# zengxianyu/sketchedit

Hardware: AMD Instinct MI355X
Metric: images/sec (higher is better)
Workload: dtype f32; 1 GPU; SketchEdit inference forward (netM+netG, use_cam, pool max) 256x256 batch 32 per GPU, procedural weights; global_batch=32, size=256, per_gpu_batch=32, execution=default, two streams

## Files before the change

sketchedit_amd/csrc/se_api.hip:

```cpp
#include "../../include/sketchedit_hip.h"
#include "../../include/sketchedit_png.h"
#include "se_kernels.h"
#include "se_pack.h"

#include <cstdarg>
#include <cstdint>
#include <cstdlib>
#include <cstdio>
#include <cstring>
#include <algorithm>
#include <map>
#include <mutex>
#include <numeric>
#include <string>
#include <vector>

using namespace se;

namespace {


#define ENC(p)                                                                                    \
  {p "2_downsample", 24, 96, 3, 2, 1, ACT_ELU, 0}, {p "3", 48, 96, 3, 1, 1, ACT_ELU, 0},          \
      {p "4_downsample", 48, 192, 3, 2, 1, ACT_ELU, 0}, {p "5", 96, 192, 3, 1, 1, ACT_ELU, 0},    \
      {p "6", 96, 192, 3, 1, 1, ACT_ELU, 0}, {p "7_atrous", 96, 192, 3, 1, 2, ACT_ELU, 0},        \
      {p "8_atrous", 96, 192, 3, 1, 4, ACT_ELU, 0}, {p "9_atrous", 96, 192, 3, 1, 8, ACT_ELU, 0}, \
      {p "10_atrous", 96, 192, 3, 1, 16, ACT_ELU, 0}
#define DEC(p, c11in, c17out)                                                                        \
  {p "11", c11in, 192, 3, 1, 1, ACT_ELU, 0}, {p "12", 96, 192, 3, 1, 1, ACT_ELU, 0},                 \
      {p "13_upsample_conv", 96, 96, 3, 1, 1, ACT_ELU, 1}, {p "14", 48, 96, 3, 1, 1, ACT_ELU, 0},    \
      {p "15_upsample_conv", 48, 48, 3, 1, 1, ACT_ELU, 1}, {p "16", 24, 24, 3, 1, 1, ACT_ELU, 0},    \
      {p "17", 12, c17out, 3, 1, 1, ACT_NONE, 0}

const LayerDef G_LAYERS[] = {
    {"conv1", 5, 48, 5, 1, 1, ACT_ELU, 0}, ENC("conv"), DEC("conv", 192, 3),
    {"wconv1", 5, 48, 5, 1, 1, ACT_ELU, 0}, ENC("wconv"),
    {"xconv1", 3, 48, 5, 1, 1, ACT_ELU, 0},
    {"xconv2_downsample", 24, 48, 3, 2, 1, ACT_ELU, 0}, {"xconv3", 24, 96, 3, 1, 1, ACT_ELU, 0},
    {"xconv4_downsample", 48, 96, 3, 2, 1, ACT_ELU, 0}, {"xconv5", 48, 192, 3, 1, 1, ACT_ELU, 0},
    {"xconv6", 96, 192, 3, 1, 1, ACT_ELU, 0}, {"xconv7_atrous", 96, 192, 3, 1, 2, ACT_ELU, 0},
    {"xconv8_atrous", 96, 192, 3, 1, 4, ACT_ELU, 0}, {"xconv9_atrous", 96, 192, 3, 1, 8, ACT_ELU, 0},
    {"xconv10_atrous", 96, 192, 3, 1, 16, ACT_ELU, 0},
    {"pmconv1", 3, 48, 5, 1, 1, ACT_ELU, 0},
    {"pmconv2_downsample", 24, 48, 3, 2, 1, ACT_ELU, 0}, {"pmconv3", 24, 96, 3, 1, 1, ACT_ELU, 0},
    {"pmconv4_downsample", 48, 192, 3, 2, 1, ACT_ELU, 0}, {"pmconv5", 96, 192, 3, 1, 1, ACT_ELU, 0},
    {"pmconv6", 96, 192, 3, 1, 1, ACT_RELU, 0}, {"pmconv9", 96, 192, 3, 1, 1, ACT_ELU, 0},
    {"pmconv10", 96, 192, 3, 1, 1, ACT_ELU, 0},
    DEC("allconv", 192, 3),
};
const LayerDef M_LAYERS[] = {
    {"conv1", 4, 48, 5, 1, 1, ACT_ELU, 0}, ENC("conv"), DEC("conv", 96, 3), DEC("conv_mask_", 96, 1),
};
const int NG = sizeof(G_LAYERS) / sizeof(LayerDef), NM = sizeof(M_LAYERS) / sizeof(LayerDef);


struct Arena {
  struct Blk { size_t off, size; bool used; };
  std::vector<Blk> blks;
  size_t cap = 0, peak = 0;
  bool dry = false;
  char* base = nullptr;
  void reset(char* b, size_t c, bool d, int which = 0) {
    base = d ? (char*)(which ? ((size_t)1 << 62) + 4096 : 4096) : b;
    cap = d ? (size_t)1 << 61 : c; dry = d; peak = 0;
    blks.clear(); blks.push_back({0, cap, false});
  }
  bool owns(const void* p) const { return (size_t)p >= (size_t)base && (size_t)p < (size_t)base + cap; }
  float* alloc(size_t nfloats) {
    size_t need = (nfloats * 4 + 255) & ~(size_t)255;
    for (size_t i = 0; i < blks.size(); ++i) {
      if (!blks[i].used && blks[i].size >= need) {
        size_t off = blks[i].off;
        if (blks[i].size > need) {
          Blk rest{off + need, blks[i].size - need, false};
          blks[i].size = need;
          blks.insert(blks.begin() + i + 1, rest);
        }
        blks[i].used = true;
        if (off + need > peak) peak = off + need;
        return (float*)(base + off);
      }
    }
    return nullptr;
  }
  void release(const float* p) {
    if (!p) return;
    size_t off = (const char*)p - base;
    for (size_t i = 0; i < blks.size(); ++i) {
      if (blks[i].off == off && blks[i].used) {
        blks[i].used = false;
        if (i + 1 < blks.size() && !blks[i + 1].used) { blks[i].size += blks[i + 1].size; blks.erase(blks.begin() + i + 1); }
        if (i > 0 && !blks[i - 1].used) { blks[i - 1].size += blks[i].size; blks.erase(blks.begin() + i); }
        return;
      }
    }
  }
};

}

struct se_ctx {
  int device = 0;
  std::mutex mu;
  std::string err;
  std::map<std::string, Layer> G, M;
  Layer wconv1_j4;
  float* zeros = nullptr;
  float* lut8 = nullptr;
  Arena arena;
  Arena arena2;
  hipStream_t st = nullptr;
  hipStream_t st_main = nullptr;
  hipStream_t st_side = nullptr;
  hipEvent_t ev_fork = nullptr, ev_join = nullptr;
  bool dry = false;
  bool low_latency = false;
  int cur_net = SE_NET_G;
  bool bf16 = false;
  bool serial = false;
  bool fork2 = true;
  bool conservative = false;
  const se_netG_taps* taps = nullptr;
  float* vbias_ws = nullptr;
  const float* vec32 = nullptr;
  unsigned char* rgb8 = nullptr;
  unsigned char* m8 = nullptr;
  Profiler prof;
  struct Peaks { size_t main, side; };
  std::map<std::vector<long long>, Peaks> peaks;
  size_t dry_max_act = 0;
  std::map<std::vector<long long>, long long> act_per_img;
  struct GraphEntry {
    std::vector<long long> key;
    hipGraph_t graph = nullptr;
    hipGraphExec_t exec = nullptr;
    hipStream_t stream = nullptr;
    unsigned long long last_use = 0;
  };
  unsigned long long graph_clock = 0;
  std::vector<GraphEntry> graphs;
  struct ResampleTable {
    int in, out, filter, ksize;
    std::vector<int> host;
    int* dev = nullptr;
    unsigned long long last_use = 0;
  };
  std::vector<ResampleTable> rs_tables;
  unsigned long long rs_clock = 0;
  unsigned char* rs_scratch = nullptr;
  size_t rs_scratch_bytes = 0;
  hipStream_t rs_stream = nullptr;
  bool rs_used = false;
  hipEvent_t rs_event = nullptr;
  se_window* win_host = nullptr;
  se_window* win_dev = nullptr;
  size_t win_cap = 0, win_pos = 0;
  hipEvent_t win_half_done[2] = {nullptr, nullptr};
  bool win_half_used[2] = {false, false};
  hipStream_t win_stream = nullptr;
  bool win_used = false;
  hipEvent_t win_event = nullptr;
};

namespace {

thread_local std::string g_create_err;

int fail(se_ctx* c, const char* fmt, ...) {
  char buf[512];
  va_list ap;
  va_start(ap, fmt);
  vsnprintf(buf, sizeof buf, fmt, ap);
  va_end(ap);
  if (c) c->err = buf; else g_create_err = buf;
  return 1;
}
#define HIPCHK(c, call)                                                                   \
  do {                                                                                    \
    hipError_t e_ = (call);                                                               \
    if (e_ != hipSuccess) return fail(c, "%s failed: %s (%s:%d)", #call, hipGetErrorString(e_), __FILE__, __LINE__); \
  } while (0)

int xcd_remap_enabled() { return opt(OPT_XCD_REMAP); }

long long addr_limit() {
  const int v = opt(OPT_TEST_OFFSET_LIMIT);
  return v > 0 ? (long long)v : (1ll << 31);
}

int poison_byte() {
  const int v = opt(OPT_TEST_POISON);
  return v >= 1 && v <= 255 ? v : 0;
}
int poison(se_ctx* c, void* p, size_t bytes, hipStream_t st) {
  const int v = poison_byte();
  if (!v || !p || !bytes) return 0;
  HIPCHK(c, hipMemsetAsync(p, v, bytes, st));
  return 0;
}

int try_rtile(se_ctx* c, const Layer& L, bool bf, const float* src0, int C0, const float* src1, float* dst, int B, int Hin, int Win,
              int Ho, int Wo, int pad, bool* done) {
  *done = false;
  const LayerDef& d = L.def;
  if (!opt(OPT_RTILE) || src1 || d.stride != 1 || d.rate != 1 || (L.cfg != GC_N48 && L.cfg != GC_N24)) return 0;
  {
    const int TR0 = rtile_rows(bf);
    const long tiles = (long)B * ((Hin + TR0 - 1) / TR0) * ((Win + 15) / 16) * (d.up ? 4 : 1);
    if (c->low_latency && tiles < opt(OPT_RTILE_LL_MIN)) return 0;
  }
  const int es = bf ? 2 : 4, gran = bf ? 8 : 4;
  const DirectImage& di = L.direct[bf];
  const int CG = di.CG, nch = di.nch;
  const float* wimg = di.w;
  if (!wimg || C0 != CG * gran) return 0;
  {
    const int wx_mode = opt(OPT_RTILE_WX);
    if (wx_mode != 0 && !bf && L.d_wx && d.k == 3 && !d.up && C0 == 24 && d.cin == 24 && d.cout == 24 && (Win % 2) == 0 &&
        (long long)B * Hin * Win * 96 < (1ll << 31)) {
      RTileParams p;
      memset(&p, 0, sizeof p);
      p.src = src0; p.wpk = L.d_wx; p.bias = L.d_b; p.dst = dst;
      p.B = B; p.Hin = Hin; p.Win = Win; p.C = C0; p.G = L.G; p.OH = Ho; p.OW = Wo;
      p.ty = (Hin + 15) / 16; p.tx = (Win + 15) / 16;
      p.act = d.act; p.xcd = xcd_remap_enabled(); p.NP = 32;
      udiv_magic_host((unsigned)(p.ty * p.tx), &p.div_cg_m, &p.div_cg_l);
      udiv_magic_host((unsigned)p.tx, &p.div_rw_m, &p.div_rw_l);
      const double alg = 2.0 * (double)B * Ho * Wo * d.cout * d.cin * 9;
      const bool two_d = wx_mode != 1 && L.d_wx2 && (Hin % 2) == 0;
      set_launch_cost(alg, 4.0 * ((double)B * Hin * Win * d.cin + (double)B * Ho * Wo * (d.cout / 2)), d.name,
                      (double)B * p.ty * p.tx * 8.0 * (two_d ? 96.0 : 160.0) * 2048.0);
      if (two_d) {
        p.wpk = L.d_wx2;
        HIPCHK(c, launch_rtilew2(p, c->st));
        *done = true;
        return 0;
      }
      HIPCHK(c, launch_rtilew(p, c->st));
      *done = true;
      return 0;
    }
  }
  if (opt(OPT_RTILE_DENSE) != 0 && !bf && L.d_wd && L.dense && d.k == 5 && !d.up && L.cfg == GC_N48 && (long long)Hin * Win * C0 * 4 < (1ll << 31)) {
    const long long per_img = (long long)Hin * Win * C0 * 4;
    const long long lim = addr_limit();
    const int bmax = (int)std::max<long long>(1, (lim - 1) / per_img);
    for (int b0 = 0; b0 < B; b0 += bmax) {
      const int nb = std::min(bmax, B - b0);
      RTileParams p;
      memset(&p, 0, sizeof p);
      p.src = src0 + (size_t)b0 * Hin * Win * C0; p.wpk = L.d_wd; p.bias = L.d_b; p.dst = dst + (size_t)b0 * Ho * Wo * L.G;
      p.B = nb; p.Hin = Hin; p.Win = Win; p.C = C0; p.G = L.G; p.OH = Ho; p.OW = Wo;
      p.ty = (Hin + 7) / 8; p.tx = (Win + 15) / 16;
      p.act = d.act; p.xcd = xcd_remap_enabled(); p.dense = L.dense; p.nch = L.nchd; p.NP = 48;
      const double alg = 2.0 * (double)nb * Ho * Wo * d.cout * d.cin * 25;
      if (opt(OPT_RTILE_D5W) != 0 && L.d_wdw && (Win % 2) == 0) {
        p.wpk = L.d_wdw; p.dense = L.dense + 100;
        set_launch_cost(alg, 4.0 * ((double)nb * Hin * Win * d.cin + (double)nb * Ho * Wo * (d.cout / 2)), d.name,
                        (double)nb * p.ty * p.tx * 4.0 * (6.0 * ((5 * L.dense + 3) / 4) * 3.0) * 2048.0);
        HIPCHK(c, launch_rtile(p, c->st));
        continue;
      }
      set_launch_cost(alg, 4.0 * ((double)nb * Hin * Win * d.cin + (double)nb * Ho * Wo * (d.cout / 2)), d.name,
                      2.0 * (double)nb * Hin * Win * 48.0 * (4.0 * ((25 * L.dense + 3) / 4)));
      HIPCHK(c, launch_rtile(p, c->st));
    }
    *done = true;
    return 0;
  }
  if (opt(OPT_RTILE_DENSE) != 0 && bf && L.d_w16d && d.k == 5 && !d.up && L.cfg == GC_N48 && C0 == 8 &&
      (long long)B * Hin * Win * 16 < (1ll << 31)) {
    RTileParams p;
    memset(&p, 0, sizeof p);
    p.src = src0; p.wpk = L.d_w16d; p.bias = L.d_b; p.dst = dst;
    p.B = B; p.Hin = Hin; p.Win = Win; p.C = C0; p.CG = 1; p.T = 25; p.KW = 5;
    p.pad = pad; p.OH = Ho; p.OW = Wo; p.G = (L.G + 7) & ~7;
    p.nch = 2; p.NP = 48; p.RH = 32 + 4; p.RW = 21;
    p.raw_bytes = (p.RH * p.RW * 8 + 1023) & ~1023;
    udiv_magic_host((unsigned)p.RW, &p.div_rw_m, &p.div_rw_l);
    udiv_magic_host(1u, &p.div_cg_m, &p.div_cg_l);
    p.ty = (Hin + 31) / 32; p.tx = (Win + 15) / 16;
    p.act = d.act; p.bf16 = 1; p.xcd = xcd_remap_enabled(); p.dense = 204;
    const double alg = 2.0 * (double)B * Ho * Wo * d.cout * d.cin * 25;
    set_launch_cost(alg, 2.0 * ((double)B * Hin * Win * d.cin + (double)B * Ho * Wo * (d.cout / 2)), d.name,
                    2.0 * (double)B * Hin * Win * 48.0 * 128.0);
    HIPCHK(c, launch_rtile(p, c->st));
    *done = true;
    return 0;
  }
  const int KW = d.up ? 2 : d.k, KH = KW;
  RTileParams p;
  memset(&p, 0, sizeof p);
  const int TR = rtile_rows(bf);
  p.RH = TR + KH - 1; p.RW = 16 + KW - 1;
  p.raw_bytes = (p.RH * p.RW * C0 * es + 1023) & ~1023;
  if (p.raw_bytes + nch * L.NP * 128 > 80 * 1024) return 0;
  if ((long long)B * Hin * Win * C0 * es >= (1ll << 31)) return 0;
  p.src = src0; p.wpk = wimg; p.bias = L.d_b; p.dst = dst;
  p.B = B; p.Hin = Hin; p.Win = Win; p.C = C0; p.CG = CG; p.T = L.T; p.KW = KW;
  p.magicCG = (65536 + CG - 1) / CG; p.magicKW = 256 / KW + 1;
  for (int gi = 0; gi < nch * 8 + 8; ++gi)
    if (((gi * p.magicCG) >> 16) != gi / CG) return 0;
  for (int t = 0; t <= L.T + 8; ++t)
    if (((t * p.magicKW) >> 8) != t / KW) return 0;
  p.pad = pad; p.up2 = d.up ? 1 : 0; p.OH = Ho; p.OW = Wo;
  p.G = bf ? (L.G + 7) & ~7 : L.G;
  p.nch = nch; p.NP = L.NP;
  udiv_magic_host((unsigned)(C0 * es / 16), &p.div_cg_m, &p.div_cg_l);
  udiv_magic_host((unsigned)p.RW, &p.div_rw_m, &p.div_rw_l);
  p.ty = (Hin + TR - 1) / TR; p.tx = (Win + 15) / 16;
  p.act = d.act; p.bf16 = bf ? 1 : 0; p.xcd = xcd_remap_enabled();
  {
    const double alg = 2.0 * (double)B * Ho * Wo * d.cout * d.cin * d.k * d.k;
    const double exec = 2.0 * (double)B * Hin * Win * (d.up ? 4.0 : 1.0) * L.NP * (nch * (bf ? 64.0 : 32.0));
    set_launch_cost(alg, (double)es * ((double)B * Hin * Win * d.cin + (double)B * Ho * Wo * (d.cout / 2)), d.name, exec);
  }
  HIPCHK(c, launch_rtile(p, c->st));
  *done = true;
  return 0;
}

int run_gather(se_ctx* c, const Layer& L, bool bf, const float* src0, int C0, const float* src1, int C1, int src1_vec, float* dst,
               int B, int Hin, int Win, int Ho, int Wo, int pad) {
  const LayerDef& d = L.def;
  const DirectImage& di = L.direct[bf];
  const int es = bf ? 2 : 4, gran = bf ? 8 : 4;
  GConvParams p;
  memset(&p, 0, sizeof p);
  p.bf16 = bf ? 1 : 0;
  p.src0 = src0; p.src1 = src1 ? src1 : src0; p.wpk = di.w; p.bias = L.d_b; p.dst = dst; p.zeros = c->zeros;
  p.B = B; p.Hin = Hin; p.Win = Win; p.Ho = d.up ? Hin : Ho; p.Wo = d.up ? Win : Wo;
  p.up2 = d.up ? 1 : 0; p.OH = Ho; p.OW = Wo;
  p.C0 = C0; p.C1 = C1 ? C1 : C0; p.C0g = C0 / gran; p.CG = di.CG;
  const int KW = d.up ? 2 : d.k;
  p.T = L.T; p.KW = KW; p.stride = d.stride; p.dil = d.rate; p.pad = pad;
  p.magicCG = (65536 + di.CG - 1) / di.CG; p.magicKW = 256 / KW + 1; p.magicKH = L.T / KW;
  for (int gi = 0; gi < di.nch * 8 + 8; ++gi)
    if (((gi * p.magicCG) >> 16) != gi / di.CG) return fail(c, "layer %s: magic division check failed", d.name);
  for (int t = 0; t <= L.T + 8; ++t)
    if (((t * p.magicKW) >> 8) != t / KW) return fail(c, "layer %s: magic tap division check failed", d.name);
  const int Gs = bf ? (L.G + 7) & ~7 : L.G;
  if ((double)B * Hin * Win * (C0 > C1 ? C0 : C1) * es >= 2147483648.0 || (double)B * Ho * Wo * Gs * es >= 2147483648.0)
    return fail(c, "layer %s: a tensor of this launch exceeds 2^31 bytes (32-bit byte offsets) -- split the batch", d.name);
  for (int j = 0; j < p.magicKH; ++j) p.rep |= 1u << (j * KW);
  udiv_magic_host((unsigned)(p.Ho * p.Wo), &p.div_hw_m, &p.div_hw_l);
  udiv_magic_host((unsigned)p.Wo, &p.div_w_m, &p.div_w_l);
  p.Hlim = Hin; p.Wlim = Win;
  p.src1_vec = src1_vec; p.nch = di.nch; p.G = Gs; p.act = d.act; p.total_pix = B * p.Ho * p.Wo;
  p.xcd = xcd_remap_enabled();
  p.np_full = L.NP; p.nf_full = L.NP / 32; p.small_grid = c->low_latency ? 1 : 0;
  {
    const double alg = 2.0 * (double)B * Ho * Wo * d.cout * d.cin * d.k * d.k;
    const double exec = 2.0 * (double)B * p.Ho * p.Wo * (d.up ? 4.0 : 1.0) * L.NP * (di.nch * (bf ? 64.0 : 32.0));
    set_launch_cost(alg, (double)es * ((double)B * Hin * Win * d.cin + (double)B * Ho * Wo * (d.cout / 2)), d.name, exec);
  }
  HIPCHK(c, launch_gconv(L.cfg, p, c->st));
  return 0;
}

static bool rconv16_dual_ok(const Layer& L, const LayerDef& d, int Hin, int Win) {
  if (opt(OPT_RCONV16_DUAL) == 0) return false;
  return L.d_w16s && (d.rate % 2) == 0 && Win / d.rate == 8 && Hin / d.rate <= 8 && Hin / d.rate >= 4;
}

int run_gconv16(se_ctx* c, const Layer& L, const float* src0, int C0, const float* src1, int C1, int src1_vec, float* dst,
                int B, int Hin, int Win, int Ho, int Wo, int pad) {
  const LayerDef& d = L.def;
  if (!L.direct[1].w) return fail(c, "layer %s: no bf16 weight image", d.name);
  if ((C0 + C1) != L.direct[1].CG * 8) return fail(c, "layer %s: bf16 source channels %d+%d != packed %d", d.name, C0, C1, L.direct[1].CG * 8);
  const bool use_rconv = opt(OPT_RCONV16) != 0;
  {
    if (opt(OPT_VECBIAS) != 0 && use_rconv && !c->low_latency && src1 && src1_vec && c->vbias_ws && c->vec32 && L.d_w16s && L.d_wv16 &&
        d.k == 3 && d.stride == 1 && d.rate == 1 && !d.up && d.cin == 192 && d.cout == 192 && C0 == 96 && C1 == 96 &&
        Hin >= 12 && Win >= 12 && (long long)B * Hin * Win * 192 < (1ll << 31)) {
      HIPCHK(c, launch_vecbias(L.d_wv16, c->vec32, c->vbias_ws, B, 96, c->st, 1));
      RConvParams rp;
      memset(&rp, 0, sizeof rp);
      rp.src = src0; rp.wpk = L.d_w16s; rp.bias = L.d_b; rp.dst = dst; rp.vbias = c->vbias_ws;
      rp.B = B; rp.h = Hin; rp.w = Win; rp.d = 1; rp.hs = Hin; rp.ws = Win;
      rp.ty = (Hin + 7) / 8; rp.tx = (Win + 15) / 16;
      rp.act = d.act; rp.xcd = xcd_remap_enabled();
      const double alg = 2.0 * (double)B * Ho * Wo * d.cout * d.cin * 9;
      set_launch_cost(alg, 2.0 * 2.0 * (double)B * Hin * Win * 96, d.name, 2.0 * (double)B * Hin * Win * 192.0 * 864.0);
      HIPCHK(c, launch_rconv16(rp, c->st));
      return 0;
    }
  }
  if (use_rconv && !c->low_latency && d.k == 3 && d.stride == 1 && !d.up && d.cin == 96 && d.cout == 192 && !src1 && C0 == 96 &&
      (Hin % d.rate) == 0 && (Win % d.rate) == 0 && L.direct[1].nch == 14 && L.d_w16s && (long long)B * Hin * Win * 192 < (1ll << 31) &&
      ((Hin / d.rate >= 12 && Win / d.rate >= 12) || rconv16_dual_ok(L, d, Hin, Win))) {
    RConvParams rp;
    memset(&rp, 0, sizeof rp);
    rp.dual = !(Hin / d.rate >= 12 && Win / d.rate >= 12);
    rp.src = src0; rp.wpk = L.d_w16s; rp.bias = L.d_b; rp.dst = dst;
    rp.B = B; rp.h = Hin; rp.w = Win; rp.d = d.rate; rp.hs = Hin / d.rate; rp.ws = Win / d.rate;
    rp.ty = (rp.hs + 7) / 8; rp.tx = (rp.ws + 15) / 16;
    rp.act = d.act; rp.xcd = xcd_remap_enabled();
    const double alg = 2.0 * (double)B * Ho * Wo * d.cout * d.cin * 9;
    set_launch_cost(alg, 2.0 * 2.0 * (double)B * Hin * Win * 96, d.name, 2.0 * (double)B * Hin * Win * 192.0 * 864.0);
    HIPCHK(c, launch_rconv16(rp, c->st));
    return 0;
  }
  const bool use_rconv96 = opt(OPT_RCONV96) != 0;
  if (use_rconv96 && !c->low_latency && L.d_w96 && !src1 && C0 == d.cin && Hin >= 12 && Win >= 12 &&
      (long long)B * Ho * Wo * 96 < (1ll << 31) && (long long)B * Hin * Win * C0 * 2 < (1ll << 31)) {
    RConv96Params rp;
    memset(&rp, 0, sizeof rp);
    rp.src = src0; rp.wpk = L.d_w96; rp.bias = L.d_b; rp.dst = dst;
    rp.B = B; rp.h = Hin; rp.w = Win; rp.CG = C0 / 8;
    rp.stride = d.stride; rp.oh = Ho; rp.ow = Wo;
    rp.ty = ((d.stride == 2 ? Ho : Hin) + 15) / 16; rp.tx = ((d.stride == 2 ? Wo : Win) + 15) / 16;
    rp.up2 = d.up ? 1 : 0; rp.act = d.act; rp.xcd = xcd_remap_enabled();
    const int T = d.up ? 4 : 9, nstep = (T * rp.CG + 3) / 4;
    const double alg = 2.0 * (double)B * Ho * Wo * d.cout * d.cin * 9;
    set_launch_cost(alg, 2.0 * ((double)B * Hin * Win * d.cin + (double)B * Ho * Wo * 48), d.name,
                    2.0 * (double)B * (d.stride == 2 ? (double)Ho * Wo : (double)Hin * Win) * (d.up ? 4.0 : 1.0) * 96.0 * (nstep * 32.0));
    HIPCHK(c, launch_rconv96(rp, c->st));
    return 0;
  }
  {
    bool done = false;
    if (try_rtile(c, L, true, src0, C0, src1, dst, B, Hin, Win, Ho, Wo, pad, &done)) return 1;
    if (done) return 0;
  }
  return run_gather(c, L, true, src0, C0, src1, C1, src1_vec, dst, B, Hin, Win, Ho, Wo, pad);
}

static WinoParams wino_params(const float* src, const float* upk, const float* bias, float* dst, int B, int h, int w, int d,
                              int tcols, int act) {
  WinoParams wp;
  memset(&wp, 0, sizeof wp);
  wp.src = src; wp.upk = upk; wp.bias = bias; wp.dst = dst;
  wp.B = B; wp.h = h; wp.w = w; wp.d = d; wp.th = h / 2; wp.tw = w / tcols;
  wp.total_tiles = B * wp.th * wp.tw; wp.act = act;
  wp.xcd = xcd_remap_enabled();
  udiv_magic_host((unsigned)(wp.th * wp.tw), &wp.div_tpi_m, &wp.div_tpi_l);
  udiv_magic_host((unsigned)wp.tw, &wp.div_tw_m, &wp.div_tw_l);
  udiv_magic_host((unsigned)wp.d, &wp.div_d_m, &wp.div_d_l);
  return wp;
}

int run_gconv(se_ctx* c, const Layer& L, const float* src0, int C0, const float* src1, int C1, int src1_vec, float* dst,
              int B, int Hin, int Win) {
  const LayerDef& d = L.def;
  const ConvShape sh = conv_shape(d, Hin, Win);
  const int Ho = sh.Ho, Wo = sh.Wo, pad = sh.pad;
  if (!L.packed) return fail(c, "layer %s: weights not loaded", d.name);
  if (c->bf16) return run_gconv16(c, L, src0, C0, src1, C1, src1_vec, dst, B, Hin, Win, Ho, Wo, pad);
  if ((C0 + C1) != L.direct[0].CG * 4) return fail(c, "layer %s: source channels %d+%d != packed %d", d.name, C0, C1, L.direct[0].CG * 4);
  const int ll_min_wg = opt(OPT_LL_WINO_MIN_WG), ll_min_wg48 = opt(OPT_LL_WINO48_MIN_WG);
  auto wino_grid_ok = [&](long wgs, bool n192 = false) {
    const int m = n192 ? ll_min_wg : ll_min_wg48;
    return !c->low_latency || (m > 0 && wgs >= m);
  };
  const bool use_wino = opt(OPT_WINOGRAD) != 0;
  const bool wino_src_ok = (!src1 && C0 == 96 && d.cin == 96) || (src1 && C0 == 96 && C1 == 96 && d.cin == 192);
  const bool wino_addr_ok = (long long)B * Hin * Win * 384 < (1ll << 31);
  const double alg3x3 = 2.0 * (double)B * Ho * Wo * d.cout * d.cin * 9;
  if (use_wino && !d.up && L.d_u && wino_src_ok && !wino_addr_ok) {
    static bool said = false;
    if (!said) {
      said = true;
      fprintf(stderr, "sketchedit_hip: layer %s: %d x %dx%d x 96 floats exceed the Winograd kernel's 32-bit byte offsets; "
                      "using the direct kernel (about 2x slower) -- split the batch\n", d.name, B, Hin, Win);
    }
  }
  if (use_wino && !d.up && L.d_u && wino_src_ok && wino_addr_ok && (Hin % (2 * d.rate)) == 0 && (Win % (2 * d.rate)) == 0 &&
      wino_grid_ok(((long)(Hin / 2) * (Win / 2) + 63) / 64, true)) {
    const bool folded = opt(OPT_VECBIAS) != 0 && src1 && src1_vec && d.rate == 1 && L.d_u1 && L.d_wv && c->vbias_ws && Hin >= 2 && Win >= 2;
    if (folded) HIPCHK(c, launch_vecbias(L.d_wv, src1, c->vbias_ws, B, 96, c->st));
    const float* s1 = folded ? nullptr : src1;
    const int f43_mode = opt(OPT_WINOGRAD_F43);
    const bool f43_net_ok = c->cur_net == SE_NET_G || (f43_mode == 1 && !c->conservative);
    const bool f43 = (f43_mode == 1 || f43_mode == 2) && f43_net_ok && (s1 ? (!src1_vec && L.d_u24b) : L.d_u24 != nullptr) && L.d_ub24 && (Win % (4 * d.rate)) == 0;
    WinoParams wp = f43 ? wino_params(src0, s1 ? L.d_u24b : L.d_u24, L.d_ub24, dst, B, Hin, Win, d.rate, 4, d.act)
                        : wino_params(src0, folded ? L.d_u1 : L.d_u, L.d_b, dst, B, Hin, Win, d.rate, 2, d.act);
    wp.src1 = s1; wp.src1_vec = folded ? 0 : src1_vec; wp.vbias = folded ? c->vbias_ws : nullptr;
    if ((double)B * Hin * Win * 384.0 >= 2147483648.0) return fail(c, "layer %s: tensor exceeds 2^31 bytes", d.name);
    if (f43) {
      set_launch_cost(alg3x3, 4.0 * 2.0 * (double)B * Hin * Win * 96, d.name, alg3x3 * 24.0 / 72.0 * (folded ? 0.5 : 1.0));
      HIPCHK(c, launch_wino24(wp, c->st));
      return 0;
    }
    set_launch_cost(alg3x3, 4.0 * 2.0 * (double)B * Hin * Win * 96, d.name, alg3x3 * 16.0 / 36.0 * (folded ? 0.5 : 1.0));
    HIPCHK(c, launch_wino(wp, c->st));
    return 0;
  }
  {
    if (use_wino && opt(OPT_WINOGRAD_F43) != 0 && !d.up && !src1 && C0 == 48 && d.cin == 48 && d.cout == 192 && d.stride == 1 && L.d_u24 && L.d_ub24 &&
        (long long)B * Hin * Win * 384 < (1ll << 31) && (Hin % (2 * d.rate)) == 0 && (Win % (4 * d.rate)) == 0 &&
        wino_grid_ok(((long)(Hin / 2) * (Win / 4) + 31) / 32, true)) {
      const WinoParams wp = wino_params(src0, L.d_u24, L.d_ub24, dst, B, Hin, Win, d.rate, 4, d.act);
      set_launch_cost(alg3x3, 4.0 * ((double)B * Hin * Win * 48 + (double)B * Hin * Win * 96), d.name, alg3x3 * 24.0 / 72.0);
      HIPCHK(c, launch_wino24_c48(wp, c->st));
      return 0;
    }
  }
  const bool use_wino48 = opt(OPT_WINOGRAD48) != 0;
  if (use_wino && use_wino48 && !d.up && L.d_u && L.d_ub && !src1 && C0 == 48 && d.cin == 48 && (long long)B * Hin * Win * 192 < (1ll << 31) &&
      (Hin % (2 * d.rate)) == 0 && (Win % (2 * d.rate)) == 0 && wino_grid_ok(((long)(Hin / 2) * (Win / 2) + 63) / 64)) {
    const WinoParams wp = wino_params(src0, L.d_u, L.d_ub, dst, B, Hin, Win, d.rate, 2, d.act);
    set_launch_cost(alg3x3, 4.0 * 2.0 * (double)B * Hin * Win * 48, d.name, alg3x3 * 16.0 / 36.0);
    HIPCHK(c, launch_wino48(wp, c->st));
    return 0;
  }
  if (use_wino && use_wino48 && !d.up && L.d_u && L.d_ub && !src1 && C0 == 24 && d.cin == 24 && d.cout == 96 && d.stride == 1 &&
      (long long)B * Hin * Win * 192 < (1ll << 31) && (Hin % (2 * d.rate)) == 0 && (Win % (2 * d.rate)) == 0 &&
      wino_grid_ok(((long)(Hin / 2) * (Win / 2) + 63) / 64)) {
    const WinoParams wp = wino_params(src0, L.d_u, L.d_ub, dst, B, Hin, Win, d.rate, 2, d.act);
    set_launch_cost(alg3x3, 4.0 * ((double)B * Hin * Win * 24 + (double)B * Hin * Win * 48), d.name, alg3x3 * 16.0 / 36.0);
    HIPCHK(c, launch_wino48_c24(wp, c->st));
    return 0;
  }
  const bool use_winoup = opt(OPT_WINOGRAD_UP) != 0;
  if (use_wino && use_winoup && d.up && L.d_u && L.d_ub && !src1 && C0 == 96 && d.cin == 96 &&
      (long long)B * Hin * Win * 384 < (1ll << 31) && (Hin % 2) == 0 && (Win % 2) == 0 &&
      wino_grid_ok(4 * (((long)(Hin / 2) * (Win / 2) + 63) / 64))) {
    const WinoParams wp = wino_params(src0, L.d_u, L.d_ub, dst, B, Hin, Win, 1, 2, d.act);
    set_launch_cost(alg3x3, 4.0 * ((double)B * Hin * Win * 96 + (double)B * Ho * Wo * 48), d.name,
                    alg3x3 * 9.0 / 36.0);
    HIPCHK(c, launch_winoup(wp, c->st));
    return 0;
  }
  const bool use_winoup48 = opt(OPT_WINOGRAD_UP48) != 0;
  if (use_wino && use_winoup && use_winoup48 && d.up && L.d_u && L.d_ub && !src1 && C0 == 48 && d.cin == 48 && d.cout == 48 &&
      (long long)B * Hin * Win * 192 < (1ll << 31) && (long long)B * Ho * Wo * 96 < (1ll << 31) && (Hin % 2) == 0 && (Win % 2) == 0 &&
      wino_grid_ok(4 * (((long)(Hin / 2) * (Win / 2) + 63) / 64))) {
    const WinoParams wp = wino_params(src0, L.d_u, L.d_ub, dst, B, Hin, Win, 1, 2, d.act);
    set_launch_cost(alg3x3, 4.0 * ((double)B * Hin * Win * 48 + (double)B * Ho * Wo * 24), d.name,
                    alg3x3 * 9.0 / 36.0 * 28.0 / 27.0);
    HIPCHK(c, launch_winoup48(wp, c->st));
    return 0;
  }
  {
    bool done = false;
    if (try_rtile(c, L, false, src0, C0, src1, dst, B, Hin, Win, Ho, Wo, pad, &done)) return 1;
    if (done) return 0;
  }
  return run_gather(c, L, false, src0, C0, src1, C1, src1_vec, dst, B, Hin, Win, Ho, Wo, pad);
}

struct Act {
  float* p = nullptr;
  int H = 0, W = 0, C = 0;
};

struct Plan {
  se_ctx* c;
  std::map<std::string, Layer>& net;
  int B;
  int rc = 0;
  Arena* ar;
  Plan(se_ctx* c_, std::map<std::string, Layer>& n, int B_) : c(c_), net(n), B(B_), ar(&c_->arena) {}
  float* alloc_raw(size_t nfloats) {
    float* p = ar->alloc(nfloats);
    if (!p && !rc) rc = fail(c, "workspace too small (need more than %zu bytes)", ar->cap);
    if (p && !rc && !c->dry && poison(c, p, (nfloats * 4 + 255) & ~(size_t)255, c->st)) rc = 1;
    return p;
  }
  Act alloc(int H, int W, int C) {
    Act a; a.H = H; a.W = W;
    if (c->bf16) {
      a.C = (C + 7) & ~7;
      a.p = alloc_raw(((size_t)B * H * W * a.C + 1) / 2);
    } else {
      a.C = C;
      a.p = alloc_raw((size_t)B * H * W * C);
    }
    if (c->dry) c->dry_max_act = std::max(c->dry_max_act, (size_t)B * H * W * a.C * (c->bf16 ? 2 : 4));
    return a;
  }
  void release(const float* p) {
    if (!p) return;
    if (c->arena2.owns(p)) c->arena2.release(p); else c->arena.release(p);
  }
  void free(Act& a) { release(a.p); a.p = nullptr; }
  bool forked() const { return (c->low_latency || (c->fork2 && !c->serial)) && c->st_side; }
  int side_begin() {
    if (!forked()) return 0;
    ar = &c->arena2;
    if (c->dry) return 0;
    HIPCHK(c, hipEventRecord(c->ev_fork, c->st_main));
    HIPCHK(c, hipStreamWaitEvent(c->st_side, c->ev_fork, 0));
    c->st = c->st_side;
    return 0;
  }
  int side_end() {
    if (!forked()) return 0;
    ar = &c->arena;
    if (c->dry) return 0;
    HIPCHK(c, hipEventRecord(c->ev_join, c->st_side));
    c->st = c->st_main;
    return 0;
  }
  int join() {
    if (!forked() || c->dry) return 0;
    HIPCHK(c, hipStreamWaitEvent(c->st_main, c->ev_join, 0));
    return 0;
  }
  Act conv(const char* name, Act& in, bool rel = true, const float* src1 = nullptr, int C1 = 0, int vec = 0) {
    if (rc) return Act();
    return conv_layer(net.at(name), in, rel, src1, C1, vec);
  }
  Act conv_layer(Layer& L, Act& in, bool rel = true, const float* src1 = nullptr, int C1 = 0, int vec = 0) {
    Act out;
    if (rc) return out;
    const ConvShape sh = conv_shape(L.def, in.H, in.W);
    out = alloc(sh.Ho, sh.Wo, L.def.cout / 2);
    if (rc) return out;
    if (!c->dry) rc = run_gconv(c, L, in.p, in.C, src1, C1, vec, out.p, B, in.H, in.W);
    if (rel) free(in);
    return out;
  }
};

Act encoder(Plan& P, const std::string& p, Act& in, Act* keep9, Layer* first = nullptr) {
  Act x = first ? P.conv_layer(*first, in) : P.conv((p + "1").c_str(), in);
  x = P.conv((p + "2_downsample").c_str(), x);
  x = P.conv((p + "3").c_str(), x);
  x = P.conv((p + "4_downsample").c_str(), x);
  x = P.conv((p + "5").c_str(), x);
  x = P.conv((p + "6").c_str(), x);
  x = P.conv((p + "7_atrous").c_str(), x);
  x = P.conv((p + "8_atrous").c_str(), x);
  Act x9 = P.conv((p + "9_atrous").c_str(), x);
  Act x10 = P.conv((p + "10_atrous").c_str(), x9, keep9 == nullptr);
  if (keep9) *keep9 = x9;
  return x10;
}

Act decoder(Plan& P, const std::string& p, Act& in, const float* src1 = nullptr, int C1 = 0, int vec = 0) {
  Act x = P.conv((p + "11").c_str(), in, true, src1, C1, vec);
  x = P.conv((p + "12").c_str(), x);
  x = P.conv((p + "13_upsample_conv").c_str(), x);
  x = P.conv((p + "14").c_str(), x);
  x = P.conv((p + "15_upsample_conv").c_str(), x);
  x = P.conv((p + "16").c_str(), x);
  return x;
}

int small(Plan& P, const char* name, Act& in, int mode, float* out_nchw, float* hard, const float* img,
          const float* mask, float* xnow, float* composed, int no_mask_coarse, long packed_bs = 0,
          const unsigned char* lock = nullptr) {
  if (P.rc) return P.rc;
  se_ctx* c = P.c;
  if (!c->dry) {
    Layer& L = P.net.at(name);
    if (!L.packed) return P.rc = fail(c, "layer %s: weights not loaded", name);
    SmallConvParams sp;
    memset(&sp, 0, sizeof sp);
    sp.x = in.p; sp.w = L.direct[c->bf16].w; sp.b = L.d_b; sp.B = P.B; sp.H = in.H; sp.W = in.W; sp.cout = L.def.cout;
    sp.bf16 = c->bf16 ? 1 : 0;
    sp.mode = mode; sp.out_nchw = out_nchw; sp.hard = hard; sp.img = img; sp.mask = mask; sp.xnow = xnow;
    sp.composed = composed; sp.no_mask_coarse = no_mask_coarse;
    if (mode == 3) { sp.rgb8 = c->rgb8; sp.m8 = c->m8; }
    if (mode == 0) sp.lock = lock;
    if (packed_bs) {
      if (mode == 0) sp.out_bs = packed_bs;
      if (mode == 3) { sp.mask_bs = packed_bs; sp.comp_bs = packed_bs; }
    }
    set_launch_cost(2.0 * (double)P.B * in.H * in.W * L.def.cout * 108.0,
                    4.0 * (double)P.B * in.H * in.W * (12 + L.def.cout), L.def.name);
    hipError_t e = launch_small_conv(sp, c->st);
    if (e != hipSuccess) return P.rc = fail(c, "small conv %s: %s", name, hipGetErrorString(e));
  }
  P.free(in);
  return 0;
}

int plan_netM(se_ctx* c, const float* image, const float* sketch, float* mask_out, float* hard_out, float* maskim_out,
              int B, int H, int W, long packed_bs = 0, const unsigned char* lock = nullptr) {
  Plan P(c, c->M, B);
  c->cur_net = SE_NET_M;
  Act in = P.alloc(H, W, 4);
  if (P.rc) return P.rc;
  if (!c->dry) HIPCHK(c, c->bf16 ? launch_pack_m16(image, sketch, in.p, B, H, W, c->st) : launch_pack_m(image, sketch, in.p, B, H, W, c->st));
  Act x9;
  const bool want_img = maskim_out != nullptr;
  Act x10 = encoder(P, "conv", in, want_img ? &x9 : nullptr);
  if (want_img) {
    Act d = decoder(P, "conv", x9);
    small(P, "conv17", d, 1, maskim_out, nullptr, nullptr, nullptr, nullptr, nullptr, 0);
  }
  Act d = decoder(P, "conv_mask_", x10);
  small(P, "conv_mask_17", d, 0, mask_out, hard_out, nullptr, nullptr, nullptr, nullptr, 0, packed_bs, lock);
  return P.rc;
}

int run_attention(se_ctx* c, Plan& P, Act& x, const float* mask_full, Act& out, float* similar_nchw);

int plan_netG(se_ctx* c, const float* x, const float* x2, const float* mask, const float* mask2, const float* guide,
              float* coarse_out, float* fine_out, const float* soft_mask, float* composed_out, int B, int H, int W,
              int flags, long packed_bs = 0) {
  Plan P(c, c->G, B);
  c->cur_net = SE_NET_G;
  const int joint = (flags & SE_FLAG_JOINT_TRAIN_INP) ? 1 : 0;
  Act cin = P.alloc(H, W, 8);
  P.ar = P.forked() ? &c->arena2 : &c->arena;
  Act sin = P.alloc(H, W, joint ? 4 : 8);
  P.ar = &c->arena;
  if (P.rc) return P.rc;
  if (!c->dry)
    HIPCHK(c, (c->bf16 ? launch_pack_g16 : launch_pack_g)(x, x2, mask, mask2, guide, cin.p, sin.p, B, H, W,
                                                          (flags & SE_FLAG_NO_MASK_CC) ? 1 : 0, joint, c->st));
  if (P.side_begin()) return 1;
  Act xs = encoder(P, "wconv", sin, nullptr, joint ? &c->wconv1_j4 : nullptr);
  Act part = P.alloc(1, COLREDUCE_SPLITS, 192), vec32 = P.alloc(1, 1, 192), vec = P.alloc(1, 1, 96);
  if (P.rc) return P.rc;
  if (!c->dry)
    HIPCHK(c, launch_colreduce(xs.p, part.p, c->bf16 ? vec32.p : vec.p, B, xs.H * xs.W, 96, (flags & SE_FLAG_POOL_MAX) ? 0 : 1,
                               c->st, c->bf16 ? 1 : 0, c->bf16 ? vec.p : nullptr));
  if (!c->dry && c->taps && c->taps->style_vec)
    HIPCHK(c, hipMemcpyAsync(c->taps->style_vec, c->bf16 ? vec32.p : vec.p, (size_t)B * 96 * 4, hipMemcpyDeviceToDevice, c->st));
  P.free(xs);
  P.free(part);
  if (!c->bf16) P.free(vec32);
  if (P.side_end()) return 1;
  Act xc = encoder(P, "conv", cin, nullptr);
  if (P.rc) return P.rc;
  if (P.join()) return 1;
  float* vb = P.alloc_raw((size_t)B * 9 * 192);
  if (P.rc) return P.rc;
  c->vbias_ws = vb;
  c->vec32 = c->bf16 ? vec32.p : nullptr;
  Act d = decoder(P, "conv", xc, vec.p, 96, 1);
  c->vbias_ws = nullptr; c->vec32 = nullptr;
  P.release(vb);
  if (c->bf16) P.free(vec32);
  P.free(vec);
  Act xnow = P.alloc(H, W, 4);
  if (P.rc) return P.rc;
  small(P, "conv17", d, 2, coarse_out, nullptr, x, mask, xnow.p, nullptr, (flags & SE_FLAG_NO_MASK_COARSE) ? 1 : 0);
  if (P.rc) return P.rc;
  if (P.side_begin()) return 1;
  Act pm = P.conv("pmconv1", xnow, false);
  pm = P.conv("pmconv2_downsample", pm);
  pm = P.conv("pmconv3", pm);
  pm = P.conv("pmconv4_downsample", pm);
  pm = P.conv("pmconv5", pm);
  pm = P.conv("pmconv6", pm);
  if (P.rc) return P.rc;
  if (!c->dry && c->taps && c->taps->pmconv6)
    HIPCHK(c, (c->bf16 ? launch_nhwc16_to_nchw : launch_nhwc_to_nchw)(pm.p, c->taps->pmconv6, B, 96, 96, pm.H, pm.W, c->st));
  if (flags & SE_FLAG_USE_CAM) {
    Act att = P.alloc(pm.H, pm.W, 96);
    if (P.rc) return P.rc;
    if (run_attention(c, P, pm, mask, att, nullptr)) return P.rc ? P.rc : 1;
    P.free(pm);
    pm = att;
    if (!c->dry && c->taps && c->taps->attn_out)
      HIPCHK(c, (c->bf16 ? launch_nhwc16_to_nchw : launch_nhwc_to_nchw)(pm.p, c->taps->attn_out, B, 96, 96, pm.H, pm.W, c->st));
  }
  pm = P.conv("pmconv9", pm);
  pm = P.conv("pmconv10", pm);
  if (P.rc) return P.rc;
  if (P.side_end()) return 1;
  Act hcur = P.conv("xconv1", xnow, false);
  hcur = P.conv("xconv2_downsample", hcur);
  hcur = P.conv("xconv3", hcur);
  hcur = P.conv("xconv4_downsample", hcur);
  hcur = P.conv("xconv5", hcur);
  hcur = P.conv("xconv6", hcur);
  hcur = P.conv("xconv7_atrous", hcur);
  hcur = P.conv("xconv8_atrous", hcur);
  hcur = P.conv("xconv9_atrous", hcur);
  Act hallu = P.conv("xconv10_atrous", hcur);
  if (P.rc) return P.rc;
  if (P.join()) return 1;
  P.free(xnow);
  Act d2 = decoder(P, "allconv", hallu, pm.p, 96, 0);
  P.free(pm);
  small(P, "allconv17", d2, 3, fine_out, nullptr, x, soft_mask, nullptr, soft_mask ? composed_out : nullptr, 0, packed_bs);
  c->rgb8 = nullptr; c->m8 = nullptr;
  return P.rc;
}

int att_row_stride(int R, bool bf) {
  const int chunk = bf ? 64 : 32;
  int Rp = (R + chunk - 1) / chunk * chunk;
  return Rp;
}

bool att_streaming(int h, int w, bool bf, bool want_similar) {
  const int R = (h / 2) * (w / 2), Rp = att_row_stride(R, bf);
  const bool fits = (double)R * Rp * 4.0 < 2147483648.0;
  if (want_similar && !fits) return true;
  if (opt(OPT_ATT_STREAM) == 1 && !want_similar) return true;
  return !fits;
}

int run_attention(se_ctx* c, Plan& P, Act& x, const float* mask_full, Act& out, float* similar_nchw) {
  const int h = x.H, w = x.W, B = P.B;
  const int hs = (h - 4) / 2 + 1, ws = (w - 4) / 2 + 1, L = hs * ws, Lp = (L + 31) & ~31;
  const bool bf = c->bf16;
  const bool stream = att_streaming(h, w, bf, similar_nchw != nullptr);
  const int hc = h / 2, wc = w / 2, R = hc * wc;
  const int Rp = att_row_stride(R, bf);
  const int guard = (wc + 8 + 63) & ~63;
  if (stream && similar_nchw)
    return P.rc = fail(c, "attention: similar_out (the %d x %d score matrix) is not available on a %dx%d feature map: "
                          "it runs in the streaming form, which never forms it", L, L, h, w);
  float* part = P.alloc_raw((size_t)B * COLREDUCE_SPLITS * 96);
  float* rn = P.alloc_raw((size_t)B * 96);
  float* xn = P.alloc_raw(bf ? ((size_t)B * h * w * 96 + 1) / 2 : (size_t)B * h * w * 96);
  float *valid = nullptr, *S = nullptr, *S2 = nullptr, *xT = nullptr, *stats = nullptr;
  if (stream) {
    valid = P.alloc_raw(3 * (size_t)B * Rp);
    stats = P.alloc_raw((size_t)B * R * 2);
    xT = P.alloc_raw((bf ? (size_t)B * 4 * 96 * Rp / 2 : (size_t)B * 4 * 96 * Rp) + att_stream_xt_tail());
  } else {
    valid = P.alloc_raw(7 * ((size_t)B * Rp + guard) + (size_t)B * 768 + (size_t)B * hc * 384);
    stats = P.alloc_raw((size_t)B * R * 2);
    xT = P.alloc_raw(bf ? (size_t)B * 4 * 96 * Rp / 2 : (size_t)B * 4 * 96 * Rp);
    S = P.alloc_raw((size_t)B * R * Rp + 2 * guard);
    S2 = P.alloc_raw(bf ? (size_t)B * R * Rp / 2 : (size_t)B * R * Rp);
  }
  if (P.rc) return P.rc;
  if (!c->dry) {
    HIPCHK(c, launch_colreduce(x.p, part, rn, B, h * w, 96, 2, c->st, bf ? 1 : 0));
    AttParams a;
    memset(&a, 0, sizeof a);
    a.x = x.p; a.rn = rn; a.xn = xn; a.hard = mask_full; a.out = out.p;
    a.B = B; a.h = h; a.w = w; a.hs = hs; a.ws = ws; a.L = L; a.Lp = Lp;
    a.scale = 10.f; a.th = 0.1f;
    if (stream) {
      a.hc = hc; a.wc = wc; a.R = R; a.Rp = Rp; a.bf16 = bf ? 1 : 0;
      a.validR = valid; a.kmul = valid + (size_t)B * Rp; a.kadd = valid + 2 * (size_t)B * Rp;
      a.xT = xT; a.stats = stats;
      HIPCHK(c, launch_attention_stream(a, c->st));
    } else {
      a.hc = hc; a.wc = wc; a.R = R; a.Rp = Rp; a.bf16 = bf ? 1 : 0;
      a.validR = valid + guard; a.xT = xT; a.E = S + guard; a.P = S2; a.stats = stats; a.guard = guard; a.similar = similar_nchw;
      a.kmul = valid + ((size_t)B * Rp + guard) + guard; a.kadd = valid + 2 * ((size_t)B * Rp + guard) + guard;
      a.kadd2 = valid + 3 * ((size_t)B * Rp + guard) + guard; a.ea4 = valid + 4 * ((size_t)B * Rp + guard) + guard;
      a.ea = valid + 5 * ((size_t)B * Rp + guard) + guard; a.eb = valid + 6 * ((size_t)B * Rp + guard) + guard;
      a.emean = valid + 7 * ((size_t)B * Rp + guard); a.epart = a.emean + (size_t)B * 768;
      HIPCHK(c, launch_attention(a, c->st));
    }
  }
  P.release(S2); P.release(S); P.release(xT); P.release(stats); P.release(valid);
  P.release(xn); P.release(rn); P.release(part);
  return 0;
}

int check_dims(se_ctx* c, int B, int H, int W) {
  if (B < 1 || H < 16 || W < 16 || (H % 8) || (W % 8)) return fail(c, "bad shape B=%d H=%d W=%d (H, W must be multiples of 8, >= 16)", B, H, W);
  return 0;
}

long long max_act_bytes_per_image(se_ctx* c, int H, int W, int flags) {
  const std::vector<long long> key = {H, W, (flags & SE_FLAG_BF16) ? 1 : 0};
  auto it = c->act_per_img.find(key);
  if (it != c->act_per_img.end()) return it->second;
  const bool dry0 = c->dry, ll0 = c->low_latency, bf0 = c->bf16;
  c->dry = true; c->low_latency = false; c->bf16 = (flags & SE_FLAG_BF16) != 0;
  c->dry_max_act = 0;
  float dummy;
  c->arena.reset(nullptr, 0, true, 0); c->arena2.reset(nullptr, 0, true, 1);
  plan_netM(c, nullptr, nullptr, nullptr, nullptr, &dummy, 1, H, W, 0);
  c->arena.reset(nullptr, 0, true, 0); c->arena2.reset(nullptr, 0, true, 1);
  plan_netG(c, nullptr, nullptr, nullptr, nullptr, nullptr, nullptr, nullptr, nullptr, nullptr, 1, H, W, SE_FLAG_USE_CAM | SE_FLAG_POOL_MAX, 0);
  c->dry = dry0; c->low_latency = ll0; c->bf16 = bf0;
  const long long v = (long long)c->dry_max_act;
  c->act_per_img[key] = v;
  return v;
}

int pass_size(se_ctx* c, int B, int H, int W, int flags) {
  const long long per_img = max_act_bytes_per_image(c, H, W, flags);
  const long long lim = addr_limit();
  if (per_img <= 0) { fail(c, "internal: no activation size for %dx%d", H, W); return 0; }
  if (per_img >= lim) {
    fail(c, "a %dx%d image exceeds the kernels' 32-bit byte offsets (%lld bytes per activation, limit %lld)", H, W, per_img, lim);
    return 0;
  }
  const long long bmax = (lim - 1) / per_img;
  if (B <= bmax) return B;
  const long long passes = (B + bmax - 1) / bmax;
  return (int)((B + passes - 1) / passes);
}

se_ctx::Peaks plan_peaks(se_ctx* c, int which, int B, int H, int W, int flags, bool want_maskim) {
  const std::vector<long long> key = {which, B, H, W,
                                      flags & (SE_FLAG_USE_CAM | SE_FLAG_JOINT_TRAIN_INP | SE_FLAG_LOW_LATENCY | SE_FLAG_BF16),
                                      want_maskim ? 1 : 0, c->fork2 ? 1 : 0, opt_epoch(), c->serial ? 1 : 0};
  auto it = c->peaks.find(key);
  if (it != c->peaks.end()) return it->second;
  const bool dry0 = c->dry, ll0 = c->low_latency, bf0 = c->bf16;
  c->dry = true;
  c->low_latency = (flags & SE_FLAG_LOW_LATENCY) != 0;
  c->bf16 = (flags & SE_FLAG_BF16) != 0;
  float dummy;
  se_ctx::Peaks pk{0, 0};
  if (which & 1) {
    c->arena.reset(nullptr, 0, true, 0); c->arena2.reset(nullptr, 0, true, 1);
    plan_netM(c, nullptr, nullptr, nullptr, nullptr, want_maskim ? &dummy : nullptr, B, H, W);
    pk.main = c->arena.peak; pk.side = c->arena2.peak;
  }
  if (which & 2) {
    c->arena.reset(nullptr, 0, true, 0); c->arena2.reset(nullptr, 0, true, 1);
    plan_netG(c, nullptr, nullptr, nullptr, nullptr, nullptr, nullptr, nullptr, nullptr, nullptr, B, H, W, flags);
    if (c->arena.peak > pk.main) pk.main = c->arena.peak;
    if (c->arena2.peak > pk.side) pk.side = c->arena2.peak;
  }
  c->dry = dry0; c->low_latency = ll0; c->bf16 = bf0;
  c->peaks[key] = pk;
  return pk;
}

int carve(se_ctx* c, const se_ctx::Peaks& pk, void* ws, size_t ws_bytes, size_t tail) {
  if (ws_bytes < pk.main + pk.side + tail)
    return fail(c, "workspace too small: %zu bytes, this call needs %zu", ws_bytes, pk.main + pk.side + tail);
  c->arena.reset((char*)ws, ws_bytes - tail - pk.side, false);
  c->arena2.reset((char*)ws + (ws_bytes - tail - pk.side), pk.side, false);
  return 0;
}

void begin_call(se_ctx* c, void* stream, int flags) {
  c->st = c->st_main = (hipStream_t)stream;
  c->dry = false;
  c->low_latency = (flags & SE_FLAG_LOW_LATENCY) != 0;
  c->bf16 = (flags & SE_FLAG_BF16) != 0;
  c->conservative = (flags & SE_FLAG_CONSERVATIVE) != 0;
  c->serial = c->prof.on;
  c->taps = nullptr;
  c->rgb8 = nullptr; c->m8 = nullptr;
  c->cur_net = SE_NET_G;
  set_profiler(&c->prof);
}

void destroy_graph(se_ctx::GraphEntry& g) {
  if (g.exec) {
    if (g.stream) (void)hipStreamSynchronize(g.stream);
    (void)hipGraphExecDestroy(g.exec);
  }
  if (g.graph) (void)hipGraphDestroy(g.graph);
  g.exec = nullptr; g.graph = nullptr;
}
void drop_graphs(se_ctx* c) {
  for (auto& g : c->graphs) destroy_graph(g);
  c->graphs.clear();
}
void evict_lru_graph(se_ctx* c) {
  size_t lru = 0;
  for (size_t i = 1; i < c->graphs.size(); ++i)
    if (c->graphs[i].last_use < c->graphs[lru].last_use) lru = i;
  destroy_graph(c->graphs[lru]);
  c->graphs.erase(c->graphs.begin() + lru);
}

int rs_enter(se_ctx* c, hipStream_t st) {
  if (c->rs_used && c->rs_stream != st) {
    if (!c->rs_event) HIPCHK(c, hipEventCreateWithFlags(&c->rs_event, hipEventDisableTiming));
    HIPCHK(c, hipEventRecord(c->rs_event, c->rs_stream));
    HIPCHK(c, hipStreamWaitEvent(st, c->rs_event, 0));
  }
  c->rs_stream = st;
  c->rs_used = true;
  return 0;
}

const se_ctx::ResampleTable* rs_table(se_ctx* c, int in, int out, int filter) {
  for (auto& t : c->rs_tables)
    if (t.in == in && t.out == out && t.filter == filter) { t.last_use = ++c->rs_clock; return &t; }
  const int ksize = resample_ksize(in, out, filter);
  if (ksize < 0) { fail(c, "resize: bad arguments (in %d, out %d, filter %d)", in, out, filter); return nullptr; }
  if (ksize > RESAMPLE_MAX_KSIZE) { fail(c, "resize: %d -> %d needs %d taps per output, more than the kernels take (%d)", in, out, ksize, RESAMPLE_MAX_KSIZE); return nullptr; }
  if (c->rs_tables.size() >= 64) {
    size_t lru = 0;
    for (size_t i = 1; i < c->rs_tables.size(); ++i)
      if (c->rs_tables[i].last_use < c->rs_tables[lru].last_use) lru = i;
    (void)hipStreamSynchronize(c->rs_stream);
    (void)hipFree(c->rs_tables[lru].dev);
    c->rs_tables.erase(c->rs_tables.begin() + lru);
  }
  se_ctx::ResampleTable t;
  t.in = in; t.out = out; t.filter = filter; t.ksize = ksize;
  t.host.resize((size_t)out * (2 + ksize));
  resample_coeffs(in, out, filter, t.host.data(), t.host.data() + 2 * (size_t)out);
  hipError_t e = hipMalloc(&t.dev, t.host.size() * sizeof(int));
  if (e == hipSuccess) e = hipMemcpyAsync(t.dev, t.host.data(), t.host.size() * sizeof(int), hipMemcpyHostToDevice, c->rs_stream);
  if (e != hipSuccess) {
    if (t.dev) (void)hipFree(t.dev);
    fail(c, "resize: coefficient upload failed: %s", hipGetErrorString(e));
    return nullptr;
  }
  t.last_use = ++c->rs_clock;
  c->rs_tables.push_back(std::move(t));
  return &c->rs_tables.back();
}

unsigned char* rs_scratch(se_ctx* c, size_t bytes) {
  if (bytes > c->rs_scratch_bytes) {
    if (c->rs_scratch) {
      (void)hipStreamSynchronize(c->rs_stream);
      (void)hipFree(c->rs_scratch);
      c->rs_scratch = nullptr; c->rs_scratch_bytes = 0;
    }
    const size_t sz = (bytes + ((size_t)1 << 20) - 1) & ~(((size_t)1 << 20) - 1);
    if (hipMalloc(&c->rs_scratch, sz) != hipSuccess) { c->rs_scratch = nullptr; fail(c, "resize: cannot allocate %zu bytes", sz); return nullptr; }
    c->rs_scratch_bytes = sz;
  }
  return c->rs_scratch;
}

int resize_locked(se_ctx* c, hipStream_t st, const unsigned char* in, int B, int Hin, int Win, int C, ResizeOut o, int Hout,
                  int Wout, int filter) {
  if (!in || (o.mode == RESIZE_OUT_U8 ? !o.u8 : !o.f32)) return fail(c, "null pointer argument");
  if (B < 1 || B > 65535 || Hin < 1 || Win < 1 || Hout < 1 || Wout < 1 || Hin > 65535 || Hout > 65535 || (C != 1 && C != 3))
    return fail(c, "resize: bad shape B=%d %dx%dx%d -> %dx%d (C in {1, 3}, heights and B < 65536)", B, Hin, Win, C, Hout, Wout);
  if (filter != SE_RESAMPLE_BILINEAR && filter != SE_RESAMPLE_BICUBIC && filter != SE_RESAMPLE_LANCZOS)
    return fail(c, "resize: unsupported filter %d", filter);
  if (o.mode == RESIZE_OUT_IMAGE_F32) o.lut = c->lut8;
  if (rs_enter(c, st)) return 1;
  set_profiler(&c->prof);
  o.H = Hout; o.W = Wout;
  const bool need_h = Win != Wout, need_v = Hin != Hout;
  if (!need_h && !need_v) {
    if (o.mode == RESIZE_OUT_U8) {
      HIPCHK(c, hipMemcpyAsync(o.u8, in, (size_t)B * Hin * Win * C, hipMemcpyDeviceToDevice, st));
      return 0;
    }
    if (((size_t)Hin * Win) % 4 || ((uintptr_t)in & 3) || ((uintptr_t)o.f32 & 15))
      return fail(c, "resize: an unresized fp32 output needs H W %% 4 == 0, a 4-byte aligned input and a 16-byte aligned output");
    if (o.mode == RESIZE_OUT_IMAGE_F32 && C == 3)
      HIPCHK(c, launch_dequantize_u8(in, nullptr, c->lut8, o.f32, nullptr, B, Hin, Win, st));
    else if (o.mode == RESIZE_OUT_SKETCH_F32 && C == 1)
      HIPCHK(c, launch_dequantize_u8(nullptr, in, c->lut8, nullptr, o.f32, B, Hin, Win, st));
    else
      return fail(c, "resize: fp32 outputs are a 3-channel image or a 1-channel sketch");
    return 0;
  }
  const se_ctx::ResampleTable* th = need_h ? rs_table(c, Win, Wout, filter) : nullptr;
  const se_ctx::ResampleTable* tv = need_v ? rs_table(c, Hin, Hout, filter) : nullptr;
  if ((need_h && !th) || (need_v && !tv)) return 1;
  if (need_h && need_v) th = rs_table(c, Win, Wout, filter);
  const unsigned char* src = in;
  if (need_h) {
    ResizeOut oh = o;
    if (need_v) {
      unsigned char* mid = rs_scratch(c, (size_t)B * Hin * Wout * C);
      if (!mid) return 1;
      if (poison(c, mid, (size_t)B * Hin * Wout * C, st)) return 1;
      oh.mode = RESIZE_OUT_U8; oh.u8 = mid; oh.H = Hin;
      src = mid;
    }
    const int* d = th->dev;
    HIPCHK(c, launch_resample_h(in, d, d + 2 * (size_t)Wout, th->host.data(), th->ksize, B, Hin, Win, Wout, C, oh, st));
  }
// ... 87 lines not shown
  std::string key(name);
  if (key.rfind("module.", 0) == 0) key = key.substr(7);
  const size_t dot = key.rfind('.');
  if (dot == std::string::npos) return fail(c, "bad key %s", name);
  const std::string lname = key.substr(0, dot), kind = key.substr(dot + 1);
  auto& net = net_id == SE_NET_G ? c->G : c->M;
  auto it = net.find(lname);
  if (it == net.end()) return fail(c, "unexpected key %s for net %d", name, net_id);
  Layer& L = it->second;
  const LayerDef& d = L.def;
  if (kind == "weight") {
    if (ndim != 4 || shape[0] != d.cout || shape[1] != d.cin || shape[2] != d.k || shape[3] != d.k)
      return fail(c, "size mismatch for %s", name);
    L.w.assign(host, host + (size_t)d.cout * d.cin * d.k * d.k);
    L.have_w = true;
  } else if (kind == "bias") {
    if (ndim != 1 || shape[0] != d.cout) return fail(c, "size mismatch for %s", name);
    L.b.assign(host, host + d.cout);
    L.have_b = true;
  } else {
    return fail(c, "unexpected key %s", name);
  }
  if (!L.have_w || !L.have_b) return 0;
  std::vector<int> chans(d.cin);
  std::iota(chans.begin(), chans.end(), 0);
  if (pack_layer_images(L, chans, c->err)) return 1;
  if (std::string(d.name) == "wconv1" && d.cin == 5) {
    Layer& J = c->wconv1_j4;
    J.def = d; J.w = L.w; J.b = L.b; J.have_w = J.have_b = true;
    return pack_layer_images(J, {0, 1, 2, 4}, c->err);
  }
  return 0;
}

int se_weights_ready(se_ctx* c) {
  if (!c) return 0;
  std::lock_guard<std::mutex> lk(c->mu);
  for (auto* net : {&c->G, &c->M})
    for (auto& kv : *net)
      if (!kv.second.packed) return 0;
  return 1;
}

size_t se_workspace_bytes(se_ctx* c, int B, int H, int W) {
  if (!c) return 0;
  std::lock_guard<std::mutex> lk(c->mu);
  if (check_dims(c, B, H, W)) return 0;
  c->fork2 = opt(OPT_FORK_DEFAULT) != 0;
  size_t peak = 0;
  for (int cam = 0; cam < 2; ++cam)
    for (int joint = 0; joint < 2; ++joint)
      for (int ll = 0; ll < 2; ++ll)
        for (int bf = 0; bf < 2; ++bf) {
          const int flags = (cam ? SE_FLAG_USE_CAM : 0) | (joint ? SE_FLAG_JOINT_TRAIN_INP : 0) | (ll ? SE_FLAG_LOW_LATENCY : 0) |
                            (bf ? SE_FLAG_BF16 : 0) | SE_FLAG_POOL_MAX;
          const int nb = pass_size(c, B, H, W, flags);
          if (!nb) return 0;
          const int last = B % nb;
          for (int ser = 0; ser < 2; ++ser)
            for (int mi = 0; mi < 2; ++mi)
              for (int bb : {nb, last}) {
                if (!bb) continue;
                c->serial = ser != 0;
                const se_ctx::Peaks pk = plan_peaks(c, 3, bb, H, W, flags, mi != 0);
                if (pk.main + pk.side > peak) peak = pk.main + pk.side;
              }
          c->serial = false;
        }
  return peak + 6 * (((size_t)B * H * W * 4 + 255) & ~(size_t)255);
}

int se_netM_forward_ex(se_ctx* c, void* stream, const float* image, const float* sketch, float* mask_out,
                       float* maskim_out, void* ws, size_t ws_bytes, int B, int H, int W, int exec_flags) {
  if (!c) return 1;
  std::lock_guard<std::mutex> lk(c->mu);
  if (check_dims(c, B, H, W)) return 1;
  if (!image || !sketch || !mask_out || !ws) return fail(c, "null pointer argument");
  HIPCHK(c, hipSetDevice(c->device));
  c->serial = c->prof.on;
  c->fork2 = opt(OPT_FORK_DEFAULT) != 0;
  exec_flags &= SE_FLAG_LOW_LATENCY | SE_FLAG_BF16 | SE_FLAG_CONSERVATIVE;
  const int nb = pass_size(c, B, H, W, exec_flags);
  if (!nb) return 1;
  const size_t HW = (size_t)H * W;
  for (int b0 = 0; b0 < B; b0 += nb) {
    const int bb = std::min(nb, B - b0);
    if (carve(c, plan_peaks(c, 1, bb, H, W, exec_flags, maskim_out != nullptr), ws, ws_bytes, 0)) return 1;
    begin_call(c, stream, exec_flags);
    const int rc = plan_netM(c, image + b0 * 3 * HW, sketch + b0 * HW, mask_out + b0 * HW, nullptr,
                             maskim_out ? maskim_out + b0 * 3 * HW : nullptr, bb, H, W);
    if (rc) return rc;
  }
  return 0;
}

int se_netM_forward(se_ctx* c, void* stream, const float* image, const float* sketch, float* mask_out,
                    float* maskim_out, void* ws, size_t ws_bytes, int B, int H, int W) {
  return se_netM_forward_ex(c, stream, image, sketch, mask_out, maskim_out, ws, ws_bytes, B, H, W, 0);
}

int se_netG_forward_taps(se_ctx* c, void* stream, const float* x, const float* x2, const float* mask, const float* mask2,
                         const float* guide, float* coarse_out, float* fine_out, void* ws, size_t ws_bytes, int B, int H,
                         int W, int flags, const se_netG_taps* taps) {
  if (!c) return 1;
  std::lock_guard<std::mutex> lk(c->mu);
  if (check_dims(c, B, H, W)) return 1;
  if (!x || !x2 || !mask || !mask2 || !guide || !fine_out || !ws) return fail(c, "null pointer argument");
  HIPCHK(c, hipSetDevice(c->device));
  c->serial = c->prof.on;
  c->fork2 = opt(OPT_FORK_DEFAULT) != 0;
  const int nb = pass_size(c, B, H, W, flags);
  if (!nb) return 1;
  if (taps && nb < B) return fail(c, "se_netG_forward_taps: %d images do not fit one pass (%d)", B, nb);
  const size_t HW = (size_t)H * W;
  for (int b0 = 0; b0 < B; b0 += nb) {
    const int bb = std::min(nb, B - b0);
    if (carve(c, plan_peaks(c, 2, bb, H, W, flags, false), ws, ws_bytes, 0)) return 1;
    begin_call(c, stream, flags);
    c->taps = taps;
    const int rc = plan_netG(c, x + b0 * 3 * HW, x2 + b0 * 3 * HW, mask + b0 * HW, mask2 + b0 * HW, guide + b0 * HW,
                             coarse_out ? coarse_out + b0 * 3 * HW : nullptr, fine_out + b0 * 3 * HW, nullptr, nullptr, bb, H, W, flags);
    c->taps = nullptr;
    if (rc) return rc;
  }
  return 0;
}

int se_netG_forward(se_ctx* c, void* stream, const float* x, const float* x2, const float* mask, const float* mask2,
                    const float* guide, float* coarse_out, float* fine_out, void* ws, size_t ws_bytes, int B, int H,
                    int W, int flags) {
  return se_netG_forward_taps(c, stream, x, x2, mask, mask2, guide, coarse_out, fine_out, ws, ws_bytes, B, H, W, flags, nullptr);
}

namespace {
int enqueue_inference(se_ctx* c, void* stream, const float* image, const float* sketch, float* composed_out, float* mask_out,
                      float* hard_out, float* maskim_out, float* coarse_out, float* fine_out, void* ws, size_t ws_bytes,
                      int B, int H, int W, int flags, const unsigned char* lock8 = nullptr) {
  const size_t plane = ((size_t)B * H * W * 4 + 255) & ~(size_t)255;
  float* hard_all = hard_out ? hard_out : (float*)((char*)ws + ws_bytes - plane);
  const size_t HW = (size_t)H * W;
  const long packed_bs = (flags & SE_FLAG_PACKED_OUT) ? 4l * H * W : 0;
  if (packed_bs) mask_out = composed_out + 3 * HW;
  const size_t comp_bs = packed_bs ? (size_t)packed_bs : 3 * HW, mask_bs = packed_bs ? (size_t)packed_bs : HW;
  const int nb = pass_size(c, B, H, W, flags);
  if (!nb) return 1;
  if (!hard_out && poison(c, hard_all, plane, (hipStream_t)stream)) return 1;
  for (int b0 = 0; b0 < B; b0 += nb) {
    const int bb = std::min(nb, B - b0);
    const se_ctx::Peaks pk = plan_peaks(c, 3, bb, H, W, flags, maskim_out != nullptr);
    if (carve(c, pk, ws, ws_bytes, plane)) return 1;
    const float *img = image + b0 * 3 * HW, *sk = sketch + b0 * HW;
    float *hard = hard_all + b0 * HW, *mk = mask_out + b0 * mask_bs;
    begin_call(c, stream, flags);
    int rc = plan_netM(c, img, sk, mk, hard, maskim_out ? maskim_out + b0 * 3 * HW : nullptr, bb, H, W, packed_bs,
                       lock8 ? lock8 + b0 * HW : nullptr);
    if (rc) return rc;
    if (carve(c, pk, ws, ws_bytes, plane)) return 1;
    rc = plan_netG(c, img, img, hard, hard, sk, coarse_out ? coarse_out + b0 * 3 * HW : nullptr, fine_out ? fine_out + b0 * 3 * HW : nullptr,
                   mk, composed_out + b0 * comp_bs, bb, H, W, flags, packed_bs);
    if (rc) return rc;
  }
  return 0;
}
}

int se_inference(se_ctx* c, void* stream, const float* image, const float* sketch, float* composed_out,
                 float* mask_out, float* hard_out, float* maskim_out, float* coarse_out, float* fine_out, void* ws,
                 size_t ws_bytes, int B, int H, int W, int flags) {
  if (!c) return 1;
  std::lock_guard<std::mutex> lk(c->mu);
  if (check_dims(c, B, H, W)) return 1;
  if (!image || !sketch || !composed_out || (!mask_out && !(flags & SE_FLAG_PACKED_OUT)) || !ws) return fail(c, "null pointer argument");
  HIPCHK(c, hipSetDevice(c->device));
  c->serial = c->prof.on;
  c->fork2 = opt(OPT_FORK_DEFAULT) != 0;
  if (!(flags & SE_FLAG_GRAPH) || c->prof.on || poison_byte() != 0)
    return enqueue_inference(c, stream, image, sketch, composed_out, mask_out, hard_out, maskim_out, coarse_out, fine_out, ws,
                             ws_bytes, B, H, W, flags);
  const std::vector<long long> key = {(long long)(size_t)image, (long long)(size_t)sketch, (long long)(size_t)composed_out,
                                      (long long)(size_t)mask_out, (long long)(size_t)hard_out, (long long)(size_t)maskim_out,
                                      (long long)(size_t)coarse_out, (long long)(size_t)fine_out, (long long)(size_t)ws,
                                      (long long)ws_bytes, B, H, W, flags, opt_epoch()};
  se_ctx::GraphEntry* ge = nullptr;
  for (auto& g : c->graphs)
    if (g.key == key) { ge = &g; break; }
  if (!ge) {
    if (c->graphs.size() >= 16) evict_lru_graph(c);
    c->graphs.emplace_back();
    c->graphs.back().key = key;
    c->graphs.back().last_use = ++c->graph_clock;
    return enqueue_inference(c, stream, image, sketch, composed_out, mask_out, hard_out, maskim_out, coarse_out, fine_out, ws,
                             ws_bytes, B, H, W, flags);
  }
  ge->last_use = ++c->graph_clock;
  if (!ge->exec) {
    if (!stream) return fail(c, "SE_FLAG_GRAPH needs a non-default stream (capture is not permitted on the legacy stream)");
    HIPCHK(c, hipStreamBeginCapture((hipStream_t)stream, hipStreamCaptureModeThreadLocal));
    const int rc = enqueue_inference(c, stream, image, sketch, composed_out, mask_out, hard_out, maskim_out, coarse_out,
                                     fine_out, ws, ws_bytes, B, H, W, flags);
    hipGraph_t graph = nullptr;
    const hipError_t e = hipStreamEndCapture((hipStream_t)stream, &graph);
    if (rc) { if (graph) (void)hipGraphDestroy(graph); return rc; }
    if (e != hipSuccess) return fail(c, "hipStreamEndCapture failed: %s", hipGetErrorString(e));
    hipGraphExec_t exec = nullptr;
    const hipError_t e2 = hipGraphInstantiate(&exec, graph, nullptr, nullptr, 0);
    if (e2 != hipSuccess) { (void)hipGraphDestroy(graph); return fail(c, "hipGraphInstantiate failed: %s", hipGetErrorString(e2)); }
    ge->graph = graph; ge->exec = exec;
  }
  ge->stream = (hipStream_t)stream;
  ge->last_use = ++c->graph_clock;
  HIPCHK(c, hipGraphLaunch(ge->exec, (hipStream_t)stream));
  return 0;
}

int se_inference_locked(se_ctx* c, void* stream, const float* image, const float* sketch, const unsigned char* lock_u8,
                        float* composed_out, float* mask_out, float* hard_out, float* maskim_out, float* coarse_out, float* fine_out,
                        void* ws, size_t ws_bytes, int B, int H, int W, int flags) {
  if (!c) return 1;
  std::lock_guard<std::mutex> lk(c->mu);
  if (check_dims(c, B, H, W)) return 1;
  if (!image || !sketch || !composed_out || (!mask_out && !(flags & SE_FLAG_PACKED_OUT)) || !ws) return fail(c, "null pointer argument");
  HIPCHK(c, hipSetDevice(c->device));
  c->serial = c->prof.on;
  c->fork2 = opt(OPT_FORK_DEFAULT) != 0;
  return enqueue_inference(c, stream, image, sketch, composed_out, mask_out, hard_out, maskim_out, coarse_out, fine_out, ws,
                           ws_bytes, B, H, W, flags & ~SE_FLAG_GRAPH, lock_u8);
}

namespace {
int inference_u8_locked(se_ctx* c, void* stream, const float* image, const float* sketch, unsigned char* rgb_out,
                        unsigned char* mask_u8_out, void* ws, size_t ws_bytes, int B, int H, int W, int flags, int tail_planes,
                        const unsigned char* lock8 = nullptr) {
  flags &= ~(SE_FLAG_GRAPH | SE_FLAG_PACKED_OUT);
  const size_t plane = ((size_t)B * H * W * 4 + 255) & ~(size_t)255;
  const size_t tail = (2 + (size_t)tail_planes) * plane;
  if (ws_bytes < tail) return fail(c, "workspace too small: %zu bytes", ws_bytes);
  float* hard_all = (float*)((char*)ws + ws_bytes - tail + plane);
  float* soft_all = (float*)((char*)ws + ws_bytes - tail);
  const size_t HW = (size_t)H * W;
  const int nb = pass_size(c, B, H, W, flags);
  if (!nb) return 1;
  if (poison(c, soft_all, 2 * plane, (hipStream_t)stream)) return 1;
  for (int b0 = 0; b0 < B; b0 += nb) {
    const int bb = std::min(nb, B - b0);
    const se_ctx::Peaks pk = plan_peaks(c, 3, bb, H, W, flags, false);
    if (carve(c, pk, ws, ws_bytes, tail)) return 1;
    const float *img = image + b0 * 3 * HW, *sk = sketch + b0 * HW;
    float *hard = hard_all + b0 * HW, *soft = soft_all + b0 * HW;
    begin_call(c, stream, flags);
    int rc = plan_netM(c, img, sk, soft, hard, nullptr, bb, H, W, 0, lock8 ? lock8 + b0 * HW : nullptr);
    if (rc) return rc;
    if (carve(c, pk, ws, ws_bytes, tail)) return 1;
    c->rgb8 = rgb_out + b0 * 3 * HW; c->m8 = mask_u8_out ? mask_u8_out + b0 * HW : nullptr;
    rc = plan_netG(c, img, img, hard, hard, sk, nullptr, nullptr, soft, nullptr, bb, H, W, flags);
    if (rc) return rc;
  }
  return 0;
}
}

int se_inference_u8(se_ctx* c, void* stream, const float* image, const float* sketch, unsigned char* rgb_out,
                    unsigned char* mask_u8_out, void* ws, size_t ws_bytes, int B, int H, int W, int flags) {
  if (!c) return 1;
  std::lock_guard<std::mutex> lk(c->mu);
  if (check_dims(c, B, H, W)) return 1;
  if (!image || !sketch || !rgb_out || !ws) return fail(c, "null pointer argument");
  HIPCHK(c, hipSetDevice(c->device));
  c->serial = c->prof.on;
  c->fork2 = opt(OPT_FORK_DEFAULT) != 0;
  return inference_u8_locked(c, stream, image, sketch, rgb_out, mask_u8_out, ws, ws_bytes, B, H, W, flags, 0);
}

int se_inference_u8_locked(se_ctx* c, void* stream, const float* image, const float* sketch, const unsigned char* lock_u8,
                           unsigned char* rgb_out, unsigned char* mask_u8_out, void* ws, size_t ws_bytes, int B, int H, int W, int flags) {
  if (!c) return 1;
  std::lock_guard<std::mutex> lk(c->mu);
  if (check_dims(c, B, H, W)) return 1;
  if (!image || !sketch || !rgb_out || !ws) return fail(c, "null pointer argument");
  HIPCHK(c, hipSetDevice(c->device));
  c->serial = c->prof.on;
  c->fork2 = opt(OPT_FORK_DEFAULT) != 0;
  return inference_u8_locked(c, stream, image, sketch, rgb_out, mask_u8_out, ws, ws_bytes, B, H, W, flags, 0, lock_u8);
}

int se_dequantize_u8(se_ctx* c, void* stream, const unsigned char* image_u8, const unsigned char* sketch_u8, float* image_out,
                     float* sketch_out, int B, int H, int W) {
  if (!c) return 1;
  std::lock_guard<std::mutex> lk(c->mu);
  if (check_dims(c, B, H, W)) return 1;
  if ((image_out && !image_u8) || (sketch_out && !sketch_u8)) return fail(c, "null pointer argument");
  HIPCHK(c, hipSetDevice(c->device));
  set_profiler(&c->prof);
  HIPCHK(c, launch_dequantize_u8(image_u8, sketch_u8, c->lut8, image_out, sketch_out, B, H, W, (hipStream_t)stream));
  return 0;
}

int se_inference_u8io(se_ctx* c, void* stream, const unsigned char* image_u8, const unsigned char* sketch_u8,
                      unsigned char* rgb_out, unsigned char* mask_u8_out, void* ws, size_t ws_bytes, int B, int H, int W,
                      int flags) {
  if (!c) return 1;
  std::lock_guard<std::mutex> lk(c->mu);
  if (check_dims(c, B, H, W)) return 1;
  if (!image_u8 || !sketch_u8 || !rgb_out || !ws) return fail(c, "null pointer argument");
  HIPCHK(c, hipSetDevice(c->device));
  c->serial = c->prof.on;
  c->fork2 = opt(OPT_FORK_DEFAULT) != 0;
  const size_t plane = ((size_t)B * H * W * 4 + 255) & ~(size_t)255;
  if (ws_bytes < 6 * plane) return fail(c, "workspace too small: %zu bytes", ws_bytes);
  float* image = (float*)((char*)ws + ws_bytes - 4 * plane);
  float* sketch = (float*)((char*)ws + ws_bytes - plane);
  set_profiler(&c->prof);
  if (poison(c, image, 4 * plane, (hipStream_t)stream)) return 1;
// ... 973 lines not shown
```

sketchedit_amd/csrc/se_attention.hip:

```cpp
#include "se_device.h"

#include <cstdlib>

namespace se {


template <bool BF16>
__global__ void att2_prep_kernel(const AttParams p) {
  const long idx = (long)blockIdx.x * 256 + threadIdx.x;
  const long nx = (long)p.B * p.h * p.w * (BF16 ? 12 : 24);
  if (idx < nx) {
    if (BF16) {
      const int cg = idx % 12;
      const long pix = idx / 12;
      const int b = pix / (p.h * p.w);
      const uint4 v = *(const uint4*)((const char*)p.x + idx * 16);
      const f32x4 r0 = *(const f32x4*)(p.rn + b * 96 + cg * 8), r1 = *(const f32x4*)(p.rn + b * 96 + cg * 8 + 4);
      *(uint4*)((char*)p.xn + idx * 16) =
          make_uint4(pack_bf16x2(bf16_lo(v.x) * r0[0], bf16_hi(v.x) * r0[1]), pack_bf16x2(bf16_lo(v.y) * r0[2], bf16_hi(v.y) * r0[3]),
                     pack_bf16x2(bf16_lo(v.z) * r1[0], bf16_hi(v.z) * r1[1]), pack_bf16x2(bf16_lo(v.w) * r1[2], bf16_hi(v.w) * r1[3]));
    } else {
      const int cg = idx % 24;
      const long pix = idx / 24;
      const int b = pix / (p.h * p.w);
      const f32x4 v = *(const f32x4*)(p.x + idx * 4);
      f32x4 r = *(const f32x4*)(p.rn + b * 96 + cg * 4);
      if (p.sym) r = (f32x4){sqrtf(r[0]), sqrtf(r[1]), sqrtf(r[2]), sqrtf(r[3])};
      *(f32x4*)(p.xn + idx * 4) = v * r;
    }
  }
  if (idx < (long)p.B * p.Rp) {
    const int b = idx / p.Rp, s = idx - (long)b * p.Rp;
    float val = -1.f;
    const int sy = s / p.wc, sx = s - sy * p.wc;
    if (s < p.R && sy < p.hs && sx < p.ws) {
      const int H = p.h * 4, W = p.w * 4;
      float hole = 0.f;
      for (int yy = 0; yy < 16; ++yy)
        for (int xx = 0; xx < 16; ++xx) hole += p.hard[((long)b * H + sy * 8 + yy) * W + sx * 8 + xx];
      const float mm = 1.f - hole * (1.f / 256.f);
      val = mm > p.th ? 1.f : 0.f;
    }
    p.validR[idx] = val;
    if (p.kmul) {
      p.kmul[idx] = val > 0.f ? p.scale * 1.44269504088896340736f : 0.f;
      p.kadd[idx] = val >= 0.f ? 0.f : -INFINITY;
    }
  }
  if (idx < p.guard) {
    p.validR[-1 - idx] = -1.f;
    if (p.kmul) { p.kmul[-1 - idx] = 0.f; p.kadd[-1 - idx] = -INFINITY; }
    p.E[-1 - idx] = 0.f;
    p.E[(size_t)p.B * p.R * p.Rp + idx] = 0.f;
  }
}

template <bool BF16>
__global__ __launch_bounds__(256) void att2_transpose_kernel(const AttParams p) {
  __shared__ float t[32][97];
  const int s0 = blockIdx.x * 32, cls = blockIdx.y, b = blockIdx.z, py = cls >> 1, px = cls & 1;
  for (int e = threadIdx.x; e < 32 * 96; e += 256) {
    const int sl = e / 96, c = e - sl * 96, s = s0 + sl;
    float v = 0.f;
    if (s < p.R) {
      const int sy = s / p.wc, sx = s - sy * p.wc;
      const size_t at = ((size_t)(b * p.h + 2 * sy + py) * p.w + 2 * sx + px) * 96 + c;
      v = BF16 ? __uint_as_float((unsigned)((const unsigned short*)p.x)[at] << 16) : p.x[at];
    }
    t[sl][c] = v;
  }
  __syncthreads();
  for (int e = threadIdx.x; e < 96 * 32; e += 256) {
    const int c = e >> 5, sl = e & 31;
    const size_t at = (((size_t)b * 4 + cls) * 96 + c) * p.Rp + s0 + sl;
    if (BF16) ((unsigned short*)p.xT)[at] = (unsigned short)(__float_as_uint(t[sl][c]) >> 16);
    else p.xT[at] = t[sl][c];
  }
}

template <bool BF16>
__global__ __launch_bounds__(384) void att2_emean1_kernel(const AttParams p) {
  const int ry = blockIdx.x, b = blockIdx.y, e = threadIdx.x, cls = e / 96, c = e - cls * 96;
  const size_t row0 = ((size_t)(b * p.h + 2 * ry + (cls >> 1)) * p.w + (cls & 1)) * 96 + c;
  float acc = 0.f;
  for (int rx = 0; rx < p.wc; ++rx) {
    const size_t at = row0 + (size_t)rx * 192;
    acc += BF16 ? bf16_lo(((const unsigned short*)p.x)[at]) : p.x[at];
  }
  p.epart[((size_t)b * p.hc + ry) * 384 + e] = acc;
}
__global__ __launch_bounds__(384) void att2_emean2_kernel(const AttParams p) {
  const int b = blockIdx.x, e = threadIdx.x, c = e % 96;
  float a4[4] = {0.f, 0.f, 0.f, 0.f};
  for (int ry = 0; ry < p.hc; ry += 4)
#pragma unroll
    for (int u = 0; u < 4; ++u)
      if (ry + u < p.hc) a4[u] += p.epart[((size_t)b * p.hc + ry + u) * 384 + e];
  const float acc = (a4[0] + a4[1]) + (a4[2] + a4[3]);
  const float m = acc / (float)p.R;
  p.emean[(size_t)b * 768 + e] = m;
  p.emean[(size_t)b * 768 + 384 + e] = m * p.rn[b * 96 + c];
}
template <bool BF16>
__global__ __launch_bounds__(256) void att2_eoff_kernel(const AttParams p) {
  const int lane = threadIdx.x & 63;
  const long gi = (long)blockIdx.x * 4 + (threadIdx.x >> 6);
  if (gi >= (long)p.B * p.Rp) return;
  const int b = (int)(gi / p.Rp), r = (int)(gi - (long)b * p.Rp);
  const float* mx = p.emean + (size_t)b * 768, *mk = mx + 384;
  float a = 0.f, bb = 0.f, g = 0.f;
  if (r < p.R) {
    const int ry = r / p.wc, rx = r - ry * p.wc;
#pragma unroll
    for (int t = 0; t < 6; ++t) {
      const int e = t * 64 + lane, cls = e / 96, c = e - cls * 96;
      const size_t at = ((size_t)(b * p.h + 2 * ry + (cls >> 1)) * p.w + 2 * rx + (cls & 1)) * 96 + c;
      const float xv = BF16 ? bf16_lo(((const unsigned short*)p.x)[at]) : p.x[at];
      const float kv = BF16 ? bf16_lo(((const unsigned short*)p.xn)[at]) : p.xn[at];
      a = fmaf(xv, mk[e], a);
      bb = fmaf(mx[e], kv, bb);
      g = fmaf(mx[e], mk[e], g);
    }
#pragma unroll
    for (int o = 32; o > 0; o >>= 1) { a += __shfl_xor(a, o); bb += __shfl_xor(bb, o); g += __shfl_xor(g, o); }
    bb -= g;
  }
  if (lane == 0) { p.ea[gi] = a; p.eb[gi] = bb; }
}
__global__ __launch_bounds__(256) void att2_eoff4_kernel(const AttParams p) {
  const long gi = (long)blockIdx.x * 256 + threadIdx.x;
  if (gi >= (long)p.B * p.Rp) return;
  const int b = (int)(gi / p.Rp), k = (int)(gi - (long)b * p.Rp);
  const float* ea = p.ea + (size_t)b * p.Rp, *eb = p.eb + (size_t)b * p.Rp;
  auto at = [&](const float* t, int i) { return i < p.R ? t[i] : 0.f; };
  p.ea4[gi] = ((at(ea, k) + at(ea, k + 1)) + at(ea, k + p.wc)) + at(ea, k + p.wc + 1);
  const float b4 = ((at(eb, k) + at(eb, k + 1)) + at(eb, k + p.wc)) + at(eb, k + p.wc + 1);
  p.kadd2[gi] = fmaf(b4, p.kmul[gi], p.kadd[gi]);
}

template <int NT, int PT, bool BF16>
__global__ __launch_bounds__(256) void att2_pair_kernel(const AttParams p) {
  constexpr int PXB = BF16 ? 192 : 384;
  constexpr int PIX = PT * 64, NP = NT * 16;
  constexpr int XBYTES = PIX * 128, WBYTES = NP * 128;
  constexpr int NX = PT * 2, NW = (NT * 2 + 3) / 4;
  extern __shared__ __attribute__((aligned(16))) char smem[];
  char* Xb = smem;
  char* Wb = smem + 2 * XBYTES;

  const int tid = threadIdx.x, lane = tid & 63;
  const int w = __builtin_amdgcn_readfirstlane(tid >> 6);
  int b = blockIdx.z, bx = blockIdx.x, by = blockIdx.y;
  if (p.sym) {
    static_assert(PIX == 4 * NP, "tile enumeration");
    const int lb = xcd_tile(blockIdx.x, gridDim.x);
    b = lb / p.symT;
    const int t = lb - b * p.symT;
    int pn = (int)((sqrtf(64.f + 128.f * (float)t) - 8.f) * (1.f / 64.f));
    while (32 * (pn + 1) * (pn + 1) + 8 * (pn + 1) <= t) ++pn;
    while (32 * pn * pn + 8 * pn > t) --pn;
    const int u = t - (32 * pn * pn + 8 * pn);
    if (u < 64 * pn) {
      bx = u >> 4;
      by = 16 * pn + (u & 15);
    } else {
      const int v = u - 64 * pn;
      const int j = v < 16 ? 0 : (v < 28 ? 1 : (v < 36 ? 2 : 3));
      bx = 4 * pn + j;
      by = 16 * pn + 4 * j + (v - (j == 0 ? 0 : (j == 1 ? 16 : (j == 2 ? 28 : 36))));
    }
    if (by * NP >= p.R) return;
  }
  const int q0 = bx * PIX, k0 = by * NP;
  auto origin = [&](int i) -> unsigned {
    if (i >= p.R) return 0x80000000u;
    const int ry = i / p.wc, rx = i - ry * p.wc;
    return (unsigned)(((2 * ry) * p.w + 2 * rx) * PXB);
  };
  const se_i32x4 rs_q = make_rsrc((const char*)(p.sym ? p.xn : p.x) + (size_t)b * p.h * p.w * PXB, (unsigned)p.h * p.w * (unsigned)PXB);
  const se_i32x4 rs_k = make_rsrc((const char*)p.xn + (size_t)b * p.h * p.w * PXB, (unsigned)p.h * p.w * (unsigned)PXB);
  unsigned qo[NX], ko[NW];
#pragma unroll
  for (int i = 0; i < NX; ++i) qo[i] = origin(q0 + (i * 4 + w) * 8 + (lane >> 3));
#pragma unroll
  for (int j = 0; j < NW; ++j) ko[j] = (j * 4 + w) < NT * 2 ? origin(k0 + (j * 4 + w) * 8 + (lane >> 3)) : 0x80000000u;

  const int s_log = (lane & 7) ^ (4 * (w & 1) + (lane >> 4));
  int off0, off1;
  frag_offsets(lane, off0, off1);
  const unsigned lds_x = lds_addr_of(Xb), lds_w = lds_addr_of(Wb);

  auto stage = [&](int ch, int buf) {
    const int gi = ch * 8 + s_log;
    constexpr int GPP = BF16 ? 12 : 24;
    const int tap = (gi * (BF16 ? 5462 : 2731)) >> 16, cg = gi - tap * GPP;
    const unsigned doff = (unsigned)((__mul24(tap >> 1, p.w) + (tap & 1)) * PXB + cg * 16);
    const unsigned xdst = lds_x + buf * XBYTES, wdst = lds_w + buf * WBYTES;
#pragma unroll
    for (int i = 0; i < NX; ++i) bufdma16(qo[i] + doff, rs_q, xdst + (i * 4 + w) * 1024);
#pragma unroll
    for (int j = 0; j < NW; ++j) {
      const int rbk = j * 4 + w;
      if (rbk < NT * 2) bufdma16(ko[j] + doff, rs_k, wdst + rbk * 1024);
    }
  };

  f32x4 acc[NT][PT];
#pragma unroll
  for (int nt = 0; nt < NT; ++nt)
#pragma unroll
    for (int pt = 0; pt < PT; ++pt) acc[nt][pt] = (f32x4){0.f, 0.f, 0.f, 0.f};
  if (BF16 && p.e16) {
    const float* ea = p.ea + (size_t)b * p.Rp, *eb = p.eb + (size_t)b * p.Rp;
    float eq[PT];
#pragma unroll
    for (int pt = 0; pt < PT; ++pt) eq[pt] = ea[min(q0 + w * PT * 16 + pt * 16 + (lane & 15), p.Rp - 1)];
#pragma unroll
    for (int nt = 0; nt < NT; ++nt) {
      const f32x4 ek = *(const f32x4*)(eb + min(k0 + nt * 16 + (lane >> 4) * 4, p.Rp - 4));
#pragma unroll
      for (int pt = 0; pt < PT; ++pt) acc[nt][pt] = (f32x4){-(eq[pt] + ek[0]), -(eq[pt] + ek[1]), -(eq[pt] + ek[2]), -(eq[pt] + ek[3])};
    }
  }
  constexpr int NCH = BF16 ? 6 : 12;
  stage(0, 0);
  dma_wait_all();
  __syncthreads();
  for (int ch = 0; ch < NCH; ++ch) {
    const int buf = ch & 1;
    if (ch + 1 < NCH) stage(ch + 1, buf ^ 1);
    if (BF16) mfma_chunk16<NT, PT>(acc, Wb + buf * WBYTES, Xb + buf * XBYTES + w * PT * 2048, off0, off1);
    else mfma_chunk<NT, PT>(acc, Wb + buf * WBYTES, Xb + buf * XBYTES + w * PT * 2048, off0, off1);
    dma_wait_all();
// ... 645 lines not shown
  float qc[4];
#pragma unroll
  for (int j = 0; j < 4; ++j) {
    const int qy = qy0 + w, qx = qx0 + j;
    qc[j] = (EH && qy < p.hs && qx < p.ws) ? p.ea4[(size_t)b * p.Rp + qy * p.wc + qx] : 0.f;
  }
  for (int n = 0; n < nchunks; ++n) {
    const char* Eb = smem + (n % NS) * SB;
    const float* Kt = (const float*)(smem + (n % NS) * SB + NIP * 1024);
    __syncthreads();
    const int c = 2 * lane;
    f32x2 r0[5], r1[5];
    float x0[5], x1[5];
#pragma unroll
    for (int j = 0; j < 5; ++j) {
      lds_row3<EH>(Eb + (w * 5 + j) * WSB, c, r0[j], x0[j]);
      lds_row3<EH>(Eb + (w * 5 + 5 + j) * WSB, c + p.wc, r1[j], x1[j]);
    }
    const f32x2 mu = *(const f32x2*)(Kt + c), ad = *(const f32x2*)(Kt + C + c);
    const bool live = n * C + c < p.Rp;
#pragma unroll
    for (int j = 0; j < 4; ++j) {
      f32x2 sum = ((r0[j] + (f32x2){r0[j + 1][1], x0[j + 1]}) + r1[j]) + (f32x2){r1[j + 1][1], x1[j + 1]};
      if (EH) sum += (f32x2){qc[j], qc[j]};
      f32x2 t = sum * mu + ad;
      if (!live) t = (f32x2){-INFINITY, -INFINITY};
      const float mn = fmaxf(m_[j], fmaxf(t[0], t[1]));
      l_[j] = l_[j] * __builtin_amdgcn_exp2f(m_[j] - mn) + (__builtin_amdgcn_exp2f(t[0] - mn) + __builtin_amdgcn_exp2f(t[1] - mn));
      m_[j] = mn;
    }
  }
#pragma unroll
  for (int j = 0; j < 4; ++j) {
    float m = m_[j];
#pragma unroll
    for (int o = 32; o > 0; o >>= 1) m = fmaxf(m, __shfl_xor(m, o));
    float l = l_[j] * __builtin_amdgcn_exp2f(m_[j] - m);
#pragma unroll
    for (int o = 32; o > 0; o >>= 1) l += __shfl_xor(l, o);
    const int qy = qy0 + w, qx = qx0 + j;
    if (lane == 0 && qy < p.hs && qx < p.ws) *(float2*)(p.stats + ((size_t)b * p.R + qy * p.wc + qx) * 2) = make_float2(m, 1.f / l);
  }
}

template <int PT, int NT, bool BF16>
__global__ __launch_bounds__(256) void att2_pv_kernel(const AttParams p) {
  constexpr int PIX = PT * 64, NP = NT * 16, NRH = 6 / NT;
  constexpr int ES = BF16 ? 2 : 4;
  constexpr int XBYTES = PIX * 128, WBYTES = NP * 128;
  constexpr int NX = PT * 2, NW = (NT * 2 + 3) / 4;
  extern __shared__ __attribute__((aligned(16))) char smem[];
  char* Xb = smem;
  char* Wb = smem + 2 * XBYTES;

  const int tid = threadIdx.x, lane = tid & 63;
  const int w = __builtin_amdgcn_readfirstlane(tid >> 6);
  const int lb = xcd_tile(blockIdx.x, gridDim.x);
  const int cls = lb & 3, py = cls >> 1, px = cls & 1;
  const int rh = (lb >> 2) % NRH, lt = (lb >> 2) / NRH;
  const int nt_ = (p.R + PIX - 1) / PIX;
  const int b = lt / nt_, t0 = (lt - b * nt_) * PIX;
  const int s_log = (lane & 7) ^ (4 * (w & 1) + (lane >> 4));
  const se_i32x4 rs_P = make_rsrc((const char*)p.Pt + (size_t)b * p.R * p.Rp * ES, (unsigned)p.R * p.Rp * (unsigned)ES);
  const se_i32x4 rs_V = make_rsrc((const char*)p.xT + (((size_t)b * 4 + cls) * 96 + rh * NP) * p.Rp * ES, (unsigned)NP * p.Rp * (unsigned)ES);
  unsigned xo[NX], wo[NW];
#pragma unroll
  for (int i = 0; i < NX; ++i) {
    const int rl = (i * 4 + w) * 8 + (lane >> 3);
    const int r = t0 + rl;
    xo[i] = (rl < PIX && r < p.R) ? (unsigned)(r * p.Rp) * (unsigned)ES + s_log * 16u : 0x80000000u;
  }
#pragma unroll
  for (int j = 0; j < NW; ++j) {
    const int rl = (j * 4 + w) * 8 + (lane >> 3);
    wo[j] = rl < NP ? (unsigned)(rl * p.Rp) * (unsigned)ES + s_log * 16u : 0x80000000u;
  }
  int off0, off1;
  frag_offsets(lane, off0, off1);
  const unsigned lds_x = lds_addr_of(Xb), lds_w = lds_addr_of(Wb);
  const int nch = BF16 ? p.Rp >> 6 : p.Rp >> 5;

  auto stage = [&](int ch, int buf) {
    const unsigned delta = (unsigned)ch * 128u;
#pragma unroll
    for (int i = 0; i < NX; ++i)
      if ((i * 4 + w) * 8 < PIX) bufdma16(xo[i] + delta, rs_P, lds_x + buf * XBYTES + (i * 4 + w) * 1024);
#pragma unroll
    for (int j = 0; j < NW; ++j)
      if ((j * 4 + w) * 8 < NP) bufdma16(wo[j] + delta, rs_V, lds_w + buf * WBYTES + (j * 4 + w) * 1024);
  };

  f32x4 acc[NT][PT];
#pragma unroll
  for (int nt = 0; nt < NT; ++nt)
#pragma unroll
    for (int pt = 0; pt < PT; ++pt) acc[nt][pt] = (f32x4){0.f, 0.f, 0.f, 0.f};

  stage(0, 0);
  dma_wait_all();
  __syncthreads();
  for (int ch = 0; ch < nch; ++ch) {
    const int buf = ch & 1;
    if (ch + 1 < nch) stage(ch + 1, buf ^ 1);
    if (BF16) mfma_chunk16<NT, PT>(acc, Wb + buf * WBYTES, Xb + buf * XBYTES + w * PT * 2048, off0, off1);
    else mfma_chunk<NT, PT>(acc, Wb + buf * WBYTES, Xb + buf * XBYTES + w * PT * 2048, off0, off1);
    dma_wait_all();
    __syncthreads();
  }
  const int q = lane >> 4;
#pragma unroll
  for (int pt = 0; pt < PT; ++pt) {
    const int i = t0 + (w * PT + pt) * 16 + (lane & 15);
    if (i >= p.R) continue;
    const int yy = i / p.wc, xx = i - yy * p.wc;
    char* o = (char*)p.out + (((long)(b * p.h + 2 * yy + py) * p.w + 2 * xx + px) * 96 + rh * NP) * ES;
#pragma unroll
    for (int nt = 0; nt < NT; ++nt) {
      const f32x4 a = acc[nt][pt];
      if (BF16) *(uint2*)(o + (nt * 16 + q * 4) * 2) = make_uint2(pack_bf16x2(a[0], a[1]), pack_bf16x2(a[2], a[3]));
      else *(f32x4*)(o + (nt * 16 + q * 4) * 4) = a;
    }
  }
}

template <bool BF16>
__global__ void att2_similar_kernel(const AttParams p) {
  const long idx = (long)blockIdx.x * 256 + threadIdx.x;
  if (idx >= (long)p.B * p.L * p.L) return;
  const int i = idx % p.L;
  const long bj = idx / p.L;
  const int j = bj % p.L, b = bj / p.L;
  const int r = (i / p.ws) * p.wc + i % p.ws, s = (j / p.ws) * p.wc + j % p.ws;
  const size_t at = ((size_t)b * p.R + r) * p.Rp + s;
  p.similar[idx] = BF16 ? bf16_lo(((const unsigned short*)p.P)[at]) : p.P[at];
}

static bool att_lds_form(int wc) {
  return wc % 4 == 0 && wc <= 124 && opt(OPT_ATT_PTILDE_LDS) != 0;
}
static bool att_fused(bool bf16, int Rp, int wc) {
  const int e1 = opt(OPT_ATT_FUSED), e2 = opt(OPT_ATT_FUSED_BF16);
  const int f32mode = e1 < 0 ? -1 : (e1 != 0 ? 1 : 0);
  if (bf16) {
    if (e2 == 0) return false;
    if (e2 > 0) return f32mode < 0 ? att_lds_form(wc) : f32mode == 1;
    return f32mode != 0 && att_lds_form(wc);
  }
  return f32mode < 0 ? (Rp <= 1024 || att_lds_form(wc)) : f32mode == 1;
}

template <bool BF16>
static void enqueue_att2_prep(const AttParams& p, hipStream_t st) {
  const long n = (long)p.B * p.h * p.w * (BF16 ? 12 : 24);
  hipLaunchKernelGGL(att2_prep_kernel<BF16>, dim3((unsigned)((n + 255) / 256)), dim3(256), 0, st, p);
  hipLaunchKernelGGL(att2_transpose_kernel<BF16>, dim3(p.Rp / 32, 4, p.B), dim3(256), 0, st, p);
}

template <bool BF16>
static hipError_t launch_attention_v2_t(const AttParams& p0, hipStream_t st) {
  AttParams p = p0;
  const bool fused = att_fused(BF16, p.Rp, p.wc) && !p.similar && p.stats;
  p.Pt = fused ? p.P : p.E;
  p.sym = (!BF16 && opt(OPT_ATT_SYM) != 0) ? 1 : 0;
  const bool stats_lds = opt(OPT_ATT_STATS_LDS) != 0;
  p.e16 = (BF16 && fused && att_lds_form(p.wc) && stats_lds && opt(OPT_ATT_E16) != 0) ? 1 : 0;
  {
    const long n = (long)p.B * p.h * p.w * (BF16 ? 12 : 24);
    if (p.guard < p.wc + 8 || ((n + 255) / 256) * 256 < (long)p.guard) return hipErrorInvalidValue;
    ProfScope ps_(st, PL_ATT_PREP);
    enqueue_att2_prep<BF16>(p, st);
    if (p.e16) {
      const long nr = (long)p.B * p.Rp;
      hipLaunchKernelGGL(att2_emean1_kernel<BF16>, dim3(p.hc, p.B), dim3(384), 0, st, p);
      hipLaunchKernelGGL(att2_emean2_kernel, dim3(p.B), dim3(384), 0, st, p);
      hipLaunchKernelGGL(att2_eoff_kernel<BF16>, dim3((unsigned)((nr + 3) / 4)), dim3(256), 0, st, p);
      hipLaunchKernelGGL(att2_eoff4_kernel, dim3((unsigned)((nr + 255) / 256)), dim3(256), 0, st, p);
    }
  }
  {
    const double alg_flops = 2.0 * p.B * (double)p.L * p.L * 1536.0;
    const double alg_bytes = (BF16 ? 2.0 : 4.0) * 2.0 * p.B * (double)p.h * p.w * 96;
    const long big_grid = (long)((p.R + 255) / 256) * ((p.R + 63) / 64) * p.B;
    if (big_grid >= 512) {
      constexpr int NT = 4, PT = 4;
      constexpr int LDS = 2 * PT * 64 * 128 + 2 * NT * 16 * 128;
      hipError_t e = ensure_max_lds((const void*)att2_pair_kernel<NT, PT, BF16>, LDS);
      if (e != hipSuccess) return e;
      dim3 grid((p.R + PT * 64 - 1) / (PT * 64), (p.Rp + NT * 16 - 1) / (NT * 16), p.B);
      if (p.sym) {
        const int np = ((int)grid.y + 15) / 16;
        p.symT = 32 * np * np + 8 * np;
        grid = dim3((unsigned)(p.symT * p.B));
      }
      set_launch_cost(alg_flops, alg_bytes, nullptr, 2.0 * (double)grid.x * grid.y * grid.z * (PT * 64.0) * (NT * 16.0) * 384.0);
      set_launch_grid((long)grid.x * grid.y * grid.z);
      ProfScope ps_(st, PL_ATT_SCORE);
      hipLaunchKernelGGL((att2_pair_kernel<NT, PT, BF16>), grid, dim3(256), LDS, st, p);
    } else {
      constexpr int NT = 2, PT = 2;
      constexpr int LDS = 2 * PT * 64 * 128 + 2 * NT * 16 * 128;
      hipError_t e = ensure_max_lds((const void*)att2_pair_kernel<NT, PT, BF16>, LDS);
      if (e != hipSuccess) return e;
      dim3 grid((p.R + PT * 64 - 1) / (PT * 64), (p.Rp + NT * 16 - 1) / (NT * 16), p.B);
      if (p.sym) {
        const int np = ((int)grid.y + 15) / 16;
        p.symT = 32 * np * np + 8 * np;
        grid = dim3((unsigned)(p.symT * p.B));
      }
      set_launch_cost(alg_flops, alg_bytes, nullptr, 2.0 * (double)grid.x * grid.y * grid.z * (PT * 64.0) * (NT * 16.0) * 384.0);
      set_launch_grid((long)grid.x * grid.y * grid.z);
      ProfScope ps_(st, PL_ATT_SCORE);
      hipLaunchKernelGGL((att2_pair_kernel<NT, PT, BF16>), grid, dim3(256), LDS, st, p);
    }
  }
  if (fused) {
    const bool lds_form = att_lds_form(p.wc);
#define SE_LAUNCH_STATS_LDS(EH, NIP)                                                                                   \
  do {                                                                                                                 \
    constexpr int lds = 3 * ((NIP) + 1) * 1024;                                                                        \
    hipError_t e = ensure_max_lds((const void*)att2_stats_lds_kernel<EH, NIP, 3>, lds);                                \
    if (e != hipSuccess) return e;                                                                                     \
    const int npy = (p.hs + 3) / 4, npx = (p.ws + 3) / 4;                                                              \
    hipLaunchKernelGGL((att2_stats_lds_kernel<EH, NIP, 3>), dim3((unsigned)(p.B * npy * npx)), dim3(384), lds, st, p, npy, npx); \
  } while (0)
#define SE_LAUNCH_PTILDE_LDS(EH, NIP, NS)                                                                              \
  do {                                                                                                                 \
    constexpr int lds = (NS) * ((NIP) + 1) * 1024 + 25 * 256 * 4;                                                      \
    hipError_t e = ensure_max_lds((const void*)att2_ptilde_lds_kernel<BF16, EH, NIP, NS>, lds);                        \
    if (e != hipSuccess) return e;                                                                                     \
    const int npy = (p.hc + 3) / 4, npx = p.wc / 4;                                                                    \
    hipLaunchKernelGGL((att2_ptilde_lds_kernel<BF16, EH, NIP, NS>), dim3((unsigned)(p.B * npy * npx)), dim3(640), lds, st, p, npy, npx); \
  } while (0)
    {
      const long rows = tile_order_count(p.B, p.hs, p.ws);
      ProfScope ps_(st, PL_ATT_SOFTMAX);
      const dim3 grid((unsigned)((rows + 3) / 4));
      if (lds_form && stats_lds && (p.e16 || p.Rp > 1024)) {
        if (p.e16) { if (p.wc <= 64) SE_LAUNCH_STATS_LDS(true, 10); else SE_LAUNCH_STATS_LDS(true, 14); }
        else { if (p.wc <= 64) SE_LAUNCH_STATS_LDS(false, 20); else SE_LAUNCH_STATS_LDS(false, 26); }
      } else if (p.Rp <= 64 * 16) hipLaunchKernelGGL((att2_stats_kernel<16, BF16>), grid, dim3(256), 0, st, p);
      else if (p.Rp <= 64 * 64) hipLaunchKernelGGL((att2_stats_kernel<64, BF16>), grid, dim3(256), 0, st, p);
      else hipLaunchKernelGGL((att2_stats_kernel<0, BF16>), grid, dim3(256), 0, st, p);
    }
    {
      const long rows = tile_order_count(p.B, p.hc, p.wc);
      ProfScope ps_(st, PL_ATT_BOXSUM);
      const dim3 grid((unsigned)((rows + 3) / 4));
      if (lds_form) {
        bool done = false;
        if constexpr (BF16) {
          if (p.e16) {
            if (p.wc <= 64) SE_LAUNCH_PTILDE_LDS(true, 16, 3); else SE_LAUNCH_PTILDE_LDS(true, 18, 3);
            done = true;
          }
        }
        if (!done) { if (p.wc <= 64) SE_LAUNCH_PTILDE_LDS(false, 28, 4); else SE_LAUNCH_PTILDE_LDS(false, 36, 3); }
      } else if (p.wc % 4 == 0) hipLaunchKernelGGL((att2_ptilde4_kernel<BF16>), dim3((unsigned)((rows + 7) / 8)), dim3(512), 0, st, p);
      else hipLaunchKernelGGL((att2_ptilde1_kernel<BF16>), grid, dim3(256), 0, st, p);
    }
#undef SE_LAUNCH_STATS_LDS
#undef SE_LAUNCH_PTILDE_LDS
  } else {
    {
      const long rows = tile_order_count(p.B, p.hs, p.ws);
      ProfScope ps_(st, PL_ATT_SOFTMAX);
      const dim3 grid((unsigned)((rows + 3) / 4));
      if (p.Rp <= 64 * 16) hipLaunchKernelGGL((att2_softmax_reg_kernel<16, BF16>), grid, dim3(256), 0, st, p);
      else if (p.Rp <= 64 * 64) hipLaunchKernelGGL((att2_softmax_reg_kernel<64, BF16>), grid, dim3(256), 0, st, p);
      else hipLaunchKernelGGL(att2_softmax_kernel<BF16>, grid, dim3(256), 0, st, p);
    }
    if (p.similar) {
      const long n = (long)p.B * p.L * p.L;
      ProfScope ps_(st, PL_LAYOUT);
      hipLaunchKernelGGL(att2_similar_kernel<BF16>, dim3((unsigned)((n + 255) / 256)), dim3(256), 0, st, p);
    }
    {
      const long rows = tile_order_count(p.B, p.hc, p.wc);
      ProfScope ps_(st, PL_ATT_BOXSUM);
      if (p.wc % (BF16 ? 8 : 4) == 0) hipLaunchKernelGGL(att2_boxsum4_kernel<BF16>, dim3((unsigned)((rows + 3) / 4)), dim3(256), 0, st, p);
      else hipLaunchKernelGGL(att2_boxsum_kernel<BF16>, dim3((unsigned)((rows + 3) / 4)), dim3(256), 0, st, p);
    }
  }
  {
    const long big_grid = (long)((p.R + 255) / 256) * 4 * p.B;
    set_launch_cost(2.0 * p.B * (double)p.L * p.L * 1536.0, (BF16 ? 2.0 : 4.0) * 2.0 * p.B * (double)p.h * p.w * 96, nullptr,
                    2.0 * p.B * 4.0 * (double)p.R * p.Rp * 96.0);
    if (big_grid >= 512) {
      constexpr int PT = BF16 ? 3 : 2, NT = 6;
      constexpr int LDS = 2 * PT * 64 * 128 + 2 * NT * 16 * 128;
      hipError_t e = ensure_max_lds((const void*)att2_pv_kernel<PT, NT, BF16>, LDS);
      if (e != hipSuccess) return e;
      dim3 grid((unsigned)(((p.R + PT * 64 - 1) / (PT * 64)) * 4 * p.B));
      set_launch_grid((long)grid.x);
      ProfScope ps_(st, PL_ATT_PV);
      hipLaunchKernelGGL((att2_pv_kernel<PT, NT, BF16>), grid, dim3(256), LDS, st, p);
    } else {
      constexpr int PT = 1, NT = 3;
      constexpr int LDS = 2 * PT * 64 * 128 + 2 * NT * 16 * 128;
      hipError_t e = ensure_max_lds((const void*)att2_pv_kernel<PT, NT, BF16>, LDS);
      if (e != hipSuccess) return e;
      dim3 grid((unsigned)(((p.R + 63) / 64) * 2 * 4 * p.B));
      set_launch_grid((long)grid.x);
      ProfScope ps_(st, PL_ATT_PV);
      hipLaunchKernelGGL((att2_pv_kernel<PT, NT, BF16>), grid, dim3(256), LDS, st, p);
    }
  }
// ... 17 lines not shown
```

sketchedit_amd/csrc/se_kernels.h:

```cpp
#pragma once
#include <hip/hip_runtime.h>
#include <stddef.h>
#include <stdint.h>

#include <vector>

struct se_window;

namespace se {

enum ProfLabel { PL_GCONV_N192 = 0, PL_GCONV_N96, PL_GCONV_N48, PL_GCONV_N24, PL_WINO_N192, PL_WINO_N96, PL_WINO_UP96, PL_SMALL_CONV, PL_PACK, PL_COLREDUCE,
                 PL_ATT_PREP, PL_ATT_SCORE, PL_ATT_SOFTMAX, PL_ATT_BOXSUM, PL_ATT_PV, PL_LAYOUT,
                 PL_ATT_STREAM_STATS, PL_ATT_STREAM_OUT, PL_RESIZE_H, PL_RESIZE_V, PL_WINDOW_GATHER, PL_WINDOW_BORDER, PL_WINDOW_PASTE,
                 PL_WINDOW_RESAMPLE_H, PL_WINDOW_PASTE_V, PL_WINDOW_SAVE, PL_WINDOW_SWAP, PL_WINDOW_LOCK_GATHER, PL_WINDOW_PASTE_LOCKED,
                 PL_WINDOW_PASTE_V_LOCKED, PL_SKETCH_TILES, PL_SKETCH_STROKES, PL_PNG_ROWS, PL_PNG_STRIPES,
                 PL_PNG_FINISH, PL_COUNT };
const char* prof_label_name(int l);
struct Profiler {
  struct Rec { int label; const char* name; double flops; double exec_flops; double bytes; long blocks; hipEvent_t a, b; };
  std::vector<Rec> recs;
  std::vector<hipEvent_t> pool;
  size_t used = 0;
  bool on = false;
};
void set_profiler(Profiler* p);
void set_launch_cost(double flops, double bytes, const char* name = nullptr, double exec_flops = -1.0);
void set_launch_grid(long blocks);
hipError_t ensure_max_lds(const void* func, int bytes);

#define SE_OPTIONS(X)                                                                                         \
  X(XCD_REMAP, 1)                                                             \
  X(RTILE, 1)                                              \
  X(RTILE_LL_MIN, 256)         \
  X(RTILE_WX, 2)          \
  X(RTILE_DENSE, 1)                                          \
  X(RTILE_D5W, 1)                                        \
  X(TEST_OFFSET_LIMIT, 0)  \
  X(TEST_POISON, 0)       \
  X(RCONV16, 1) X(RCONV16_DUAL, 1) X(RCONV96, 1) X(VECBIAS, 1)                                                  \
  X(WINOGRAD, 1) X(WINOGRAD48, 1) X(WINOGRAD_UP, 1) X(WINOGRAD_UP48, 1)                                         \
  X(WINOGRAD_F43, 1)      \
  X(GCONV_FAST, 1) X(FORK_DEFAULT, 1) X(LL_WINO_MIN_WG, 64) X(LL_WINO48_MIN_WG, 128)                            \
  X(ATT_FUSED, -1) X(ATT_FUSED_BF16, -1) X(ATT_PTILDE_LDS, 1) X(ATT_STATS_LDS, 1) X(ATT_E16, 1) X(ATT_SYM, 1)   \
  X(ATT_STREAM, 0)
enum Opt {
#define X(name, dflt) OPT_##name,
  SE_OPTIONS(X)
#undef X
  OPT_COUNT
};
int opt(int o);
int opt_set(const char* name, int value);
int opt_get(const char* name, int* value);
void opt_reset();
long long opt_epoch();

struct GConvParams {
  const float* src0;
  const float* src1;
  const float* wpk;
  const float* bias;
  float* dst;
  const float* zeros;
  int B, Hin, Win, Ho, Wo;
  int C0, C1;
  int C0g, CG;
  int T, KW;
  int magicCG, magicKW;
  int magicKH;
  unsigned rep;
  unsigned div_hw_m, div_w_m;
  int div_hw_l, div_w_l;
  int stride, dil, pad;
  int ushift;
  int up2;
  int OH, OW;
  int Hlim, Wlim;
  int src1_vec;
  int nch;
  int G;
  int act;
  int total_pix;
  int xcd;
  int np_full;
  int nf_full;
  int bf16;
  int small_grid;
};

static inline void udiv_magic_host(unsigned d, unsigned* m, int* l) {
  int ll = 0;
  while ((1ull << ll) < d) ++ll;
  *l = ll;
  *m = (unsigned)(((1ull << 32) * ((1ull << ll) - d)) / d + 1);
}

enum GConvCfg { GC_N192 = 0, GC_N96 = 1, GC_N48 = 2, GC_N24 = 3 };
static inline int gconv_np(int cfg) { return cfg == GC_N192 ? 192 : cfg == GC_N96 ? 96 : cfg == GC_N48 ? 48 : 32; }
static inline bool gconv_mixed(int cfg) { return cfg >= GC_N48; }

hipError_t launch_gconv(int cfg, const GConvParams& p, hipStream_t st);

struct WinoParams {
  const float* src;
  const float* src1;
  int src1_vec;
  const float* upk;
  const float* bias;
  float* dst;
  int B, h, w, d;
  int th, tw;
  int total_tiles;
  int act;
  int xcd;
  unsigned div_tpi_m, div_tw_m, div_d_m;
  int div_tpi_l, div_tw_l, div_d_l;
  const float* vbias;
};
hipError_t launch_wino(const WinoParams& p, hipStream_t st);
hipError_t launch_vecbias(const float* wv, const float* vec, float* T, int B, int C1, hipStream_t st, int round_vec = 0);
hipError_t launch_wino24(const WinoParams& p, hipStream_t st);
hipError_t launch_wino24_c48(const WinoParams& p, hipStream_t st);
hipError_t launch_wino48(const WinoParams& p, hipStream_t st);
hipError_t launch_wino48_c24(const WinoParams& p, hipStream_t st);
hipError_t launch_winoup(const WinoParams& p, hipStream_t st);
hipError_t launch_winoup48(const WinoParams& p, hipStream_t st);

struct RConvParams {
  const void* src;
  const void* wpk;
  const float* bias;
  void* dst;
  int B, h, w, d;
  int hs, ws;
  int ty, tx;
  int act;
  int xcd;
  const float* vbias;
  int dual;
};
hipError_t launch_rconv16(const RConvParams& p, hipStream_t st);

struct RConv96Params {
  const void* src;
  const void* wpk;
  const float* bias;
  void* dst;
  int B, h, w;
  int CG;
  int ty, tx;
  int stride, oh, ow;
  int up2;
  int act;
  int xcd;
};
hipError_t launch_rconv96(const RConv96Params& p, hipStream_t st);

struct RTileParams {
  const float* src;
  const float* wpk;
  const float* bias;
  float* dst;
  int B, Hin, Win;
  int C;
  int CG;
  int T, KW;
  int magicCG, magicKW;
  int pad;
  int up2, OH, OW;
  int G;
  int nch, NP;
  int RH, RW;
  int raw_bytes;
  unsigned div_cg_m, div_rw_m;
  int div_cg_l, div_rw_l;
  int ty, tx;
  int act, bf16, xcd;
  int dense;
};
hipError_t launch_rtile(const RTileParams& p, hipStream_t st);
hipError_t launch_rtilew(const RTileParams& p, hipStream_t st);
hipError_t launch_rtilew2(const RTileParams& p, hipStream_t st);
int rtile_rows(bool bf16);

struct SmallConvParams {
  const float* x;
  const float* w;
  const float* b;
  int B, H, W, cout;
  int mode;
  float* out_nchw;
  float* hard;
  const float* img;
  const float* mask;
  float* xnow;
  float* composed;
  int no_mask_coarse;
  long out_bs;
  long mask_bs;
  long comp_bs;
  int bf16;
  unsigned char* rgb8;
  unsigned char* m8;
  const unsigned char* lock;
};
hipError_t launch_small_conv(const SmallConvParams& p, hipStream_t st);

hipError_t launch_pack_m(const float* image, const float* sketch, float* dst4, int B, int H, int W, hipStream_t st);
hipError_t launch_pack_g(const float* x, const float* x2, const float* mask, const float* mask2, const float* guide,
                         float* coarse8, float* style8, int B, int H, int W, int no_mask_cc, int joint,
                         hipStream_t st);
hipError_t launch_nchw_to_nhwc(const float* src, float* dst, int B, int C, int Cpad, int H, int W, hipStream_t st);
hipError_t launch_dequantize_u8(const unsigned char* rgb, const unsigned char* sk8, const float* lut, float* image, float* sketch,
                                int B, int H, int W, hipStream_t st);
hipError_t launch_nhwc_to_nchw(const float* src, float* dst, int B, int C, int Cstride, int H, int W, hipStream_t st);
hipError_t launch_quantize_u8(const float* composed, const float* mask, unsigned char* rgb, unsigned char* m8, int B, int H,
                              int W, hipStream_t st);
hipError_t launch_colreduce(const float* x, float* partial, float* out, int B, int HW, int C, int op, hipStream_t st,
                            int x_bf16 = 0, float* out_bf16 = nullptr);
hipError_t launch_pack_m16(const float* image, const float* sketch, float* dst8, int B, int H, int W, hipStream_t st);
hipError_t launch_pack_g16(const float* x, const float* x2, const float* mask, const float* mask2, const float* guide,
                           float* coarse8, float* style8, int B, int H, int W, int no_mask_cc, int joint, hipStream_t st);
hipError_t launch_nchw_to_nhwc16(const float* src, float* dst, int B, int C, int Cpad, int H, int W, hipStream_t st);
hipError_t launch_nhwc16_to_nchw(const float* src, float* dst, int B, int C, int Cstride, int H, int W, hipStream_t st);
static const int COLREDUCE_SPLITS = 128;

struct AttParams {
  const float* x;
  const float* rn;
  float* xn;
  const float* hard;
  float* valid;
  float* S;
  float* out;
  int B, h, w, hs, ws, L, Lp;
  float scale;
  float th;
  int hc, wc, R, Rp;
  float* xT;
  float* E;
  float* P;
  float* Pt;
  float* stats;
  float* kmul;
  float* kadd;
  int guard;
  float* validR;
  float* similar;
  int bf16;
  int e16;
  float* emean;
  float* epart;
  float* ea;
  float* eb;
  float* ea4;
  float* kadd2;
  int sym;
  int symT;
};
hipError_t launch_attention(const AttParams& p, hipStream_t st);
hipError_t launch_att2_prep(const AttParams& p, hipStream_t st);
hipError_t launch_attention_stream(const AttParams& p, hipStream_t st);
int att_stream_xt_tail();

int resample_ksize(int in, int out, int filter);
int resample_coeffs(int in, int out, int filter, int* bounds, int* kk);
enum { RESIZE_OUT_U8 = 0, RESIZE_OUT_IMAGE_F32 = 1, RESIZE_OUT_SKETCH_F32 = 2, RESIZE_OUT_LOCK_U8 = 3 };
struct ResizeOut {
  int mode;
  unsigned char* u8;
  float* f32;
  const float* lut;
  int H, W;
};
hipError_t launch_resample_h(const unsigned char* in, const int* d_bounds, const int* d_kk, const int* h_bounds, int ksize,
                             int B, int Hrows, int Win, int Wout, int C, const ResizeOut& o, hipStream_t st);
hipError_t launch_resample_v(const unsigned char* in, const int* d_bounds, const int* d_kk, int ksize, int B, int Hin, int Hout,
                             int W, int C, const ResizeOut& o, hipStream_t st);
hipError_t launch_window_resample_h(const se_window* d_wins, const int* d_bounds, const int* d_kk, const int* h_bounds, int ksize,
                                    int B, int hs, int ws, int Wout, int C, const ResizeOut& o, hipStream_t st);
hipError_t launch_window_paste_v(const se_window* d_wins, const unsigned char* rgb, const unsigned char* m8, const int* d_bounds,
                                 const int* d_kk, int ksize, int B, int Hin, int hs, int P, int ws, hipStream_t st, bool locked = false);
hipError_t launch_window_lock_resample_h(const se_window* d_wins, const int* d_bounds, const int* d_kk, const int* h_bounds, int ksize,
                                         int B, int hs, int ws, int Wout, const ResizeOut& o, hipStream_t st);
constexpr int RESAMPLE_MAX_KSIZE = 8191;

hipError_t launch_window_gather(const se_window* d_wins, const float* lut, float* image, float* sketch, int B, int H, int W,
                                hipStream_t st);
hipError_t launch_window_border(const se_window* d_wins, const unsigned char* m8, int* hits, int B, int H, int W, int hs, int ws,
                                hipStream_t st);
hipError_t launch_window_paste(const se_window* d_wins, const unsigned char* rgb, const unsigned char* m8, int B, int H, int W,
                               hipStream_t st, bool locked = false);
hipError_t launch_window_lock_gather(const se_window* d_wins, unsigned char* out, int B, int H, int W, hipStream_t st);
hipError_t launch_window_journal(const se_window* d_wins, int B, int hs, int ws, bool swap, hipStream_t st);
hipError_t launch_sketch_tiles(const unsigned char* plane, int Hi, int Wi, int tile, int* tiles_out, hipStream_t st);
hipError_t launch_sketch_strokes(const se_window* d_wins, int B, int hs, int ws, const int* segs, long nseg_sum, unsigned char* sketch_out,
                                 hipStream_t st);
int png_stripes(int hs);
size_t png_stripe_bound(size_t n);
size_t png_slot_bytes(int ws);
hipError_t launch_png_rows(const se_window* d_wins, int B, int hs, int ws, unsigned char* ftype, hipStream_t st);
hipError_t launch_png_stripes(const se_window* d_wins, int B, int hs, int ws, const unsigned char* ftype, unsigned* sizes, unsigned* parts,
                              unsigned char* slots, hipStream_t st);
hipError_t launch_png_finish(int B, int hs, int ws, const unsigned* sizes, const unsigned* parts, const unsigned char* slots, unsigned char* out,
                             size_t cap, unsigned long long* sizes_out, hipStream_t st);

}
```

sketchedit_amd/csrc/se_misc.hip:

```cpp
#include "se_device.h"

#include <atomic>
#include <cstdlib>
#include <cstring>
#include <mutex>
#include <set>
#include <utility>

namespace se {

namespace {
struct OptTable {
  std::atomic<int> v[OPT_COUNT];
  int dflt[OPT_COUNT];
  OptTable() { load(); }
  void load() {
    static const char* names[OPT_COUNT] = {
#define X(name, d) "SE_" #name,
        SE_OPTIONS(X)
#undef X
    };
    static const int builtin[OPT_COUNT] = {
#define X(name, d) d,
        SE_OPTIONS(X)
// ... 40 lines not shown
  return 0;
}
void opt_reset() {
  OptTable& t = opt_table();
  for (int i = 0; i < OPT_COUNT; ++i) t.v[i].store(t.dflt[i], std::memory_order_relaxed);
  g_opt_epoch.fetch_add(1, std::memory_order_relaxed);
}

static thread_local Profiler* g_prof = nullptr;
static thread_local double g_next_flops = 0.0, g_next_bytes = 0.0, g_next_exec = 0.0;
static thread_local const char* g_next_name = nullptr;
static thread_local long g_next_blocks = 0;
void set_profiler(Profiler* p) { g_prof = p; }
void set_launch_grid(long blocks) { g_next_blocks = blocks; }
void set_launch_cost(double flops, double bytes, const char* name, double exec_flops) {
  g_next_flops = flops; g_next_bytes = bytes; g_next_name = name; g_next_exec = exec_flops < 0.0 ? flops : exec_flops;
}

hipError_t ensure_max_lds(const void* func, int bytes) {
  static std::mutex mu;
  static std::set<std::pair<int, const void*>> done;
  int dev = 0;
  hipError_t e = hipGetDevice(&dev);
  if (e != hipSuccess) return e;
  std::lock_guard<std::mutex> lk(mu);
  const auto key = std::make_pair(dev, func);
  if (done.count(key)) return hipSuccess;
  e = hipFuncSetAttribute(func, hipFuncAttributeMaxDynamicSharedMemorySize, bytes);
  if (e == hipSuccess) done.insert(key);
  return e;
}
const char* prof_label_name(int l) {
  static const char* n[PL_COUNT] = {"gconv_n192", "gconv_n96", "gconv_n48", "gconv_n24", "wino_n192", "wino_n96", "wino_up96", "small_conv", "pack",
                                    "colreduce", "att_prep", "att_score", "att_softmax", "att_boxsum", "att_pv", "layout",
                                    "att_stream_stats", "att_stream_out", "resize_h", "resize_v", "window_gather", "window_border",
                                    "window_paste", "window_resample_h", "window_paste_v", "window_save", "window_swap", "window_lock_gather",
                                    "window_paste_locked", "window_paste_v_locked", "sketch_tiles", "sketch_strokes", "png_rows", "png_stripes",
                                    "png_finish"};
  return (l >= 0 && l < PL_COUNT) ? n[l] : "?";
}

ProfScope::ProfScope(hipStream_t s, int label) : st(s) {
  Profiler* p = g_prof;
  const double fl = g_next_flops, by = g_next_bytes, ex = g_next_exec;
  const char* nm = g_next_name;
  const long nb = g_next_blocks;
  g_next_blocks = 0;
  g_next_flops = g_next_bytes = g_next_exec = 0.0;
  g_next_name = nullptr;
  if (!p || !p->on) return;
  Profiler::Rec r;
  r.label = label; r.name = nm; r.flops = fl; r.exec_flops = ex; r.bytes = by; r.blocks = nb;
  if (p->used + 2 > p->pool.size()) return;
  r.a = p->pool[p->used++];
  r.b = p->pool[p->used++];
  (void)hipEventRecord(r.a, st);
  p->recs.push_back(r);
  idx = (int)p->recs.size() - 1;
}
ProfScope::~ProfScope() {
  if (idx >= 0) (void)hipEventRecord(g_prof->recs[idx].b, st);
}


template <int COUT, bool BF16, int SR>
__global__ __launch_bounds__(256) void small_conv_kernel(const SmallConvParams p) {
  const int HW = p.H * p.W;
  const int strips = (p.H + SR - 1) / SR;
  const long sidx = (long)xcd_tile(blockIdx.x, gridDim.x) * 256 + threadIdx.x;
  if (sidx >= (long)p.B * strips * p.W) return;
  const int b = (int)(sidx / ((long)strips * p.W));
  const int rem0 = (int)(sidx - (long)b * strips * p.W);
  const int sy = rem0 / p.W, x = rem0 - sy * p.W, y0 = sy * SR;
  f32x2 acc[SR][COUT];
#pragma unroll
  for (int o = 0; o < SR; ++o)
#pragma unroll
    for (int c = 0; c < COUT; ++c) acc[o][c] = (f32x2){p.b[c], 0.f};
  const f32x2* w2 = (const f32x2*)p.w;
  constexpr int PXB = BF16 ? 32 : 48;
  const __amdgpu_buffer_rsrc_t rs = __builtin_amdgcn_make_buffer_rsrc((void*)p.x, 0, (int)((unsigned)p.B * (unsigned)HW * (unsigned)PXB), 0x00020000);
  typedef unsigned u32x4 __attribute__((ext_vector_type(4)));
  typedef unsigned u32x2 __attribute__((ext_vector_type(2)));
  constexpr int RD = BF16 ? 6 : 12;
  auto load_row = [&](int r, unsigned (&raw)[3][RD]) {
    const int iy = y0 - 1 + r;
    const bool rowin = (unsigned)iy < (unsigned)p.H;
#pragma unroll
    for (int kx = 0; kx < 3; ++kx) {
      const int ix = x + kx - 1;
      const bool in = rowin && (unsigned)ix < (unsigned)p.W;
      const unsigned off = in ? (unsigned)((b * p.H + iy) * p.W + ix) * (unsigned)PXB : 0x80000000u;
      if (BF16) {
        const u32x4 a = __builtin_amdgcn_raw_buffer_load_b128(rs, (int)off, 0, 0);
        const u32x2 c = __builtin_amdgcn_raw_buffer_load_b64(rs, (int)off, 16, 0);
        raw[kx][0] = a[0]; raw[kx][1] = a[1]; raw[kx][2] = a[2]; raw[kx][3] = a[3]; raw[kx][4] = c[0]; raw[kx][5 % RD] = c[1];
      } else {
#pragma unroll
        for (int q = 0; q < 3; ++q) {
          const u32x4 t = __builtin_amdgcn_raw_buffer_load_b128(rs, (int)off, q * 16, 0);
#pragma unroll
          for (int e = 0; e < 4; ++e) raw[kx][(q * 4 + e) % RD] = t[e];
        }
      }
    }
  };
  auto use_row = [&](int r, const unsigned (&raw)[3][RD]) {
#pragma unroll
    for (int kx = 0; kx < 3; ++kx) {
      f32x2 v[6];
#pragma unroll
      for (int i = 0; i < 6; ++i)
        v[i] = BF16 ? (f32x2){bf16_lo(raw[kx][i % RD]), bf16_hi(raw[kx][i % RD])}
                    : (f32x2){__uint_as_float(raw[kx][(2 * i) % RD]), __uint_as_float(raw[kx][(2 * i + 1) % RD])};
#pragma unroll
      for (int o = 0; o < SR; ++o) {
        const int ky = r - o;
        if (ky < 0 || ky > 2) continue;
#pragma unroll
        for (int c = 0; c < COUT; ++c) {
          const f32x2* wc = w2 + (c * 9 + ky * 3 + kx) * 6;
#pragma unroll
          for (int i = 0; i < 6; ++i) acc[o][c] = v[i] * wc[i] + acc[o][c];
        }
      }
    }
  };
  unsigned rawA[3][RD], rawB[3][RD];
  load_row(0, rawA);
#pragma unroll 1
  for (int r = 0; r < SR + 2; r += 2) {
    load_row(r + 1, rawB);
    use_row(r, rawA);
    if (r + 2 < SR + 2) load_row(r + 2, rawA);
    use_row(r + 1, rawB);
  }
#pragma unroll
  for (int o = 0; o < SR; ++o) {
    const int y = y0 + o;
    if (y >= p.H) break;
    const int rem = y * p.W + x;
    const long idx = (long)b * HW + rem;
    float a1[COUT];
#pragma unroll
    for (int c = 0; c < COUT; ++c) a1[c] = acc[o][c][0] + acc[o][c][1];
    if (p.mode == 4) {
#pragma unroll
      for (int c = 0; c < COUT; ++c) p.out_nchw[((long)b * COUT + c) * HW + rem] = a1[c];
      continue;
    }
    if (p.mode == 0) {
      const float m = (p.lock && p.lock[idx]) ? 0.f : sigmoidf_(a1[0]);
      p.out_nchw[p.out_bs ? (long)b * p.out_bs + rem : idx] = m;
      if (p.hard) p.hard[idx] = m > 0.5f ? 1.f : 0.f;
      continue;
    }
    if constexpr (COUT == 3) {
      float t[3];
#pragma unroll
      for (int c = 0; c < 3; ++c) t[c] = tanh_fast(a1[c]);
      if (p.out_nchw) {
#pragma unroll
        for (int c = 0; c < 3; ++c) p.out_nchw[((long)b * 3 + c) * HW + rem] = t[c];
      }
      if (p.mode == 2) {
        const float m = p.mask[idx];
        f32x4 ov;
#pragma unroll
        for (int c = 0; c < 3; ++c) {
          const float xin = p.img[((long)b * 3 + c) * HW + rem] * (1.f - m);
          ov[c] = p.no_mask_coarse ? t[c] : t[c] * m + xin * (1.f - m);
        }
        ov[3] = 0.f;
        if (BF16) *(uint4*)((char*)p.xnow + idx * 16) = make_uint4(pack_bf16x2(ov[0], ov[1]), pack_bf16x2(ov[2], 0.f), 0u, 0u);
        else *(f32x4*)(p.xnow + idx * 4) = ov;
      } else if (p.mode == 3 && (p.composed || p.rgb8 || p.m8)) {
        const float m = p.mask[p.mask_bs ? (long)b * p.mask_bs + rem : idx];
        const long cb = p.comp_bs ? (long)b * p.comp_bs : (long)b * 3 * HW;
#pragma unroll
        for (int c = 0; c < 3; ++c) {
          const float im = p.img[((long)b * 3 + c) * HW + rem];
          const float v = t[c] * m + im * (1.f - m);
          if (p.composed) p.composed[cb + (long)c * HW + rem] = v;
          if (p.rgb8) p.rgb8[idx * 3 + c] = (unsigned char)(int)(((v + 1.f) * 0.5f) * 255.f);
        }
        if (p.m8) p.m8[idx] = (unsigned char)(int)(m * 255.f);
      }
    }
  }
}

hipError_t launch_small_conv(const SmallConvParams& p0, hipStream_t st) {
  const long HW = (long)p0.H * p0.W;
  const long pxb = p0.bf16 ? 32 : 48;
  if (HW * pxb >= (1l << 31)) return hipErrorInvalidValue;
  const int nbmax = (int)(((1l << 31) - 1) / (HW * pxb));
  ProfScope ps_(st, PL_SMALL_CONV);
  for (int b0 = 0; b0 < p0.B; b0 += nbmax) {
    SmallConvParams p = p0;
    p.B = p0.B - b0 < nbmax ? p0.B - b0 : nbmax;
    p.x = (const float*)((const char*)p0.x + (size_t)b0 * HW * pxb);
    const long cs = p0.mode == 4 ? p0.cout : (p0.mode == 0 ? 1 : 3);
    if (p0.out_nchw) p.out_nchw = p0.out_nchw + (size_t)b0 * (p0.out_bs ? p0.out_bs : cs * HW);
    if (p0.hard) p.hard = p0.hard + (size_t)b0 * HW;
    if (p0.lock) p.lock = p0.lock + (size_t)b0 * HW;
    if (p0.img) p.img = p0.img + (size_t)b0 * 3 * HW;
    if (p0.mask) p.mask = p0.mask + (size_t)b0 * (p0.mask_bs ? p0.mask_bs : HW);
    if (p0.xnow) p.xnow = (float*)((char*)p0.xnow + (size_t)b0 * HW * 16);
    if (p0.composed) p.composed = p0.composed + (size_t)b0 * (p0.comp_bs ? p0.comp_bs : 3 * HW);
    if (p0.rgb8) p.rgb8 = p0.rgb8 + (size_t)b0 * HW * 3;
    if (p0.m8) p.m8 = p0.m8 + (size_t)b0 * HW;
    const long n4 = (long)p.B * ((p.H + 3) / 4) * p.W;
    const bool small = (n4 + 255) / 256 < 256;
    const long n = small ? (long)p.B * ((p.H + 1) / 2) * p.W : n4;
    const int grid = (int)((n + 255) / 256);
#define SE_SC_LAUNCH(CO, BF)                                                                                        \
    do {                                                                                                              \
      if (small) hipLaunchKernelGGL((small_conv_kernel<CO, BF, 2>), dim3(grid), dim3(256), 0, st, p);                 \
      else hipLaunchKernelGGL((small_conv_kernel<CO, BF, 4>), dim3(grid), dim3(256), 0, st, p);                       \
    } while (0)
    if (p.cout == 1 && !p.bf16) SE_SC_LAUNCH(1, false);
    else if (p.cout == 3 && !p.bf16) SE_SC_LAUNCH(3, false);
    else if (p.cout == 1) SE_SC_LAUNCH(1, true);
    else if (p.cout == 3) SE_SC_LAUNCH(3, true);
    else return hipErrorInvalidValue;
#undef SE_SC_LAUNCH
  }
  return hipGetLastError();
}

__global__ void pack_m_kernel(const float* __restrict__ image, const float* __restrict__ sketch,
                              float* __restrict__ dst, int B, int HW) {
  const long idx = (long)blockIdx.x * 256 + threadIdx.x;
  if (idx >= (long)B * HW) return;
  const int b = idx / HW, rem = idx - (long)b * HW;
  f32x4 o;
  o[0] = image[((long)b * 3 + 0) * HW + rem];
  o[1] = image[((long)b * 3 + 1) * HW + rem];
  o[2] = image[((long)b * 3 + 2) * HW + rem];
  o[3] = sketch[idx];
  *(f32x4*)(dst + idx * 4) = o;
}
hipError_t launch_pack_m(const float* image, const float* sketch, float* dst4, int B, int H, int W, hipStream_t st) {
  const long n = (long)B * H * W;
  ProfScope ps_(st, PL_PACK);
  hipLaunchKernelGGL(pack_m_kernel, dim3((unsigned)((n + 255) / 256)), dim3(256), 0, st, image, sketch, dst4, B, H * W);
  return hipGetLastError();
}

__global__ void pack_g_kernel(const float* __restrict__ x, const float* __restrict__ x2, const float* __restrict__ mask,
                              const float* __restrict__ mask2, const float* __restrict__ guide,
                              float* __restrict__ coarse8, float* __restrict__ style8, int B, int HW, int no_mask_cc,
                              int joint) {
  const long idx = (long)blockIdx.x * 256 + threadIdx.x;
  if (idx >= (long)B * HW) return;
  const int b = idx / HW, rem = idx - (long)b * HW;
  const float m = mask[idx], m2 = mask2[idx], g = guide[idx];
  f32x4 c0, c1, s0, s1;
#pragma unroll
  for (int c = 0; c < 3; ++c) {
    const long o = ((long)b * 3 + c) * HW + rem;
    c0[c] = x[o] * (1.f - m);
    s0[c] = no_mask_cc ? x2[o] : x2[o] * m2;
  }
  c0[3] = g;
  c1 = (f32x4){m, 0.f, 0.f, 0.f};
  s0[3] = joint ? g * 0.f : g;
  s1 = (f32x4){m2, 0.f, 0.f, 0.f};
  *(f32x4*)(coarse8 + idx * 8) = c0;
  *(f32x4*)(coarse8 + idx * 8 + 4) = c1;
  if (joint) {
    s0[3] = m2;
    *(f32x4*)(style8 + idx * 4) = s0;
  } else {
    *(f32x4*)(style8 + idx * 8) = s0;
    *(f32x4*)(style8 + idx * 8 + 4) = s1;
  }
}
hipError_t launch_pack_g(const float* x, const float* x2, const float* mask, const float* mask2, const float* guide,
                         float* coarse8, float* style8, int B, int H, int W, int no_mask_cc, int joint,
                         hipStream_t st) {
  const long n = (long)B * H * W;
  ProfScope ps_(st, PL_PACK);
  hipLaunchKernelGGL(pack_g_kernel, dim3((unsigned)((n + 255) / 256)), dim3(256), 0, st, x, x2, mask, mask2, guide,
                     coarse8, style8, B, H * W, no_mask_cc, joint);
  return hipGetLastError();
}

__global__ void pack_m16_kernel(const float* __restrict__ image, const float* __restrict__ sketch, uint4* __restrict__ dst,
                                int B, int HW) {
  const long idx = (long)blockIdx.x * 256 + threadIdx.x;
  if (idx >= (long)B * HW) return;
  const int b = idx / HW, rem = idx - (long)b * HW;
  dst[idx] = make_uint4(pack_bf16x2(image[((long)b * 3 + 0) * HW + rem], image[((long)b * 3 + 1) * HW + rem]),
                        pack_bf16x2(image[((long)b * 3 + 2) * HW + rem], sketch[idx]), 0u, 0u);
}
hipError_t launch_pack_m16(const float* image, const float* sketch, float* dst8, int B, int H, int W, hipStream_t st) {
  const long n = (long)B * H * W;
  ProfScope ps_(st, PL_PACK);
  hipLaunchKernelGGL(pack_m16_kernel, dim3((unsigned)((n + 255) / 256)), dim3(256), 0, st, image, sketch, (uint4*)dst8, B, H * W);
  return hipGetLastError();
}
__global__ void pack_g16_kernel(const float* __restrict__ x, const float* __restrict__ x2, const float* __restrict__ mask,
                                const float* __restrict__ mask2, const float* __restrict__ guide, uint4* __restrict__ coarse8,
                                uint4* __restrict__ style8, int B, int HW, int no_mask_cc, int joint) {
  const long idx = (long)blockIdx.x * 256 + threadIdx.x;
  if (idx >= (long)B * HW) return;
  const int b = idx / HW, rem = idx - (long)b * HW;
  const float m = mask[idx], m2 = mask2[idx], g = guide[idx];
  float c[3], s[3];
#pragma unroll
  for (int k = 0; k < 3; ++k) {
    const long o = ((long)b * 3 + k) * HW + rem;
    c[k] = x[o] * (1.f - m);
    s[k] = no_mask_cc ? x2[o] : x2[o] * m2;
  }
  coarse8[idx] = make_uint4(pack_bf16x2(c[0], c[1]), pack_bf16x2(c[2], g), pack_bf16x2(m, 0.f), 0u);
  style8[idx] = joint ? make_uint4(pack_bf16x2(s[0], s[1]), pack_bf16x2(s[2], m2), 0u, 0u)
                      : make_uint4(pack_bf16x2(s[0], s[1]), pack_bf16x2(s[2], g), pack_bf16x2(m2, 0.f), 0u);
}
hipError_t launch_pack_g16(const float* x, const float* x2, const float* mask, const float* mask2, const float* guide,
                           float* coarse8, float* style8, int B, int H, int W, int no_mask_cc, int joint, hipStream_t st) {
  const long n = (long)B * H * W;
  ProfScope ps_(st, PL_PACK);
  hipLaunchKernelGGL(pack_g16_kernel, dim3((unsigned)((n + 255) / 256)), dim3(256), 0, st, x, x2, mask, mask2, guide,
                     (uint4*)coarse8, (uint4*)style8, B, H * W, no_mask_cc, joint);
  return hipGetLastError();
}
__global__ void nchw_to_nhwc16_kernel(const float* __restrict__ src, unsigned short* __restrict__ dst, int B, int C, int Cpad,
                                      int HW) {
  const long idx = (long)blockIdx.x * 256 + threadIdx.x;
  if (idx >= (long)B * HW * Cpad) return;
  const int c = idx % Cpad;
  const long pix = idx / Cpad;
  const int b = pix / HW, rem = pix - (long)b * HW;
  dst[idx] = (unsigned short)(pack_bf16x2(c < C ? src[((long)b * C + c) * HW + rem] : 0.f, 0.f) & 0xffffu);
}
hipError_t launch_nchw_to_nhwc16(const float* src, float* dst, int B, int C, int Cpad, int H, int W, hipStream_t st) {
  const long n = (long)B * H * W * Cpad;
  ProfScope ps_(st, PL_LAYOUT);
  hipLaunchKernelGGL(nchw_to_nhwc16_kernel, dim3((unsigned)((n + 255) / 256)), dim3(256), 0, st, src, (unsigned short*)dst, B, C,
                     Cpad, H * W);
  return hipGetLastError();
}
__global__ void nhwc16_to_nchw_kernel(const unsigned short* __restrict__ src, float* __restrict__ dst, int B, int C, int Cs,
                                      int HW) {
  const long idx = (long)blockIdx.x * 256 + threadIdx.x;
  if (idx >= (long)B * C * HW) return;
  const int rem = idx % HW;
  const long bc = idx / HW;
  const int c = bc % C, b = bc / C;
  dst[idx] = __uint_as_float((unsigned)src[((long)b * HW + rem) * Cs + c] << 16);
}
hipError_t launch_nhwc16_to_nchw(const float* src, float* dst, int B, int C, int Cstride, int H, int W, hipStream_t st) {
  const long n = (long)B * C * H * W;
  ProfScope ps_(st, PL_LAYOUT);
  hipLaunchKernelGGL(nhwc16_to_nchw_kernel, dim3((unsigned)((n + 255) / 256)), dim3(256), 0, st, (const unsigned short*)src, dst,
                     B, C, Cstride, H * W);
  return hipGetLastError();
}

__global__ void nchw_to_nhwc_kernel(const float* __restrict__ src, float* __restrict__ dst, int B, int C, int Cpad,
                                    int HW) {
  const long idx = (long)blockIdx.x * 256 + threadIdx.x;
// ... 9 lines not shown
  hipLaunchKernelGGL(nchw_to_nhwc_kernel, dim3((unsigned)((n + 255) / 256)), dim3(256), 0, st, src, dst, B, C, Cpad,
                     H * W);
  return hipGetLastError();
}
__global__ void nhwc_to_nchw_kernel(const float* __restrict__ src, float* __restrict__ dst, int B, int C, int Cs,
                                    int HW) {
  const long idx = (long)blockIdx.x * 256 + threadIdx.x;
  if (idx >= (long)B * C * HW) return;
  const int rem = idx % HW;
  const long bc = idx / HW;
  const int c = bc % C, b = bc / C;
  dst[idx] = src[((long)b * HW + rem) * Cs + c];
}
__global__ void quantize_u8_kernel(const float* __restrict__ comp, const float* __restrict__ mask,
                                   unsigned char* __restrict__ rgb, unsigned char* __restrict__ m8, int B, int HW) {
  const long q = (long)blockIdx.x * blockDim.x + threadIdx.x;
  const long nq = (long)B * HW / 4;
  if (q >= nq) return;
  const long pix = q * 4;
  const int b = (int)(pix / HW);
  const long in = pix - (long)b * HW;
  if (rgb) {
    unsigned char o[12];
#pragma unroll
    for (int c = 0; c < 3; ++c) {
      const float4 v = *(const float4*)(comp + ((long)b * 3 + c) * HW + in);
      const float f[4] = {v.x, v.y, v.z, v.w};
#pragma unroll
      for (int i = 0; i < 4; ++i) o[i * 3 + c] = (unsigned char)(int)(((f[i] + 1.f) * 0.5f) * 255.f);
    }
    unsigned* dst = (unsigned*)(rgb + pix * 3);
    dst[0] = o[0] | (o[1] << 8) | (o[2] << 16) | ((unsigned)o[3] << 24);
    dst[1] = o[4] | (o[5] << 8) | (o[6] << 16) | ((unsigned)o[7] << 24);
    dst[2] = o[8] | (o[9] << 8) | (o[10] << 16) | ((unsigned)o[11] << 24);
  }
  if (m8) {
    const float4 v = *(const float4*)(mask + pix);
    *(unsigned*)(m8 + pix) = (unsigned)(unsigned char)(int)(v.x * 255.f) | ((unsigned)(unsigned char)(int)(v.y * 255.f) << 8) |
                             ((unsigned)(unsigned char)(int)(v.z * 255.f) << 16) | ((unsigned)(unsigned char)(int)(v.w * 255.f) << 24);
  }
}
hipError_t launch_quantize_u8(const float* composed, const float* mask, unsigned char* rgb, unsigned char* m8, int B, int H,
                              int W, hipStream_t st) {
  const long nq = (long)B * H * W / 4;
  ProfScope ps_(st, PL_LAYOUT);
  hipLaunchKernelGGL(quantize_u8_kernel, dim3((unsigned)((nq + 255) / 256)), dim3(256), 0, st, composed, mask, rgb, m8, B, H * W);
  return hipGetLastError();
}

__global__ void dequant_u8_kernel(const unsigned char* __restrict__ rgb, const unsigned char* __restrict__ sk8,
                                  const float* __restrict__ lut, float* __restrict__ image, float* __restrict__ sketch, int B, int HW) {
  __shared__ float T[256];
  T[threadIdx.x] = lut[threadIdx.x];
  __syncthreads();
  const long q = (long)blockIdx.x * 256 + threadIdx.x;
  if (q >= (long)B * HW / 4) return;
  const long pix = q * 4;
  const int b = (int)(pix / HW);
  const long in = pix - (long)b * HW;
  if (image) {
    const unsigned* src = (const unsigned*)(rgb + pix * 3);
    const unsigned w0 = src[0], w1 = src[1], w2 = src[2];
    unsigned char v[12];
#pragma unroll
    for (int i = 0; i < 4; ++i) { v[i] = (w0 >> (8 * i)) & 255u; v[4 + i] = (w1 >> (8 * i)) & 255u; v[8 + i] = (w2 >> (8 * i)) & 255u; }
#pragma unroll
    for (int c = 0; c < 3; ++c)
      *(float4*)(image + ((long)b * 3 + c) * HW + in) = make_float4(T[v[c]], T[v[3 + c]], T[v[6 + c]], T[v[9 + c]]);
  }
  if (sketch) {
    const unsigned w = *(const unsigned*)(sk8 + pix);
    *(float4*)(sketch + pix) = make_float4((w & 0xffu) ? 1.f : 0.f, (w & 0xff00u) ? 1.f : 0.f, (w & 0xff0000u) ? 1.f : 0.f, (w & 0xff000000u) ? 1.f : 0.f);
  }
}
hipError_t launch_dequantize_u8(const unsigned char* rgb, const unsigned char* sk8, const float* lut, float* image, float* sketch,
                                int B, int H, int W, hipStream_t st) {
  const long nq = (long)B * H * W / 4;
  ProfScope ps_(st, PL_LAYOUT);
  hipLaunchKernelGGL(dequant_u8_kernel, dim3((unsigned)((nq + 255) / 256)), dim3(256), 0, st, rgb, sk8, lut, image, sketch, B, H * W);
  return hipGetLastError();
}

hipError_t launch_nhwc_to_nchw(const float* src, float* dst, int B, int C, int Cstride, int H, int W, hipStream_t st) {
  const long n = (long)B * C * H * W;
  ProfScope ps_(st, PL_LAYOUT);
  hipLaunchKernelGGL(nhwc_to_nchw_kernel, dim3((unsigned)((n + 255) / 256)), dim3(256), 0, st, src, dst, B, C, Cstride,
                     H * W);
  return hipGetLastError();
}

template <bool BF16>
__global__ __launch_bounds__(256) void colreduce_partial_kernel(const float* __restrict__ x, float* __restrict__ partial,
                                                                int HW, int C, int op) {
  constexpr int V = BF16 ? 8 : 4;
  __shared__ float red[256 * V];
  const int b = blockIdx.y, sp = blockIdx.x;
  const int per = (HW + COLREDUCE_SPLITS - 1) / COLREDUCE_SPLITS;
  const int p0 = sp * per, p1 = min(HW, p0 + per);
  const int CV = C / V;
  const int groups = 256 / CV;
  const int cv = threadIdx.x % CV, g = threadIdx.x / CV;
  float a[V];
#pragma unroll
  for (int e = 0; e < V; ++e) a[e] = op == 0 ? -INFINITY : 0.f;
  auto acc = [&](const uint4 u) {
    float v[V];
    if (BF16) {
      v[0] = bf16_lo(u.x); v[1] = bf16_hi(u.x); v[2] = bf16_lo(u.y); v[3] = bf16_hi(u.y);
      if (V == 8) { v[4] = bf16_lo(u.z); v[5] = bf16_hi(u.z); v[6] = bf16_lo(u.w); v[7] = bf16_hi(u.w); }
    } else {
      v[0] = __uint_as_float(u.x); v[1] = __uint_as_float(u.y); v[2] = __uint_as_float(u.z); v[3] = __uint_as_float(u.w);
    }
#pragma unroll
    for (int e = 0; e < V; ++e) a[e] = op == 0 ? fmaxf(a[e], v[e]) : (op == 1 ? a[e] + v[e] : fmaf(v[e], v[e], a[e]));
  };
  if (g < groups) {
    const uint4* row = (const uint4*)x + (long)b * HW * CV + cv;
    int pp = p0 + g;
    for (; pp + 3 * groups < p1; pp += 4 * groups) {
      const uint4 u0 = row[(long)pp * CV], u1 = row[(long)(pp + groups) * CV], u2 = row[(long)(pp + 2 * groups) * CV],
                  u3 = row[(long)(pp + 3 * groups) * CV];
      acc(u0); acc(u1); acc(u2); acc(u3);
    }
    for (; pp < p1; pp += groups) acc(row[(long)pp * CV]);
  }
#pragma unroll
  for (int e = 0; e < V; ++e) red[threadIdx.x * V + e] = a[e];
  __syncthreads();
  for (int c = threadIdx.x; c < C; c += 256) {
    const int cv2 = c / V, e = c - cv2 * V;
    float r = red[cv2 * V + e];
    for (int gg = 1; gg < groups; ++gg) {
      const float v = red[(gg * CV + cv2) * V + e];
      r = op == 0 ? fmaxf(r, v) : r + v;
    }
    partial[((long)b * COLREDUCE_SPLITS + sp) * C + c] = r;
  }
}
__global__ void colreduce_final_kernel(const float* __restrict__ partial, float* __restrict__ out, unsigned short* out16,
                                       int HW, int C, int op, int total) {
  const int idx = blockIdx.x * 256 + threadIdx.x;
  if (idx >= total) return;
  const int b = idx / C, c = idx - b * C;
  float r = op == 0 ? -INFINITY : 0.f;
  for (int sp = 0; sp < COLREDUCE_SPLITS; ++sp) {
    const float v = partial[((long)b * COLREDUCE_SPLITS + sp) * C + c];
    r = op == 0 ? fmaxf(r, v) : r + v;
  }
  if (op == 1) r = r / (float)HW;
  if (op == 2) r = 1.f / sqrtf(r + 1e-8f);
  out[idx] = r;
  if (out16) out16[idx] = (unsigned short)(pack_bf16x2(r, 0.f) & 0xffffu);
}
__global__ __launch_bounds__(768) void vecbias_kernel(const float* __restrict__ wv, const float* __restrict__ vec, float* __restrict__ T, int C1, int round_vec) {
  __shared__ float red[8][9][96];
  const int b = blockIdx.x, half = blockIdx.y;
  const int r = threadIdx.x % 96, g = threadIdx.x / 96, n = half * 96 + r;
  const int cg = C1 / 8;
  const float* v = vec + (size_t)b * C1 + g * cg;
  float part[9];
#pragma unroll
  for (int t = 0; t < 9; ++t) {
    const float* w = wv + ((size_t)t * C1 + g * cg) * 192 + n;
    float a0 = 0.f, a1 = 0.f, a2 = 0.f, a3 = 0.f;
    int c = 0;
    auto vv = [&](int i) { return round_vec ? bf16_lo(pack_bf16x2(v[i], 0.f) & 0xffffu) : v[i]; };
    for (; c + 4 <= cg; c += 4) {
      a0 = fmaf(w[(size_t)(c + 0) * 192], vv(c + 0), a0);
      a1 = fmaf(w[(size_t)(c + 1) * 192], vv(c + 1), a1);
      a2 = fmaf(w[(size_t)(c + 2) * 192], vv(c + 2), a2);
      a3 = fmaf(w[(size_t)(c + 3) * 192], vv(c + 3), a3);
    }
    for (; c < cg; ++c) a0 = fmaf(w[(size_t)c * 192], vv(c), a0);
    part[t] = (a0 + a1) + (a2 + a3);
  }
#pragma unroll
  for (int t = 0; t < 9; ++t) red[g][t][r] = part[t];
  __syncthreads();
  if (g == 0) {
#pragma unroll
    for (int t = 0; t < 9; ++t) {
      float a = red[0][t][r];
#pragma unroll
      for (int k = 1; k < 8; ++k) a += red[k][t][r];
      part[t] = a;
    }
#pragma unroll
    for (int cy = 0; cy < 3; ++cy)
#pragma unroll
      for (int cx = 0; cx < 3; ++cx) {
        float a = 0.f;
#pragma unroll
        for (int ky = 0; ky < 3; ++ky)
#pragma unroll
          for (int kx = 0; kx < 3; ++kx) {
            const bool in = !((cy == 0 && ky == 0) || (cy == 2 && ky == 2) || (cx == 0 && kx == 0) || (cx == 2 && kx == 2));
            if (in) a += part[ky * 3 + kx];
          }
        T[((size_t)b * 9 + cy * 3 + cx) * 192 + n] = a;
      }
  }
}
hipError_t launch_vecbias(const float* wv, const float* vec, float* T, int B, int C1, hipStream_t st, int round_vec) {
  if (C1 % 8) return hipErrorInvalidValue;
  ProfScope ps_(st, PL_COLREDUCE);
  hipLaunchKernelGGL(vecbias_kernel, dim3(B, 2), dim3(768), 0, st, wv, vec, T, C1, round_vec);
  return hipGetLastError();
}

hipError_t launch_colreduce(const float* x, float* partial, float* out, int B, int HW, int C, int op, hipStream_t st,
                            int x_bf16, float* out_bf16) {
  if (C > 256 || C % (x_bf16 ? 8 : 4)) return hipErrorInvalidValue;
  ProfScope ps_(st, PL_COLREDUCE);
  if (x_bf16) hipLaunchKernelGGL(colreduce_partial_kernel<true>, dim3(COLREDUCE_SPLITS, B), dim3(256), 0, st, x, partial, HW, C, op);
  else hipLaunchKernelGGL(colreduce_partial_kernel<false>, dim3(COLREDUCE_SPLITS, B), dim3(256), 0, st, x, partial, HW, C, op);
  hipLaunchKernelGGL(colreduce_final_kernel, dim3((B * C + 255) / 256), dim3(256), 0, st, partial, out,
                     (unsigned short*)out_bf16, HW, C, op, B * C);
  return hipGetLastError();
}

}
```

sketchedit_amd/kernel_labels.py:

```python

KERNEL_LABELS = {
    "wino_kernel": "wino_n192", "wino24_kernel": "wino_n192", "rconv16": "gconv_n192", "gconv_kernel<12": "gconv_n192",
    "wino48_kernel": "wino_n96", "rconv96": "gconv_n96", "gconv_kernel<6": "gconv_n96",
    "winoup_kernel": "wino_up96",
    "winoup48_kernel": "gconv_n48", "rtile_dense5w_kernel": "gconv_n48", "rtile_dense5_kernel": "gconv_n48",
    "rtile_kernel<3": "gconv_n48", "gconv_kernel<3": "gconv_n48",
    "rtilew2_kernel": "gconv_n24", "rtilew_kernel": "gconv_n24", "rtile_kernel<2": "gconv_n24", "gconv_kernel<2": "gconv_n24",
    "dtail_kernel": "dtail",
    "att2_pair_kernel": "att_score", "att2_pv_kernel": "att_pv",
    "att2_softmax": "att_softmax", "att2_stats": "att_softmax",
    "att2_boxsum": "att_boxsum", "att2_ptilde": "att_boxsum",
    "att2_prep": "att_prep", "att2_transpose": "att_prep", "att2_emean": "att_prep", "att2_eoff": "att_prep",
    "att2_similar": "layout",
    "small_conv_kernel": "small_conv", "pack_": "pack", "colreduce": "colreduce", "vecbias_kernel": "colreduce",
    "nchw_to_nhwc": "layout", "nhwc_to_nchw": "layout", "nhwc16_to_nchw": "layout", "quantize_u8_kernel": "layout",
    "dequant_u8_kernel": "layout",
    "(anonymous namespace)::window_resample_h_kernel": "window_resample_h", "(anonymous namespace)::window_paste_v_kernel": "window_paste_v",
    "window_resample_h_kernel": "window_resample_h", "window_paste_v_kernel": "window_paste_v",
    "(anonymous namespace)::resample_h_kernel": "resize_h", "(anonymous namespace)::resample_v_kernel": "resize_v",
    "resample_h_kernel": "resize_h", "resample_v_kernel": "resize_v",
    "(anonymous namespace)::window_gather_kernel": "window_gather", "(anonymous namespace)::window_border_kernel": "window_border",
    "(anonymous namespace)::window_paste_kernel": "window_paste",
    "window_gather_kernel": "window_gather", "window_border_kernel": "window_border", "window_paste_kernel": "window_paste",
    "(anonymous namespace)::window_save_kernel": "window_save", "(anonymous namespace)::window_swap_kernel": "window_swap",
    "window_save_kernel": "window_save", "window_swap_kernel": "window_swap",
    "(anonymous namespace)::sketch_tiles_kernel": "sketch_tiles", "sketch_tiles_kernel": "sketch_tiles",
    "(anonymous namespace)::sketch_strokes_kernel": "sketch_strokes", "sketch_strokes_kernel": "sketch_strokes",
    "(anonymous namespace)::png_rows_kernel": "png_rows", "(anonymous namespace)::png_stripe_kernel": "png_stripes",
    "(anonymous namespace)::png_finish_kernel": "png_finish",
    "png_rows_kernel": "png_rows", "png_stripe_kernel": "png_stripes", "png_finish_kernel": "png_finish",
}


def kernel_key(name):
    return name.split("(")[0].replace("void se::", "").replace("se::", "")


def label_of(name):
    k = kernel_key(name)
    return next((v for pre, v in KERNEL_LABELS.items() if k.startswith(pre)), None)
```

Measured before the change: 2958 images/sec.

## Fuse glue kernels: pack netG inputs in netM tail, merge att prep, fold pooling

```diff
diff --git a/sketchedit_amd/csrc/se_api.hip b/sketchedit_amd/csrc/se_api.hip
--- a/sketchedit_amd/csrc/se_api.hip
+++ b/sketchedit_amd/csrc/se_api.hip
@@ -123,6 +123,7 @@
   const se_netG_taps* taps = nullptr;
   float* vbias_ws = nullptr;
   const float* vec32 = nullptr;
+  struct PendingVec { const float* part = nullptr; float* out = nullptr; float* out16 = nullptr; int HW = 0, op = 0; } pvec;
   unsigned char* rgb8 = nullptr;
   unsigned char* m8 = nullptr;
   Profiler prof;
@@ -358,6 +359,20 @@
   return 0;
 }
 
+static int finish_style_vec(se_ctx* c, int B) {
+  if (!c->pvec.part) return 0;
+  HIPCHK(c, launch_colreduce_final(c->pvec.part, c->pvec.out, B, c->pvec.HW, 96, c->pvec.op, c->st, c->pvec.out16));
+  c->pvec.part = nullptr;
+  return 0;
+}
+static int run_vecbias(se_ctx* c, const float* wv, const float* vec, int B, int round_vec) {
+  if (c->pvec.part) {
+    HIPCHK(c, launch_vecbias_pooled(wv, c->pvec.part, c->pvec.out, c->pvec.out16, c->vbias_ws, B, 96, c->pvec.HW, c->pvec.op, c->st, round_vec));
+    c->pvec.part = nullptr;
+  } else HIPCHK(c, launch_vecbias(wv, vec, c->vbias_ws, B, 96, c->st, round_vec));
+  return 0;
+}
+
 static bool rconv16_dual_ok(const Layer& L, const LayerDef& d, int Hin, int Win) {
   if (opt(OPT_RCONV16_DUAL) == 0) return false;
   return L.d_w16s && (d.rate % 2) == 0 && Win / d.rate == 8 && Hin / d.rate <= 8 && Hin / d.rate >= 4;
@@ -373,7 +388,7 @@
     if (opt(OPT_VECBIAS) != 0 && use_rconv && !c->low_latency && src1 && src1_vec && c->vbias_ws && c->vec32 && L.d_w16s && L.d_wv16 &&
         d.k == 3 && d.stride == 1 && d.rate == 1 && !d.up && d.cin == 192 && d.cout == 192 && C0 == 96 && C1 == 96 &&
         Hin >= 12 && Win >= 12 && (long long)B * Hin * Win * 192 < (1ll << 31)) {
-      HIPCHK(c, launch_vecbias(L.d_wv16, c->vec32, c->vbias_ws, B, 96, c->st, 1));
+      if (run_vecbias(c, L.d_wv16, c->vec32, B, 1)) return 1;
       RConvParams rp;
       memset(&rp, 0, sizeof rp);
       rp.src = src0; rp.wpk = L.d_w16s; rp.bias = L.d_b; rp.dst = dst; rp.vbias = c->vbias_ws;
@@ -401,6 +416,7 @@
     HIPCHK(c, launch_rconv16(rp, c->st));
     return 0;
   }
+  if (src1 && src1_vec && finish_style_vec(c, B)) return 1;
   const bool use_rconv96 = opt(OPT_RCONV96) != 0;
   if (use_rconv96 && !c->low_latency && L.d_w96 && !src1 && C0 == d.cin && Hin >= 12 && Win >= 12 &&
       (long long)B * Ho * Wo * 96 < (1ll << 31) && (long long)B * Hin * Win * C0 * 2 < (1ll << 31)) {
@@ -468,7 +484,8 @@
   if (use_wino && !d.up && L.d_u && wino_src_ok && wino_addr_ok && (Hin % (2 * d.rate)) == 0 && (Win % (2 * d.rate)) == 0 &&
       wino_grid_ok(((long)(Hin / 2) * (Win / 2) + 63) / 64, true)) {
     const bool folded = opt(OPT_VECBIAS) != 0 && src1 && src1_vec && d.rate == 1 && L.d_u1 && L.d_wv && c->vbias_ws && Hin >= 2 && Win >= 2;
-    if (folded) HIPCHK(c, launch_vecbias(L.d_wv, src1, c->vbias_ws, B, 96, c->st));
+    if (folded) { if (run_vecbias(c, L.d_wv, src1, B, 0)) return 1; }
+    else if (src1 && src1_vec && finish_style_vec(c, B)) return 1;
     const float* s1 = folded ? nullptr : src1;
     const int f43_mode = opt(OPT_WINOGRAD_F43);
     const bool f43_net_ok = c->cur_net == SE_NET_G || (f43_mode == 1 && !c->conservative);
@@ -486,6 +503,7 @@
     HIPCHK(c, launch_wino(wp, c->st));
     return 0;
   }
+  if (src1 && src1_vec && finish_style_vec(c, B)) return 1;
   {
     if (use_wino && opt(OPT_WINOGRAD_F43) != 0 && !d.up && !src1 && C0 == 48 && d.cin == 48 && d.cout == 192 && d.stride == 1 && L.d_u24 && L.d_ub24 &&
         (long long)B * Hin * Win * 384 < (1ll << 31) && (Hin % (2 * d.rate)) == 0 && (Win % (4 * d.rate)) == 0 &&
@@ -551,11 +569,12 @@
   int B;
   int rc = 0;
   Arena* ar;
+  bool no_poison = false;
   Plan(se_ctx* c_, std::map<std::string, Layer>& n, int B_) : c(c_), net(n), B(B_), ar(&c_->arena) {}
   float* alloc_raw(size_t nfloats) {
     float* p = ar->alloc(nfloats);
     if (!p && !rc) rc = fail(c, "workspace too small (need more than %zu bytes)", ar->cap);
-    if (p && !rc && !c->dry && poison(c, p, (nfloats * 4 + 255) & ~(size_t)255, c->st)) rc = 1;
+    if (p && !rc && !c->dry && !no_poison && poison(c, p, (nfloats * 4 + 255) & ~(size_t)255, c->st)) rc = 1;
     return p;
   }
   Act alloc(int H, int W, int C) {
@@ -569,6 +588,12 @@
     }
     if (c->dry) c->dry_max_act = std::max(c->dry_max_act, (size_t)B * H * W * a.C * (c->bf16 ? 2 : 4));
     return a;
+  }
+  void alloc_g_inputs(int H, int W, int joint, Act& cin, Act& sin) {
+    cin = alloc(H, W, 8);
+    ar = forked() ? &c->arena2 : &c->arena;
+    sin = alloc(H, W, joint ? 4 : 8);
+    ar = &c->arena;
   }
   void release(const float* p) {
     if (!p) return;
@@ -639,9 +664,17 @@
   return x;
 }
 
+struct PrePack {
+  int flags = 0;
+  const float* image = nullptr;
+  const float* sketch = nullptr;
+  float* cin = nullptr;
+  float* sin = nullptr;
+};
+
 int small(Plan& P, const char* name, Act& in, int mode, float* out_nchw, float* hard, const float* img,
           const float* mask, float* xnow, float* composed, int no_mask_coarse, long packed_bs = 0,
-          const unsigned char* lock = nullptr) {
+          const unsigned char* lock = nullptr, const PrePack* pre = nullptr) {
   if (P.rc) return P.rc;
   se_ctx* c = P.c;
   if (!c->dry) {
@@ -655,6 +688,10 @@
     sp.composed = composed; sp.no_mask_coarse = no_mask_coarse;
     if (mode == 3) { sp.rgb8 = c->rgb8; sp.m8 = c->m8; }
     if (mode == 0) sp.lock = lock;
+    if (mode == 0 && pre) {
+      sp.img = pre->image; sp.sketch = pre->sketch; sp.pk_coarse = pre->cin; sp.pk_style = pre->sin;
+      sp.pk_no_mask_cc = (pre->flags & SE_FLAG_NO_MASK_CC) ? 1 : 0; sp.pk_joint = (pre->flags & SE_FLAG_JOINT_TRAIN_INP) ? 1 : 0;
+    }
     if (packed_bs) {
       if (mode == 0) sp.out_bs = packed_bs;
       if (mode == 3) { sp.mask_bs = packed_bs; sp.comp_bs = packed_bs; }
@@ -669,9 +706,16 @@
 }
 
 int plan_netM(se_ctx* c, const float* image, const float* sketch, float* mask_out, float* hard_out, float* maskim_out,
-              int B, int H, int W, long packed_bs = 0, const unsigned char* lock = nullptr) {
+              int B, int H, int W, long packed_bs = 0, const unsigned char* lock = nullptr, PrePack* pre = nullptr) {
   Plan P(c, c->M, B);
   c->cur_net = SE_NET_M;
+  if (pre) {
+    Act cin, sin;
+    P.alloc_g_inputs(H, W, (pre->flags & SE_FLAG_JOINT_TRAIN_INP) ? 1 : 0, cin, sin);
+    if (P.rc) return P.rc;
+    pre->cin = cin.p; pre->sin = sin.p; pre->image = image; pre->sketch = sketch;
+    if (!hard_out && !c->dry) return fail(c, "internal: packing netG's inputs needs the hard mask");
+  }
   Act in = P.alloc(H, W, 4);
   if (P.rc) return P.rc;
   if (!c->dry) HIPCHK(c, c->bf16 ? launch_pack_m16(image, sketch, in.p, B, H, W, c->st) : launch_pack_m(image, sketch, in.p, B, H, W, c->st));
@@ -683,7 +727,7 @@
     small(P, "conv17", d, 1, maskim_out, nullptr, nullptr, nullptr, nullptr, nullptr, 0);
   }
   Act d = decoder(P, "conv_mask_", x10);
-  small(P, "conv_mask_17", d, 0, mask_out, hard_out, nullptr, nullptr, nullptr, nullptr, 0, packed_bs, lock);
+  small(P, "conv_mask_17", d, 0, mask_out, hard_out, nullptr, nullptr, nullptr, nullptr, 0, packed_bs, lock, pre);
   return P.rc;
 }
 
@@ -691,29 +735,40 @@
 
 int plan_netG(se_ctx* c, const float* x, const float* x2, const float* mask, const float* mask2, const float* guide,
               float* coarse_out, float* fine_out, const float* soft_mask, float* composed_out, int B, int H, int W,
-              int flags, long packed_bs = 0) {
+              int flags, long packed_bs = 0, const PrePack* pre = nullptr) {
   Plan P(c, c->G, B);
   c->cur_net = SE_NET_G;
+  c->pvec.part = nullptr;
   const int joint = (flags & SE_FLAG_JOINT_TRAIN_INP) ? 1 : 0;
-  Act cin = P.alloc(H, W, 8);
-  P.ar = P.forked() ? &c->arena2 : &c->arena;
-  Act sin = P.alloc(H, W, joint ? 4 : 8);
-  P.ar = &c->arena;
+  Act cin, sin;
+  P.no_poison = pre != nullptr;
+  P.alloc_g_inputs(H, W, joint, cin, sin);
+  P.no_poison = false;
   if (P.rc) return P.rc;
-  if (!c->dry)
+  if (pre && !c->dry && (cin.p != pre->cin || sin.p != pre->sin)) return fail(c, "internal: netG's packed inputs are not where netM wrote them");
+  if (!c->dry && !pre)
     HIPCHK(c, (c->bf16 ? launch_pack_g16 : launch_pack_g)(x, x2, mask, mask2, guide, cin.p, sin.p, B, H, W,
                                                           (flags & SE_FLAG_NO_MASK_CC) ? 1 : 0, joint, c->st));
   if (P.side_begin()) return 1;
   Act xs = encoder(P, "wconv", sin, nullptr, joint ? &c->wconv1_j4 : nullptr);
   Act part = P.alloc(1, COLREDUCE_SPLITS, 192), vec32 = P.alloc(1, 1, 192), vec = P.alloc(1, 1, 96);
   if (P.rc) return P.rc;
-  if (!c->dry)
-    HIPCHK(c, launch_colreduce(xs.p, part.p, c->bf16 ? vec32.p : vec.p, B, xs.H * xs.W, 96, (flags & SE_FLAG_POOL_MAX) ? 0 : 1,
-                               c->st, c->bf16 ? 1 : 0, c->bf16 ? vec.p : nullptr));
-  if (!c->dry && c->taps && c->taps->style_vec)
-    HIPCHK(c, hipMemcpyAsync(c->taps->style_vec, c->bf16 ? vec32.p : vec.p, (size_t)B * 96 * 4, hipMemcpyDeviceToDevice, c->st));
+  const bool pend = opt(OPT_GLUE_VECBIAS) != 0;
+  const int pool_op = (flags & SE_FLAG_POOL_MAX) ? 0 : 1;
+  if (!c->dry) {
+    if (pend) {
+      HIPCHK(c, launch_colreduce_partial(xs.p, part.p, B, xs.H * xs.W, 96, pool_op, c->st, c->bf16 ? 1 : 0));
+      c->pvec.part = part.p; c->pvec.out = c->bf16 ? vec32.p : vec.p; c->pvec.out16 = c->bf16 ? vec.p : nullptr;
+      c->pvec.HW = xs.H * xs.W; c->pvec.op = pool_op;
+    } else {
+      HIPCHK(c, launch_colreduce(xs.p, part.p, c->bf16 ? vec32.p : vec.p, B, xs.H * xs.W, 96, pool_op,
+                                 c->st, c->bf16 ? 1 : 0, c->bf16 ? vec.p : nullptr));
+      if (c->taps && c->taps->style_vec)
+        HIPCHK(c, hipMemcpyAsync(c->taps->style_vec, c->bf16 ? vec32.p : vec.p, (size_t)B * 96 * 4, hipMemcpyDeviceToDevice, c->st));
+    }
+  }
   P.free(xs);
-  P.free(part);
+  if (!pend) P.free(part);
   if (!c->bf16) P.free(vec32);
   if (P.side_end()) return 1;
   Act xc = encoder(P, "conv", cin, nullptr);
@@ -725,6 +780,13 @@
   c->vec32 = c->bf16 ? vec32.p : nullptr;
   Act d = decoder(P, "conv", xc, vec.p, 96, 1);
   c->vbias_ws = nullptr; c->vec32 = nullptr;
+  if (c->pvec.part) { c->pvec.part = nullptr; if (!P.rc) return P.rc = fail(c, "internal: the style vector was never reduced"); }
+  if (P.rc) return P.rc;
+  if (pend) {
+    if (!c->dry && c->taps && c->taps->style_vec)
+      HIPCHK(c, hipMemcpyAsync(c->taps->style_vec, c->bf16 ? vec32.p : vec.p, (size_t)B * 96 * 4, hipMemcpyDeviceToDevice, c->st));
+    P.free(part);
+  }
   P.release(vb);
   if (c->bf16) P.free(vec32);
   P.free(vec);
@@ -894,7 +956,10 @@
   se_ctx::Peaks pk{0, 0};
   if (which & 1) {
     c->arena.reset(nullptr, 0, true, 0); c->arena2.reset(nullptr, 0, true, 1);
-    plan_netM(c, nullptr, nullptr, nullptr, nullptr, want_maskim ? &dummy : nullptr, B, H, W);
+    PrePack pre;
+    pre.flags = flags;
+    plan_netM(c, nullptr, nullptr, nullptr, nullptr, want_maskim ? &dummy : nullptr, B, H, W, 0, nullptr,
+              (which == 3 && opt(OPT_GLUE_PACK_G) != 0) ? &pre : nullptr);
     pk.main = c->arena.peak; pk.side = c->arena2.peak;
   }
   if (which & 2) {
@@ -1288,12 +1353,16 @@
     const float *img = image + b0 * 3 * HW, *sk = sketch + b0 * HW;
     float *hard = hard_all + b0 * HW, *mk = mask_out + b0 * mask_bs;
     begin_call(c, stream, flags);
+    const float *gx = img, *gx2 = img, *gmask = hard, *gmask2 = hard, *guide = sk;
+    PrePack pre;
+    pre.flags = flags;
+    const bool fuse = opt(OPT_GLUE_PACK_G) != 0 && gx2 == gx && gmask2 == gmask;
     int rc = plan_netM(c, img, sk, mk, hard, maskim_out ? maskim_out + b0 * 3 * HW : nullptr, bb, H, W, packed_bs,
-                       lock8 ? lock8 + b0 * HW : nullptr);
+                       lock8 ? lock8 + b0 * HW : nullptr, fuse ? &pre : nullptr);
     if (rc) return rc;
     if (carve(c, pk, ws, ws_bytes, plane)) return 1;
-    rc = plan_netG(c, img, img, hard, hard, sk, coarse_out ? coarse_out + b0 * 3 * HW : nullptr, fine_out ? fine_out + b0 * 3 * HW : nullptr,
-                   mk, composed_out + b0 * comp_bs, bb, H, W, flags, packed_bs);
+    rc = plan_netG(c, gx, gx2, gmask, gmask2, guide, coarse_out ? coarse_out + b0 * 3 * HW : nullptr, fine_out ? fine_out + b0 * 3 * HW : nullptr,
+                   mk, composed_out + b0 * comp_bs, bb, H, W, flags, packed_bs, fuse ? &pre : nullptr);
     if (rc) return rc;
   }
   return 0;
diff --git a/sketchedit_amd/csrc/se_attention.hip b/sketchedit_amd/csrc/se_attention.hip
--- a/sketchedit_amd/csrc/se_attention.hip
+++ b/sketchedit_amd/csrc/se_attention.hip
@@ -79,6 +79,75 @@
 }
 
 template <bool BF16>
+__global__ __launch_bounds__(256) void att2_prologue_kernel(const AttParams p) {
+  __shared__ float t[32][97];
+  const int s0 = blockIdx.x * 32, cls = blockIdx.y, b = blockIdx.z, py = cls >> 1, px = cls & 1;
+  constexpr int GPP = BF16 ? 12 : 24;
+  for (int e = threadIdx.x; e < 32 * GPP; e += 256) {
+    const int sl = e / GPP, cg = e - sl * GPP, s = s0 + sl;
+    if (s < p.R) {
+      const int sy = s / p.wc, sx = s - sy * p.wc;
+      const size_t gi = ((size_t)(b * p.h + 2 * sy + py) * p.w + 2 * sx + px) * GPP + cg;
+      if (BF16) {
+        const uint4 v = *(const uint4*)((const char*)p.x + gi * 16);
+        const f32x4 r0 = *(const f32x4*)(p.rn + b * 96 + cg * 8), r1 = *(const f32x4*)(p.rn + b * 96 + cg * 8 + 4);
+        *(uint4*)((char*)p.xn + gi * 16) =
+            make_uint4(pack_bf16x2(bf16_lo(v.x) * r0[0], bf16_hi(v.x) * r0[1]), pack_bf16x2(bf16_lo(v.y) * r0[2], bf16_hi(v.y) * r0[3]),
+                       pack_bf16x2(bf16_lo(v.z) * r1[0], bf16_hi(v.z) * r1[1]), pack_bf16x2(bf16_lo(v.w) * r1[2], bf16_hi(v.w) * r1[3]));
+        float* tp = &t[sl][cg * 8];
+        tp[0] = bf16_lo(v.x); tp[1] = bf16_hi(v.x); tp[2] = bf16_lo(v.y); tp[3] = bf16_hi(v.y);
+        tp[4] = bf16_lo(v.z); tp[5] = bf16_hi(v.z); tp[6] = bf16_lo(v.w); tp[7] = bf16_hi(v.w);
+      } else {
+        const f32x4 v = *(const f32x4*)(p.x + gi * 4);
+        f32x4 r = *(const f32x4*)(p.rn + b * 96 + cg * 4);
+        if (p.sym) r = (f32x4){sqrtf(r[0]), sqrtf(r[1]), sqrtf(r[2]), sqrtf(r[3])};
+        *(f32x4*)(p.xn + gi * 4) = v * r;
+        float* tp = &t[sl][cg * 4];
+        tp[0] = v[0]; tp[1] = v[1]; tp[2] = v[2]; tp[3] = v[3];
+      }
+    } else {
+      float* tp = &t[sl][cg * (BF16 ? 8 : 4)];
+#pragma unroll
+      for (int k = 0; k < (BF16 ? 8 : 4); ++k) tp[k] = 0.f;
+    }
+  }
+  __syncthreads();
+  for (int e = threadIdx.x; e < 96 * 32; e += 256) {
+    const int c = e >> 5, sl = e & 31;
+    const size_t at = (((size_t)b * 4 + cls) * 96 + c) * p.Rp + s0 + sl;
+    if (BF16) ((unsigned short*)p.xT)[at] = (unsigned short)(__float_as_uint(t[sl][c]) >> 16);
+    else p.xT[at] = t[sl][c];
+  }
+  if (threadIdx.x < 8) {
+    const int s = s0 + cls * 8 + threadIdx.x;
+    const long idx = (long)b * p.Rp + s;
+    float val = -1.f;
+    const int sy = s / p.wc, sx = s - sy * p.wc;
+    if (s < p.R && sy < p.hs && sx < p.ws) {
+      const int H = p.h * 4, W = p.w * 4;
+      float hole = 0.f;
+      for (int yy = 0; yy < 16; ++yy)
+        for (int xx = 0; xx < 16; ++xx) hole += p.hard[((long)b * H + sy * 8 + yy) * W + sx * 8 + xx];
+      const float mm = 1.f - hole * (1.f / 256.f);
+      val = mm > p.th ? 1.f : 0.f;
+    }
+    p.validR[idx] = val;
+    if (p.kmul) {
+      p.kmul[idx] = val > 0.f ? p.scale * 1.44269504088896340736f : 0.f;
+      p.kadd[idx] = val >= 0.f ? 0.f : -INFINITY;
+    }
+  }
+  if (blockIdx.x == 0 && cls == 0 && b == 0) {
+    for (int i = threadIdx.x; i < p.guard; i += 256) {
+      p.validR[-1 - i] = -1.f;
+      if (p.kmul) { p.kmul[-1 - i] = 0.f; p.kadd[-1 - i] = -INFINITY; }
+      p.E[-1 - i] = 0.f;
+      p.E[(size_t)p.B * p.R * p.Rp + i] = 0.f;
+    }
+  }
+}
+
+template <bool BF16>
 __global__ __launch_bounds__(384) void att2_emean1_kernel(const AttParams p) {
   const int ry = blockIdx.x, b = blockIdx.y, e = threadIdx.x, cls = e / 96, c = e - cls * 96;
   const size_t row0 = ((size_t)(b * p.h + 2 * ry + (cls >> 1)) * p.w + (cls & 1)) * 96 + c;
@@ -1030,6 +1099,10 @@
 template <bool BF16>
 static void enqueue_att2_prep(const AttParams& p, hipStream_t st) {
   const long n = (long)p.B * p.h * p.w * (BF16 ? 12 : 24);
+  if (opt(OPT_GLUE_ATT_PREP) != 0 && p.B <= 65535) {
+    hipLaunchKernelGGL(att2_prologue_kernel<BF16>, dim3(p.Rp / 32, 4, p.B), dim3(256), 0, st, p);
+    return;
+  }
   hipLaunchKernelGGL(att2_prep_kernel<BF16>, dim3((unsigned)((n + 255) / 256)), dim3(256), 0, st, p);
   hipLaunchKernelGGL(att2_transpose_kernel<BF16>, dim3(p.Rp / 32, 4, p.B), dim3(256), 0, st, p);
 }
diff --git a/sketchedit_amd/csrc/se_kernels.h b/sketchedit_amd/csrc/se_kernels.h
--- a/sketchedit_amd/csrc/se_kernels.h
+++ b/sketchedit_amd/csrc/se_kernels.h
@@ -42,7 +42,10 @@
   X(WINOGRAD_F43, 1)      \
   X(GCONV_FAST, 1) X(FORK_DEFAULT, 1) X(LL_WINO_MIN_WG, 64) X(LL_WINO48_MIN_WG, 128)                            \
   X(ATT_FUSED, -1) X(ATT_FUSED_BF16, -1) X(ATT_PTILDE_LDS, 1) X(ATT_STATS_LDS, 1) X(ATT_E16, 1) X(ATT_SYM, 1)   \
-  X(ATT_STREAM, 0)
+  X(ATT_STREAM, 0)        \
+  X(GLUE_PACK_G, 1)                \
+  X(GLUE_ATT_PREP, 1)                     \
+  X(GLUE_VECBIAS, 1)
 enum Opt {
 #define X(name, dflt) OPT_##name,
   SE_OPTIONS(X)
@@ -119,6 +122,8 @@
 };
 hipError_t launch_wino(const WinoParams& p, hipStream_t st);
 hipError_t launch_vecbias(const float* wv, const float* vec, float* T, int B, int C1, hipStream_t st, int round_vec = 0);
+hipError_t launch_vecbias_pooled(const float* wv, const float* partial, float* vec_out, float* vec_out_bf16, float* T, int B, int C1,
+                                 int HW, int op, hipStream_t st, int round_vec = 0);
 hipError_t launch_wino24(const WinoParams& p, hipStream_t st);
 hipError_t launch_wino24_c48(const WinoParams& p, hipStream_t st);
 hipError_t launch_wino48(const WinoParams& p, hipStream_t st);
@@ -203,6 +208,10 @@
   unsigned char* rgb8;
   unsigned char* m8;
   const unsigned char* lock;
+  const float* sketch;
+  float* pk_coarse;
+  float* pk_style;
+  int pk_no_mask_cc, pk_joint;
 };
 hipError_t launch_small_conv(const SmallConvParams& p, hipStream_t st);
 
@@ -218,6 +227,8 @@
                               int W, hipStream_t st);
 hipError_t launch_colreduce(const float* x, float* partial, float* out, int B, int HW, int C, int op, hipStream_t st,
                             int x_bf16 = 0, float* out_bf16 = nullptr);
+hipError_t launch_colreduce_partial(const float* x, float* partial, int B, int HW, int C, int op, hipStream_t st, int x_bf16 = 0);
+hipError_t launch_colreduce_final(const float* partial, float* out, int B, int HW, int C, int op, hipStream_t st, float* out_bf16 = nullptr);
 hipError_t launch_pack_m16(const float* image, const float* sketch, float* dst8, int B, int H, int W, hipStream_t st);
 hipError_t launch_pack_g16(const float* x, const float* x2, const float* mask, const float* mask2, const float* guide,
                            float* coarse8, float* style8, int B, int H, int W, int no_mask_cc, int joint, hipStream_t st);
diff --git a/sketchedit_amd/csrc/se_misc.hip b/sketchedit_amd/csrc/se_misc.hip
--- a/sketchedit_amd/csrc/se_misc.hip
+++ b/sketchedit_amd/csrc/se_misc.hip
@@ -216,7 +216,32 @@
     if (p.mode == 0) {
       const float m = (p.lock && p.lock[idx]) ? 0.f : sigmoidf_(a1[0]);
       p.out_nchw[p.out_bs ? (long)b * p.out_bs + rem : idx] = m;
-      if (p.hard) p.hard[idx] = m > 0.5f ? 1.f : 0.f;
+      const float hm = m > 0.5f ? 1.f : 0.f;
+      if (p.hard) p.hard[idx] = hm;
+      if (p.pk_coarse) {
+        const float g = p.sketch[idx];
+        float cx[3], sx[3];
+#pragma unroll
+        for (int k = 0; k < 3; ++k) {
+          const float v = p.img[((long)b * 3 + k) * HW + rem];
+          cx[k] = v * (1.f - hm);
+          sx[k] = p.pk_no_mask_cc ? v : v * hm;
+        }
+        if (BF16) {
+          ((uint4*)p.pk_coarse)[idx] = make_uint4(pack_bf16x2(cx[0], cx[1]), pack_bf16x2(cx[2], g), pack_bf16x2(hm, 0.f), 0u);
+          ((uint4*)p.pk_style)[idx] = p.pk_joint ? make_uint4(pack_bf16x2(sx[0], sx[1]), pack_bf16x2(sx[2], hm), 0u, 0u)
+                                                 : make_uint4(pack_bf16x2(sx[0], sx[1]), pack_bf16x2(sx[2], g), pack_bf16x2(hm, 0.f), 0u);
+        } else {
+          *(f32x4*)(p.pk_coarse + idx * 8) = (f32x4){cx[0], cx[1], cx[2], g};
+          *(f32x4*)(p.pk_coarse + idx * 8 + 4) = (f32x4){hm, 0.f, 0.f, 0.f};
+          if (p.pk_joint) {
+            *(f32x4*)(p.pk_style + idx * 4) = (f32x4){sx[0], sx[1], sx[2], hm};
+          } else {
+            *(f32x4*)(p.pk_style + idx * 8) = (f32x4){sx[0], sx[1], sx[2], g};
+            *(f32x4*)(p.pk_style + idx * 8 + 4) = (f32x4){hm, 0.f, 0.f, 0.f};
+          }
+        }
+      }
       continue;
     }
     if constexpr (COUT == 3) {
@@ -274,6 +299,9 @@
     if (p0.composed) p.composed = p0.composed + (size_t)b0 * (p0.comp_bs ? p0.comp_bs : 3 * HW);
     if (p0.rgb8) p.rgb8 = p0.rgb8 + (size_t)b0 * HW * 3;
     if (p0.m8) p.m8 = p0.m8 + (size_t)b0 * HW;
+    if (p0.sketch) p.sketch = p0.sketch + (size_t)b0 * HW;
+    if (p0.pk_coarse) p.pk_coarse = (float*)((char*)p0.pk_coarse + (size_t)b0 * HW * (p0.bf16 ? 16 : 32));
+    if (p0.pk_style) p.pk_style = (float*)((char*)p0.pk_style + (size_t)b0 * HW * ((p0.bf16 || p0.pk_joint) ? 16 : 32));
     const long n4 = (long)p.B * ((p.H + 3) / 4) * p.W;
     const bool small = (n4 + 255) / 256 < 256;
     const long n = small ? (long)p.B * ((p.H + 1) / 2) * p.W : n4;
@@ -589,12 +617,33 @@
   out[idx] = r;
   if (out16) out16[idx] = (unsigned short)(pack_bf16x2(r, 0.f) & 0xffffu);
 }
-__global__ __launch_bounds__(768) void vecbias_kernel(const float* __restrict__ wv, const float* __restrict__ vec, float* __restrict__ T, int C1, int round_vec) {
+template <bool POOLED>
+__global__ __launch_bounds__(768) void vecbias_kernel(const float* __restrict__ wv, const float* __restrict__ vec, float* __restrict__ T, int C1, int round_vec,
+                                                      float* __restrict__ vec_out, unsigned short* __restrict__ vec_out16, int HW, int op) {
   __shared__ float red[8][9][96];
+  __shared__ float pooled[POOLED ? 256 : 1];
   const int b = blockIdx.x, half = blockIdx.y;
   const int r = threadIdx.x % 96, g = threadIdx.x / 96, n = half * 96 + r;
   const int cg = C1 / 8;
-  const float* v = vec + (size_t)b * C1 + g * cg;
+  if (POOLED) {
+    const int c = threadIdx.x;
+    if (c < C1) {
+      float pv[COLREDUCE_SPLITS];
+#pragma unroll
+      for (int sp = 0; sp < COLREDUCE_SPLITS; ++sp) pv[sp] = vec[((long)b * COLREDUCE_SPLITS + sp) * C1 + c];
+      float a = op == 0 ? -INFINITY : 0.f;
+#pragma unroll
+      for (int sp = 0; sp < COLREDUCE_SPLITS; ++sp) a = op == 0 ? fmaxf(a, pv[sp]) : a + pv[sp];
+      if (op == 1) a = a / (float)HW;
+      pooled[c] = a;
+      if (half == 0) {
+        vec_out[b * C1 + c] = a;
+        if (vec_out16) vec_out16[b * C1 + c] = (unsigned short)(pack_bf16x2(a, 0.f) & 0xffffu);
+      }
+    }
+    __syncthreads();
+  }
+  const float* v = POOLED ? pooled + g * cg : vec + (size_t)b * C1 + g * cg;
   float part[9];
 #pragma unroll
   for (int t = 0; t < 9; ++t) {
@@ -641,19 +690,43 @@
 hipError_t launch_vecbias(const float* wv, const float* vec, float* T, int B, int C1, hipStream_t st, int round_vec) {
   if (C1 % 8) return hipErrorInvalidValue;
   ProfScope ps_(st, PL_COLREDUCE);
-  hipLaunchKernelGGL(vecbias_kernel, dim3(B, 2), dim3(768), 0, st, wv, vec, T, C1, round_vec);
-  return hipGetLastError();
-}
-
+  hipLaunchKernelGGL(vecbias_kernel<false>, dim3(B, 2), dim3(768), 0, st, wv, vec, T, C1, round_vec, (float*)nullptr, (unsigned short*)nullptr, 0, 0);
+  return hipGetLastError();
+}
+hipError_t launch_vecbias_pooled(const float* wv, const float* partial, float* vec_out, float* vec_out_bf16, float* T, int B, int C1,
+                                 int HW, int op, hipStream_t st, int round_vec) {
+  if (C1 % 8 || C1 > 256 || (op != 0 && op != 1)) return hipErrorInvalidValue;
+  ProfScope ps_(st, PL_COLREDUCE);
+  hipLaunchKernelGGL(vecbias_kernel<true>, dim3(B, 2), dim3(768), 0, st, wv, partial, T, C1, round_vec, vec_out, (unsigned short*)vec_out_bf16, HW, op);
+  return hipGetLastError();
+}
+
+static void enqueue_colreduce_partial(const float* x, float* partial, int B, int HW, int C, int op, hipStream_t st, int x_bf16) {
+  if (x_bf16) hipLaunchKernelGGL(colreduce_partial_kernel<true>, dim3(COLREDUCE_SPLITS, B), dim3(256), 0, st, x, partial, HW, C, op);
+  else hipLaunchKernelGGL(colreduce_partial_kernel<false>, dim3(COLREDUCE_SPLITS, B), dim3(256), 0, st, x, partial, HW, C, op);
+}
+static void enqueue_colreduce_final(const float* partial, float* out, int B, int HW, int C, int op, hipStream_t st, float* out_bf16) {
+  hipLaunchKernelGGL(colreduce_final_kernel, dim3((B * C + 255) / 256), dim3(256), 0, st, partial, out,
+                     (unsigned short*)out_bf16, HW, C, op, B * C);
+}
 hipError_t launch_colreduce(const float* x, float* partial, float* out, int B, int HW, int C, int op, hipStream_t st,
                             int x_bf16, float* out_bf16) {
   if (C > 256 || C % (x_bf16 ? 8 : 4)) return hipErrorInvalidValue;
   ProfScope ps_(st, PL_COLREDUCE);
-  if (x_bf16) hipLaunchKernelGGL(colreduce_partial_kernel<true>, dim3(COLREDUCE_SPLITS, B), dim3(256), 0, st, x, partial, HW, C, op);
-  else hipLaunchKernelGGL(colreduce_partial_kernel<false>, dim3(COLREDUCE_SPLITS, B), dim3(256), 0, st, x, partial, HW, C, op);
-  hipLaunchKernelGGL(colreduce_final_kernel, dim3((B * C + 255) / 256), dim3(256), 0, st, partial, out,
-                     (unsigned short*)out_bf16, HW, C, op, B * C);
-  return hipGetLastError();
-}
-
-}
+  enqueue_colreduce_partial(x, partial, B, HW, C, op, st, x_bf16);
+  enqueue_colreduce_final(partial, out, B, HW, C, op, st, out_bf16);
+  return hipGetLastError();
+}
+hipError_t launch_colreduce_partial(const float* x, float* partial, int B, int HW, int C, int op, hipStream_t st, int x_bf16) {
+  if (C > 256 || C % (x_bf16 ? 8 : 4)) return hipErrorInvalidValue;
+  ProfScope ps_(st, PL_COLREDUCE);
+  enqueue_colreduce_partial(x, partial, B, HW, C, op, st, x_bf16);
+  return hipGetLastError();
+}
+hipError_t launch_colreduce_final(const float* partial, float* out, int B, int HW, int C, int op, hipStream_t st, float* out_bf16) {
+  ProfScope ps_(st, PL_COLREDUCE);
+  enqueue_colreduce_final(partial, out, B, HW, C, op, st, out_bf16);
+  return hipGetLastError();
+}
+
+}
diff --git a/sketchedit_amd/kernel_labels.py b/sketchedit_amd/kernel_labels.py
--- a/sketchedit_amd/kernel_labels.py
+++ b/sketchedit_amd/kernel_labels.py
@@ -10,7 +10,7 @@
     "att2_pair_kernel": "att_score", "att2_pv_kernel": "att_pv",
     "att2_softmax": "att_softmax", "att2_stats": "att_softmax",
     "att2_boxsum": "att_boxsum", "att2_ptilde": "att_boxsum",
-    "att2_prep": "att_prep", "att2_transpose": "att_prep", "att2_emean": "att_prep", "att2_eoff": "att_prep",
+    "att2_prologue": "att_prep", "att2_prep": "att_prep", "att2_transpose": "att_prep", "att2_emean": "att_prep", "att2_eoff": "att_prep",
     "att2_similar": "layout",
     "small_conv_kernel": "small_conv", "pack_": "pack", "colreduce": "colreduce", "vecbias_kernel": "colreduce",
     "nchw_to_nhwc": "layout", "nhwc_to_nchw": "layout", "nhwc16_to_nchw": "layout", "quantize_u8_kernel": "layout",
```

Result: no change. 2954 images/sec (-0.1%).
